# yuanzhi-zhu/DiffPIR

Hardware: AMD Instinct MI355X
Metric: restored images/sec @100 NFE, 256x256 (higher is better)
Workload: dtype f32 (GEMMs as 3 x f16 MFMA on hi/lo-split fp32 operands, fp32 accumulate; exact-fp32-MFMA mode in alt_precision); 1 GPU; configs[1]: ffhq topology 256x256 deblur (61x61 Gaussian PSF), 100 NFE, batch 16/GPU, device Philox noise, hipGraph=on; global_batch=16, nfe=100, collective=none

## Files before the change

### diffpir_amd/_lib.py

```python
from __future__ import annotations

import ctypes as C
import os

_HERE = os.path.dirname(os.path.abspath(__file__))
LIB_PATH = os.environ.get("DIFFPIR_LIB") or os.path.join(_HERE, "csrc", "libdiffpir_hip.so")
ABI_VERSION = 2



class UNetDesc(C.Structure):
    _fields_ = [("image_size", C.c_int32), ("in_channels", C.c_int32), ("model_channels", C.c_int32),
                ("out_channels", C.c_int32), ("num_res_blocks", C.c_int32), ("num_head_channels", C.c_int32),
                ("n_channel_mult", C.c_int32), ("channel_mult", C.c_float * 8),
                ("n_attention_ds", C.c_int32), ("attention_ds", C.c_int32 * 8), ("num_classes", C.c_int32)]


class Tensor(C.Structure):
    _fields_ = [("name", C.c_char_p), ("data", C.c_void_p), ("ndim", C.c_int32), ("shape", C.c_int64 * 4)]


class Step(C.Structure):
    _fields_ = [("t", C.c_int32), ("last", C.c_int32), ("c1", C.c_float), ("c2", C.c_float), ("tau", C.c_float),
                ("sa_t", C.c_float), ("s1m_t", C.c_float), ("sa_p", C.c_float),
                ("k1", C.c_float), ("q", C.c_float), ("es", C.c_float), ("k2", C.c_float)]


class ImageStep(C.Structure):
    _fields_ = [("tau", C.c_float), ("k1", C.c_float), ("k2", C.c_float), ("reserved", C.c_float)]


class LoopDesc(C.Structure):
    _fields_ = [("task", C.c_int32), ("B", C.c_int32), ("H", C.c_int32), ("W", C.c_int32), ("sf", C.c_int32),
                ("kh", C.c_int32), ("kw", C.c_int32), ("in_iter", C.c_int32), ("gamma", C.c_float),
                ("guidance", C.c_float), ("sa_start", C.c_float), ("s1m_start", C.c_float),
                ("y_dev", C.c_void_p), ("k_dev", C.c_void_p), ("mask_dev", C.c_void_p), ("labels_host", C.c_void_p),
                ("noise_init_dev", C.c_void_p), ("noise_n1_dev", C.c_void_p), ("noise_n2_dev", C.c_void_p),
                ("seed", C.c_uint64), ("image_offset", C.c_int64), ("use_graph", C.c_int32),
                ("skip_dead_final_eval", C.c_int32), ("generate_mode", C.c_int32), ("first_order", C.c_int32),
                ("noise_rp_dev", C.c_void_p), ("ddim_sample", C.c_int32)]


class InpaintRow(C.Structure):
    _fields_ = [("t", C.c_int32), ("last", C.c_int32), ("pos", C.c_int32), ("back", C.c_int32),
                ("c1", C.c_float), ("c2", C.c_float), ("tau", C.c_float), ("sa_t", C.c_float), ("s1m_t", C.c_float), ("sa_p", C.c_float),
                ("k1", C.c_float), ("q", C.c_float), ("es", C.c_float), ("k2", C.c_float),
                ("sae", C.c_float), ("sb", C.c_float), ("sa_n", C.c_float), ("s1m_n", C.c_float),
                ("mix_next", C.c_int32), ("reserved", C.c_int32)]


class ProgressDesc(C.Structure):
    _fields_ = [("panel_of_step_host", C.POINTER(C.c_int32)), ("n_entries", C.c_int32), ("n_panels", C.c_int32),
                ("strip_f32", C.c_void_p), ("strip_u8", C.c_void_p), ("masked_f32", C.c_void_p), ("masked_u8", C.c_void_p),
                ("minmax_dev", C.c_void_p)]


class DpsCoef(C.Structure):
    _fields_ = [("pc1", C.c_float), ("pc2", C.c_float), ("min_log", C.c_float), ("max_log", C.c_float), ("sa_prev", C.c_float), ("s1m_prev", C.c_float)]


class PSampleCoef(C.Structure):
    _fields_ = [("c1", C.c_float), ("c2", C.c_float), ("pc1", C.c_float), ("pc2", C.c_float), ("min_log", C.c_float), ("max_log", C.c_float),
                ("ddim", C.c_int32), ("sa_prev", C.c_float), ("s1m_prev", C.c_float)]


class DegradeDesc(C.Structure):
    _fields_ = [("task", C.c_int32), ("B", C.c_int32), ("H", C.c_int32), ("W", C.c_int32), ("sf", C.c_int32),
                ("kh", C.c_int32), ("kw", C.c_int32), ("noise_level_img", C.c_float), ("seed", C.c_uint64), ("image_offset", C.c_int64)]


class Conv3Desc(C.Structure):
    _fields_ = ([(n, C.c_int32) for n in ("B", "ca", "cb", "Cout", "H", "W", "mode", "res_mode", "scaled", "prologue", "route", "split",
                                          "defer", "Cout2")] +
                [(n, C.c_void_p) for n in ("xa", "xb", "w", "bias", "res", "prm", "gamma", "beta", "film", "gamma2", "beta2", "w2", "bias2",
                                           "out", "stat_out", "out2")] +
                [(n, C.c_int32) for n in ("stat_kind_out", "path_out", "ksplit_out", "reserved")])


class Conv9Desc(C.Structure):
    _fields_ = ([(n, C.c_int32) for n in ("B", "Cin", "Cout", "H", "W", "res_mode", "hop", "Cout2")] +
                [(n, C.c_void_p) for n in ("x", "w", "bias", "res", "prm", "gamma2", "beta2", "film2", "w2", "bias2", "out", "stat_out", "out2")] +
                [(n, C.c_int32) for n in ("ran_out", "iters")] + [("ms_out", C.c_double)])


class Conv11Desc(C.Structure):
    _fields_ = ([(n, C.c_int32) for n in ("B", "Cin", "Cout", "H", "W", "res_mode", "route", "ksplit", "hop", "Cout2")] +
                [(n, C.c_void_p) for n in ("x", "w", "bias", "res", "prm", "gamma2", "beta2", "film2", "w2", "bias2", "out", "stat_out", "out2")] +
                [(n, C.c_int32) for n in ("ran_out", "iters")] + [("ms_out", C.c_double)])


class ConvUpDesc(C.Structure):
    _fields_ = ([(n, C.c_int32) for n in ("B", "Cin", "Cout", "Hs", "Ws", "hop", "force_hop", "Cout2", "route", "reserved")] +
                [(n, C.c_void_p) for n in ("x", "w", "bias", "res", "prm", "gamma2", "beta2", "film2", "w2", "bias2", "out", "stat_out", "out2")] +
                [(n, C.c_int32) for n in ("ran_out", "iters")] + [("ms_out", C.c_double)])


class RouteRec(C.Structure):
    _fields_ = ([("layer", C.c_char * 80)] + [(n, C.c_int32) for n in ("kernel", "ks", "ksplit", "hop", "stat_kind", "reserved")] +
                [("workgroups", C.c_longlong)])


class ConvKnobs(C.Structure):
    _fields_ = [(n, C.c_int32) for n in ("conv8", "conv9", "conv9_min_wg", "conv11", "conv_up", "split_below", "split_target", "fuse_small",
                                         "fuse_h1", "emit_skip")]


CONV3_QUERY_FIELDS = ("B", "Cin", "Cout", "H", "W", "precision", "grad", "w16", "w8", "w11", "conv8_source", "defer", "hop", "has_res", "stats",
                      "force_kernel")


class Conv3Query(C.Structure):
    _fields_ = [(n, C.c_int32) for n in CONV3_QUERY_FIELDS] + [("slab_floats", C.c_longlong)]


class ConvPlan(C.Structure):
    _fields_ = ([(n, C.c_int32) for n in ("kernel", "hop", "geo", "ksplit", "chunks_per_split", "stat_kind", "stat_slots", "refused")] +
                [("workgroups", C.c_longlong)])


class ResblockQuery(C.Structure):
    _fields_ = ([(n, C.c_int32) for n in ("B", "Cin", "Cout", "H", "W", "mode", "concat", "precision", "grad", "hop_allowed")] +
                [("arena_words_left", C.c_longlong), ("slab_floats", C.c_longlong)])


class ResblockPlan(C.Structure):
    _fields_ = [(n, C.c_int32) for n in ("up", "skip_emit", "hop", "arena_counters")] + [("conv1", ConvPlan), ("conv2", ConvPlan)]


def route_log(engine):
    dbg = load_debug()
    n = C.c_int(0)
    assert dbg.dpir_debug_route_log(engine.h, None, 0, C.byref(n)) == 0
    recs = (RouteRec * max(n.value, 1))()
    assert dbg.dpir_debug_route_log(engine.h, recs, n.value, C.byref(n)) == 0
    return [dict(layer=r.layer.decode(), kernel=r.kernel, ks=r.ks, ksplit=r.ksplit, hop=r.hop, stat_kind=r.stat_kind, workgroups=r.workgroups)
            for r in recs[:n.value]]


class AttentionDesc(C.Structure):
    _fields_ = ([(n, C.c_int32) for n in ("B", "C", "T", "head_ch")] + [(n, C.c_void_p) for n in ("qkv", "dAtt", "out", "dqkv")] +
                [("guard_bad_out", C.c_uint64)])


class GroupNormDesc(C.Structure):
    _fields_ = ([(n, C.c_int32) for n in ("B", "ca", "cb", "Hs", "Ws", "mode", "silu", "acc_a", "acc_b", "reserved")] +
                [(n, C.c_void_p) for n in ("xa", "xb", "gamma", "beta", "film", "dA", "ga_init", "gb_init", "extra",
                                           "prm_out", "stats_out", "ga_out", "gb_out")] +
                [(n, C.c_int32) for n in ("ns_out", "reserved2")] + [("guard_bad_out", C.c_uint64)])


PROF_CLASSES = 8
PROF_NAMES = ["conv3x3", "conv1x1", "groupnorm_stats", "attention", "fft_prox", "elementwise", "unet_forward", "loop_graph"]

SIGNATURES = {
    "dpir_version": (C.c_int, []),
    "dpir_device_count": (C.c_int, [C.POINTER(C.c_int)]),
    "dpir_create": (C.c_int, [C.c_int, C.POINTER(C.c_void_p)]),
    "dpir_destroy": (None, [C.c_void_p]),
    "dpir_last_error": (C.c_char_p, [C.c_void_p]),
    "dpir_sync": (C.c_int, [C.c_void_p]),
    "dpir_stream": (C.c_void_p, [C.c_void_p]),
    "dpir_malloc": (C.c_int, [C.c_void_p, C.c_size_t, C.POINTER(C.c_void_p)]),
    "dpir_free": (C.c_int, [C.c_void_p, C.c_void_p]),
    "dpir_h2d": (C.c_int, [C.c_void_p, C.c_void_p, C.c_void_p, C.c_size_t]),
    "dpir_d2h": (C.c_int, [C.c_void_p, C.c_void_p, C.c_void_p, C.c_size_t]),
    "dpir_d2d": (C.c_int, [C.c_void_p, C.c_void_p, C.c_void_p, C.c_size_t]),
    "dpir_load_unet": (C.c_int, [C.c_void_p, C.POINTER(UNetDesc), C.POINTER(Tensor), C.c_int]),
    "dpir_set_precision": (C.c_int, [C.c_void_p, C.c_int]),
    "dpir_unet_forward": (C.c_int, [C.c_void_p, C.c_void_p, C.c_void_p, C.c_void_p, C.c_void_p, C.c_int, C.c_int, C.c_int]),
    "dpir_model_fn_xstart": (C.c_int, [C.c_void_p, C.c_void_p, C.c_int, C.c_float, C.c_float, C.c_void_p, C.c_void_p,
                                       C.c_int, C.c_int, C.c_int]),
    "dpir_enable_grad": (C.c_int, [C.c_void_p, C.c_int]),
    "dpir_unet_vjp": (C.c_int, [C.c_void_p, C.c_void_p, C.c_void_p, C.c_void_p, C.c_void_p, C.c_void_p, C.c_void_p, C.c_int, C.c_int, C.c_int]),
    "dpir_run_dps_loop": (C.c_int, [C.c_void_p, C.POINTER(LoopDesc), C.POINTER(Step), C.POINTER(DpsCoef), C.c_int, C.c_int, C.c_float,
                                    C.c_void_p, C.c_void_p, C.c_float, C.c_void_p, C.c_void_p]),
    "dpir_p_sample": (C.c_int, [C.c_void_p, C.c_void_p, C.c_int, C.POINTER(PSampleCoef), C.c_void_p, C.c_void_p, C.c_void_p, C.c_void_p, C.c_int, C.c_int, C.c_int]),
    "dpir_eps_from_xstart": (C.c_int, [C.c_void_p, C.c_void_p, C.c_void_p, C.c_float, C.c_float, C.c_int, C.c_void_p, C.c_size_t]),
    "dpir_grad_and_value": (C.c_int, [C.c_void_p, C.c_int, C.c_void_p, C.c_void_p, C.c_int, C.c_void_p, C.c_void_p, C.c_int, C.c_int, C.c_int]),
    "dpir_blur_reflect": (C.c_int, [C.c_void_p, C.c_void_p, C.c_void_p, C.c_int, C.c_int, C.c_float, C.c_float, C.c_void_p, C.c_int, C.c_int, C.c_int]),
    "dpir_blur_reflect_adjoint": (C.c_int, [C.c_void_p, C.c_void_p, C.c_void_p, C.c_int, C.c_int, C.c_float, C.c_void_p, C.c_int, C.c_int, C.c_int]),
    "dpir_grad_and_value_blur": (C.c_int, [C.c_void_p, C.c_int, C.c_void_p, C.c_void_p, C.c_void_p, C.c_int, C.c_int, C.c_void_p, C.c_void_p,
                                           C.c_int, C.c_int, C.c_int]),
    "dpir_run_deblur_grad_loop": (C.c_int, [C.c_void_p, C.POINTER(LoopDesc), C.POINTER(Step), C.POINTER(DpsCoef), C.c_int, C.c_int, C.c_float,
                                            C.c_void_p, C.c_void_p, C.c_void_p, C.c_void_p]),
    "dpir_unet_read_tap": (C.c_int, [C.c_void_p, C.c_char_p, C.c_void_p, C.c_size_t, C.POINTER(C.c_size_t)]),
    "dpir_prox_fft_precalc": (C.c_int, [C.c_void_p, C.c_void_p, C.c_void_p, C.c_int, C.c_int, C.c_int, C.c_int, C.c_int,
                                        C.c_int, C.POINTER(C.c_void_p)]),
    "dpir_prox_free": (None, [C.c_void_p, C.c_void_p]),
    "dpir_prox_read": (C.c_int, [C.c_void_p, C.c_void_p, C.c_int, C.c_void_p, C.c_size_t]),
    "dpir_data_solution": (C.c_int, [C.c_void_p, C.c_void_p, C.c_void_p, C.c_float, C.c_void_p]),
    "dpir_prox_fft_apply": (C.c_int, [C.c_void_p, C.c_void_p, C.c_void_p, C.c_float, C.c_float]),
    "dpir_set_prox_launch": (C.c_int, [C.c_void_p, C.c_int]),
    "dpir_prox_fft_apply_timed": (C.c_int, [C.c_void_p, C.c_void_p, C.c_void_p, C.c_float, C.c_float, C.c_int, C.c_int, C.POINTER(C.c_float)]),
    "dpir_prox_mask": (C.c_int, [C.c_void_p, C.c_void_p, C.c_void_p, C.c_void_p, C.c_float, C.c_float, C.c_int, C.c_int, C.c_int]),
    "dpir_resize_down": (C.c_int, [C.c_void_p, C.c_void_p, C.c_void_p, C.c_int, C.c_int, C.c_int, C.c_int]),
    "dpir_prox_ibp": (C.c_int, [C.c_void_p, C.c_void_p, C.c_void_p, C.c_float, C.c_float, C.c_int, C.c_int, C.c_int, C.c_int, C.c_int]),
    "dpir_bicubic_up": (C.c_int, [C.c_void_p, C.c_void_p, C.c_void_p, C.c_int, C.c_int, C.c_int, C.c_int]),
    "dpir_renoise": (C.c_int, [C.c_void_p, C.c_void_p, C.c_void_p, C.POINTER(Step), C.c_void_p, C.c_void_p, C.c_int, C.c_int, C.c_int]),
    "dpir_repaint_mix": (C.c_int, [C.c_void_p, C.c_void_p, C.c_void_p, C.c_void_p, C.c_void_p, C.c_void_p, C.c_int, C.c_int, C.c_int]),
    "dpir_finalize": (C.c_int, [C.c_void_p, C.c_void_p, C.c_void_p, C.c_void_p, C.c_int, C.c_int, C.c_int]),
    "dpir_progress_snapshot": (C.c_int, [C.c_void_p, C.c_void_p, C.c_void_p, C.c_void_p, C.c_int, C.c_int, C.c_void_p, C.c_void_p, C.c_void_p, C.c_void_p,
                                         C.c_void_p, C.c_int, C.c_int, C.c_int]),
    "dpir_set_progress": (C.c_int, [C.c_void_p, C.POINTER(ProgressDesc)]),
    "dpir_randn": (C.c_int, [C.c_void_p, C.c_void_p, C.c_uint64, C.c_uint64, C.c_int64, C.c_int, C.c_int, C.c_int, C.c_int]),
    "dpir_ewise": (C.c_int, [C.c_void_p, C.c_int, C.c_void_p, C.c_void_p, C.c_size_t, C.c_float, C.c_void_p, C.c_size_t]),
    "dpir_comm_unique_id": (C.c_int, [C.c_void_p]),
    "dpir_comm_version": (C.c_int, [C.POINTER(C.c_int)]),
    "dpir_device_info": (C.c_int, [C.c_void_p, C.c_char_p, C.c_size_t]),
    "dpir_comm_init": (C.c_int, [C.c_void_p, C.c_int, C.c_int, C.c_void_p]),
    "dpir_allgather_results": (C.c_int, [C.c_void_p, C.c_void_p, C.c_void_p, C.c_size_t]),
    "dpir_comm_allreduce_max": (C.c_int, [C.c_void_p, C.POINTER(C.c_double)]),
    "dpir_comm_barrier": (C.c_int, [C.c_void_p]),
    "dpir_comm_destroy": (C.c_int, [C.c_void_p]),
    "dpir_degrade": (C.c_int, [C.c_void_p, C.POINTER(DegradeDesc), C.c_void_p, C.c_void_p, C.c_void_p, C.c_void_p, C.c_void_p]),
    "dpir_metrics": (C.c_int, [C.c_void_p, C.c_void_p, C.c_void_p, C.c_int, C.c_int, C.c_int, C.c_void_p, C.c_void_p]),
    "dpir_lpips_load": (C.c_int, [C.c_void_p, C.POINTER(Tensor), C.c_int]),
    "dpir_lpips": (C.c_int, [C.c_void_p, C.c_void_p, C.c_void_p, C.c_void_p, C.c_int, C.c_int, C.c_int, C.c_void_p]),
    "dpir_lpips_keep_taps": (C.c_int, [C.c_void_p, C.c_int]),
    "dpir_lpips_read_tap": (C.c_int, [C.c_void_p, C.c_int, C.c_void_p, C.c_size_t, C.POINTER(C.c_size_t)]),
    "dpir_fid_load": (C.c_int, [C.c_void_p, C.POINTER(Tensor), C.c_int]),
    "dpir_fid_features": (C.c_int, [C.c_void_p, C.c_void_p, C.c_void_p, C.c_int, C.c_int, C.c_int, C.c_void_p]),
    "dpir_fid_keep_taps": (C.c_int, [C.c_void_p, C.c_int]),
    "dpir_fid_read_tap": (C.c_int, [C.c_void_p, C.c_int, C.c_void_p, C.c_size_t, C.POINTER(C.c_size_t)]),
    "dpir_run_loop": (C.c_int, [C.c_void_p, C.POINTER(LoopDesc), C.POINTER(Step), C.c_int, C.c_void_p, C.c_void_p]),
    "dpir_run_loop_per_image": (C.c_int, [C.c_void_p, C.POINTER(LoopDesc), C.POINTER(Step), C.c_int, C.POINTER(ImageStep), C.POINTER(C.c_int64),
                                          C.c_void_p, C.c_void_p]),
    "dpir_randn_indexed": (C.c_int, [C.c_void_p, C.c_void_p, C.c_uint64, C.c_uint64, C.POINTER(C.c_int64), C.c_int, C.c_int, C.c_int, C.c_int]),
    "dpir_inpaint_step": (C.c_int, [C.c_void_p, C.c_void_p, C.c_void_p, C.c_int, C.c_void_p, C.c_void_p, C.POINTER(InpaintRow), C.c_int, C.c_float,
                                    C.c_void_p, C.c_void_p, C.c_void_p, C.c_void_p, C.c_uint64, C.c_int64, C.c_int, C.c_void_p, C.c_int, C.c_int, C.c_int]),
    "dpir_run_inpaint_loop": (C.c_int, [C.c_void_p, C.POINTER(LoopDesc), C.POINTER(InpaintRow), C.c_int, C.c_void_p, C.c_void_p, C.c_void_p]),
    "dpir_prof_enable": (C.c_int, [C.c_void_p, C.c_int]),
    "dpir_prof_reset": (C.c_int, [C.c_void_p]),
    "dpir_prof_read": (C.c_int, [C.c_void_p, C.POINTER(C.c_double), C.POINTER(C.c_int64)]),
    "dpir_graph_cache_size": (C.c_int, [C.c_void_p]),
    "dpir_unet_flops": (C.c_double, [C.c_void_p, C.c_int, C.c_int]),
    "dpir_unet_flops_class": (C.c_double, [C.c_void_p, C.c_int, C.c_int, C.c_int]),
}

_lib = None


class EngineLibraryError(RuntimeError):
    pass


DEBUG_LIB_PATH = os.path.join(_HERE, "csrc", "libdiffpir_dbg.so")
_dbg = None


def load_debug():
    global _dbg
    if _dbg is not None:
        return _dbg
    load()
    if not os.path.exists(DEBUG_LIB_PATH):
        raise EngineLibraryError(f"{DEBUG_LIB_PATH} not found: `make -C diffpir_amd/csrc` builds it next to the product library")
    d = C.CDLL(DEBUG_LIB_PATH)
    d.dpir_debug_conv_bench.argtypes = [C.c_void_p] + [C.c_int] * 10 + [C.POINTER(C.c_double)]
    d.dpir_debug_conv7_emit_supported.argtypes = [C.c_void_p] + [C.c_int] * 4 + [C.POINTER(C.c_int)]
    d.dpir_debug_victim.argtypes = [C.c_void_p, C.c_int, C.c_int, C.c_int, C.c_longlong, C.c_int, C.POINTER(C.c_ulonglong)]
    d.dpir_debug_victim_alu.argtypes = [C.c_void_p, C.c_int, C.c_int, C.c_int, C.c_int, C.POINTER(C.c_ulonglong)]
    for fn in (d.dpir_debug_victim_fft_pk, d.dpir_debug_victim_fft_nopk):
        fn.argtypes = [C.c_void_p, C.c_int, C.c_int, C.c_int, C.POINTER(C.c_ulonglong)]
    d.dpir_debug_conv7_check.argtypes = [C.c_void_p] + [C.c_int] * 10 + [C.POINTER(C.c_double), C.POINTER(C.c_double), C.POINTER(C.c_ulonglong),
                                                                        C.POINTER(C.c_float), C.POINTER(C.c_int)]
    d.dpir_debug_conv5_layer.argtypes = [C.c_void_p] + [C.c_int] * 7 + [C.c_void_p] * 7 + [C.POINTER(C.c_int)]
    d.dpir_debug_conv5_layer.restype = C.c_int
    d.dpir_debug_conv3_layer.argtypes = [C.c_void_p, C.POINTER(Conv3Desc)]
    d.dpir_debug_conv3_layer.restype = C.c_int
    d.dpir_debug_conv9_layer.argtypes = [C.c_void_p, C.POINTER(Conv9Desc)]
    d.dpir_debug_conv9_layer.restype = C.c_int
    d.dpir_debug_conv11_layer.argtypes = [C.c_void_p, C.POINTER(Conv11Desc)]
    d.dpir_debug_conv11_layer.restype = C.c_int
    d.dpir_debug_conv_up_layer.argtypes = [C.c_void_p, C.POINTER(ConvUpDesc)]
    d.dpir_debug_conv_up_layer.restype = C.c_int
    d.dpir_debug_route_log.argtypes = [C.c_void_p, C.POINTER(RouteRec), C.c_int, C.POINTER(C.c_int)]
    d.dpir_debug_route_log.restype = C.c_int
    d.dpir_debug_conv_knobs_default.argtypes = [C.POINTER(ConvKnobs)]
    d.dpir_debug_conv_knobs_default.restype = None
    d.dpir_debug_conv3_plan.argtypes = [C.c_void_p, C.c_int, C.POINTER(ConvKnobs)] + [C.c_int] * 3 + [C.c_void_p]
    d.dpir_debug_conv3_plan.restype = C.c_int
    d.dpir_debug_resblock_plan.argtypes = [C.POINTER(ResblockQuery), C.POINTER(ConvKnobs)] + [C.c_int] * 3 + [C.POINTER(ResblockPlan)]
    d.dpir_debug_resblock_plan.restype = C.c_int
    d.dpir_debug_attention.argtypes = [C.c_void_p, C.POINTER(AttentionDesc)]
    d.dpir_debug_attention.restype = C.c_int
    d.dpir_debug_groupnorm.argtypes = [C.c_void_p, C.POINTER(GroupNormDesc)]
    d.dpir_debug_groupnorm.restype = C.c_int
    for n in ("dpir_debug_conv_bench", "dpir_debug_victim", "dpir_debug_victim_alu", "dpir_debug_victim_fft_pk", "dpir_debug_victim_fft_nopk",
              "dpir_debug_conv7_check"):
        getattr(d, n).restype = C.c_int
    _dbg = d
    return d


def load():
    global _lib
    if _lib is not None:
        return _lib
    if not os.path.exists(LIB_PATH):
        raise EngineLibraryError(
            f"{LIB_PATH} not found: build it with `python -c 'import __graft_entry__ as g; g.build()'` "
            f"or `make -C diffpir_amd/csrc`.  There is no CPU fallback.")
    try:
        import torch
    except ImportError:
        pass
    try:
        lib = C.CDLL(LIB_PATH)
    except OSError as ex:
        raise EngineLibraryError(f"cannot load {LIB_PATH}: {ex}") from ex
    for name, (res, args) in SIGNATURES.items():
        try:
            fn = getattr(lib, name)
        except AttributeError as ex:
            raise EngineLibraryError(f"{LIB_PATH} does not export {name}") from ex
        fn.restype = res
        fn.argtypes = args
    if lib.dpir_version() != ABI_VERSION:
        raise EngineLibraryError("ABI version mismatch")
    _lib = lib
    return lib
```

### diffpir_amd/csrc/conv_plan.cpp

```cpp
#include "conv_plan.h"
#include <stdlib.h>
namespace dpir {

static bool env_on(const char* name) { const char* v = getenv(name); return !(v && atoi(v) == 0); }
static int env_int(const char* name, int dflt) { const char* v = getenv(name); return v ? atoi(v) : dflt; }

const ConvKnobs& ConvKnobs::from_env() {
    static const ConvKnobs knobs = [] {
        ConvKnobs k;
        k.conv8 = env_on("DPIR_CONV8");
        k.conv9 = env_on("DPIR_CONV9");
        k.conv9_min_wg = env_int("DPIR_CONV9_MIN_WG", k.conv9_min_wg);
        k.conv11 = env_on("DPIR_CONV11");
        k.conv_up = env_on("DPIR_CONV_UP");
        k.split_below = env_int("DPIR_SPLIT_BELOW", k.split_below);
        k.split_target = env_int("DPIR_SPLIT_TARGET", k.split_target);
        k.fuse_small = env_on("DPIR_FUSE_SMALL");
        k.fuse_h1 = env_on("DPIR_FUSE_H1");
        k.emit_skip = env_int("DPIR_EMIT_SKIP", k.emit_skip);
        return k;
    }();
    return knobs;
}

static const size_t k4GiB = (size_t)1 << 32;

Conv3Geometry geometry(int H, int W) {
    Conv3Geometry g;
    if ((W & 3) || W < 8 || H < 8) return g;
    g.geo = W >= 32 ? 0 : (W >= 16 ? 1 : 2);
    g.tw = g.geo == 0 ? 32 : (g.geo == 1 ? 16 : 8);
    g.th = g.geo == 1 ? 16 : 8;
    g.ti = g.geo == 2 ? 4 : 1;
    g.tiles_x = (W + g.tw - 1) / g.tw;
    g.tiles_y = (H + g.th - 1) / g.th;
    g.stat_slots = g.tiles_x * g.tiles_y * ((g.tw * g.th) / 64);
    return g;
}

bool group_in_wave(int Cout, int wave_channels) { return Cout >= 32 && Cout % 32 == 0 && wave_channels % (Cout / 32) == 0; }

bool conv8_shape_ok(int B, int C, int Cout, int H, int W) {
    return B > 0 && Cout >= 1 && Cout <= 16 && C % 32 == 0 && C >= 32 && C <= kConv8MaxC && H % 8 == 0 && W % 32 == 0 &&
           (size_t)C * H * W < ((size_t)1 << 30);
}

const char* conv9_refusal(int B, int Cin, int Cout, int H, int W, bool hop) {
    if (B <= 0 || Cin <= 0 || Cout <= 0) return "conv9: empty launch";
    if (H != W) return "conv9: whole-image tiles need a square image";
    if (H != 8) return "conv9: the whole-image tile is built for 8 x 8 layers only";
    if (Cin % 16) return "conv9: the input channels must be a multiple of 16";
    if (Cout % 32) return "conv9: the output channels must be a multiple of 32";
    if (hop && !group_in_wave(Cout, 32)) return "conv9: fused emission needs GroupNorm groups that do not straddle a 32-channel tile";
    if ((size_t)B * (Cin / 8) * H * W * 16 >= k4GiB) return "conv9: split activation plane exceeds the 4 GiB buffer-descriptor range";
    return nullptr;
}

bool conv11_shape_ok(int Cin, int Cout, int H, int W) {
    return Cin > 0 && Cin % 32 == 0 && Cout > 0 && Cout % 128 == 0 && W > 0 && W % 32 == 0 && H > 0 && H % 8 == 0;
}
bool conv11_hop_ok(int Cout, int H, int W, int capacity) {
    if (Cout <= 0 || Cout % 128 || W <= 0 || W % 32 || H <= 0 || H % 8 || !group_in_wave(Cout, 64)) return false;
    return (W / 32) * (H / 8) <= capacity / 2;
}

long long conv_up_workgroups(int B, int Cout, int Hs, int Ws) { return (long long)B * (Ws / 32) * (Hs / 8) * ((Cout + 63) / 64) * 2; }

const char* conv_up_refusal(int B, int Cin, int Cout, int Hs, int Ws, bool hop, int min_wg_hop, int capacity) {
    if (B <= 0 || Cin <= 0 || Cout <= 0 || Hs <= 0 || Ws <= 0) return "conv_up: bad shape";
    if (Ws & 31) return "conv_up: the source width must be a multiple of 32";
    if (Hs & 7) return "conv_up: the source height must be a multiple of 8";
    if (Cin & 15) return "conv_up: the input channels must be a multiple of 16";
    if (Cout & 31) return "conv_up: the output channels must be a multiple of 32";
    const size_t HW = (size_t)Hs * Ws;
    if ((size_t)B * (Cin / 8) * HW * 16 >= k4GiB || (size_t)Cout * HW * 16 >= k4GiB || conv_up_workgroups(B, Cout, Hs, Ws) >= ((long long)1 << 31))
        return "conv_up: operand planes or one image's output exceed the 4 GiB buffer-descriptor range";
    if (hop) {
        if ((Cout & 63) || !group_in_wave(Cout, 32)) return "conv_up: GroupNorm groups of the hop must not straddle a wave's 32 channels (Cout 128, 256, 512 or 1024)";
        const int wait_set = 2 * (Ws / 32) * (Hs / 8);
        if (wait_set > capacity / 2) return "conv_up: the hop's wait set exceeds half of the resident workgroups";
        if (conv_up_workgroups(B, Cout, Hs, Ws) < min_wg_hop) return "conv_up: too few workgroups for the hop";
        if ((size_t)B * (Cout / 8) * HW * 4 * 16 >= k4GiB) return "conv_up: the emitted planes exceed the 4 GiB range";
    }
    return nullptr;
}

bool conv7_hop_ok(int B, int Cout, int H, int W, int capacity) {
    if (geometry(H, W).geo != 0 || (W & 31) || (H & 7) || Cout <= 0 || (Cout & 127) || !group_in_wave(Cout, 64)) return false;
    const long long tiles = (long long)(W / 32) * (H / 8);
    return tiles <= capacity / 2 && tiles * (Cout / 128) * B >= kHopMinWg;
}

static Conv3Plan refuse(const char* why, int geo = -1) { Conv3Plan p; p.refusal = why; p.geo = geo; return p; }

Conv3Plan plan_conv67(const Conv3Query& q, const ConvKnobs& knobs, const DeviceCaps& caps) {
    const Conv3Geometry g = geometry(q.H, q.W);
    if (!g.ok()) return refuse("conv6: shape not tiled");
    Conv3Plan p;
    p.geo = g.geo;
    const int chunks = (q.Cin + 15) / 16;
    const long long blocks = (long long)g.pixel_tiles(q.B) * ((q.Cout + 127) / 128);
    if (blocks < 1 || chunks < 1) return refuse("conv6: empty launch", g.geo);
    int S = 1;
    if (q.slab && blocks < knobs.split_below) {
        S = (int)((knobs.split_target + blocks - 1) / blocks);
        if (S > chunks / 2) S = chunks / 2;
        if (S > 16) S = 16;
        if (S < 1) S = 1;
        if ((size_t)S * q.B * q.Cout * q.H * q.W > q.slab_floats) S = 1;
    }
    p.chunks_per_split = (chunks + S - 1) / S;
    S = (chunks + p.chunks_per_split - 1) / p.chunks_per_split;
    p.ksplit = S;
    p.workgroups = blocks * S;
    if (q.hop) {
        if (S != 1 || !conv7_hop_ok(q.B, q.Cout, q.H, q.W, caps.conv7) || q.has_res || q.out_scale_dev)
            return refuse("conv6: this launch cannot emit the next convolution's planes", g.geo);
        p.kernel = CK_CONV7; p.hop = true;
        return p;
    }
    const bool idle_half = (q.Cout & 127) != 0 && (q.Cout & 127) <= 64 && q.Cout > 32;
    const bool use6 = q.force_kernel == CK_CONV6 || (q.force_kernel != CK_CONV7 && g.geo == 0 && (S > 1 || idle_half));
    if (use6 && g.geo != 0) return refuse("conv6 is built for the 8 x 32 geometry only (conv7 has the 16 x 16 and 8 x 8 ones)", g.geo);
    p.kernel = use6 ? CK_CONV6 : (conv7_narrow(g.geo, q.Cout) ? CK_CONV7_NARROW : CK_CONV7);
    if (S > 1) p.stat_kind = q.defer ? ST_PENDING : (q.stat_plane ? ST_PLANE : ST_NONE);
    else if (q.stat_slots) { p.stat_kind = ST_SLOTS; p.stat_slots = g.stat_slots; }
    return p;
}

Conv3Plan plan_conv3(const Conv3Query& q, const ConvKnobs& knobs, const DeviceCaps& caps) {
    const Conv3Geometry g = geometry(q.H, q.W);
    const bool forced = q.force_kernel != 0;
    Conv3Plan p;
    if (!forced && knobs.conv8 && q.w8 && q.conv8_source && !q.grad && !q.hop && !q.has_res && conv8_shape_ok(q.B, q.Cin, q.Cout, q.H, q.W)) {
        p.kernel = CK_CONV8; p.geo = 0;
        p.workgroups = (long long)(q.W / 32) * (q.H / 8) * q.B;
        return p;
    }
    if (!q.w16 || !g.ok()) {
        if (q.hop) return refuse("conv: fused emission was requested for a launch that is not on the f16 3x3 path");
        if (forced) return refuse("conv: a kernel cannot be forced here (f32 engine or a shape the f16 path refuses)");
        return p;
    }
    const bool f16_infer = !q.grad && q.precision != 0;
    if (q.force_kernel == CK_CONV9 || (!forced && knobs.conv9 && (long long)q.B * (q.Cout / 32) >= knobs.conv9_min_wg)) {
        const char* why = conv9_refusal(q.B, q.Cin, q.Cout, q.H, q.W, q.hop);
        if (f16_infer && !why) {
            p.kernel = CK_CONV9; p.hop = q.hop; p.geo = g.geo;
            p.workgroups = (long long)q.B * (q.Cout / 32);
            if (!q.hop && q.stat_plane) p.stat_kind = ST_PLANE;
            return p;
        }
        if (forced) return refuse(why ? why : "conv9: an f16 inference forward only");
    }
    if (q.force_kernel == CK_CONV11 || (!forced && knobs.conv11)) {
        const long long wgs = (long long)(q.W / 32) * (q.H / 8) * q.B * (q.Cout / 128);
        const bool shape = f16_infer && q.precision == 1 && q.w11 && conv11_shape_ok(q.Cin, q.Cout, q.H, q.W);
        const bool enough = forced || wgs >= (q.hop ? kHopMinWg : knobs.split_below);
        if (shape && enough && (!q.hop || conv11_hop_ok(q.Cout, q.H, q.W, caps.conv11))) {
            p.kernel = CK_CONV11; p.hop = q.hop; p.geo = 0; p.workgroups = wgs;
            if (!q.hop && q.stat_slots) { p.stat_kind = ST_SLOTS; p.stat_slots = g.stat_slots; }
            return p;
        }
        if (forced) return refuse("conv11: f16x3 inference, Cin % 32 == 0, Cout % 128 == 0, 8 x 32 tiles inside the image; the hop: groups inside a wave and an image's tiles resident");
    }
    return plan_conv67(q, knobs, caps);
}

ResblockPlan plan_resblock(const ResblockQuery& q, const ConvKnobs& knobs, const DeviceCaps& caps) {
    ResblockPlan rp;
    const int Ho = q.mode == 1 ? q.H * 2 : (q.mode == 2 ? q.H / 2 : q.H), Wo = q.mode == 1 ? q.W * 2 : (q.mode == 2 ? q.W / 2 : q.W);
    const Conv3Geometry g = geometry(Ho, Wo);
    const bool stats = g.stat_slots > 0 && q.Cout % 32 == 0;
    const bool hops = q.hop_allowed && knobs.fuse_h1 && !q.grad && q.precision != 0;
    const bool arena = hops && q.arena_words_left > 0;
    auto arena_room = [&](int counters) { return (size_t)q.B * 64 + (size_t)q.B * counters <= q.arena_words_left; };
    Conv3Query c1, c2;
    c1.B = c2.B = q.B; c1.H = c2.H = Ho; c1.W = c2.W = Wo; c1.Cout = c2.Cout = c2.Cin = q.Cout; c1.Cin = q.Cin;
    c1.precision = c2.precision = q.precision; c1.grad = c2.grad = q.grad;
    c1.w16 = q.conv1_w16; c1.w11 = q.conv1_w11; c2.w16 = q.conv2_w16; c2.w11 = q.conv2_w11;
    c1.slab = c2.slab = q.slab; c1.slab_floats = c2.slab_floats = q.slab_floats;
    c1.defer = c2.defer = knobs.fuse_small;
    c1.stat_slots = c1.stat_plane = c2.stat_slots = c2.stat_plane = stats;
    c2.has_res = true;

    rp.up = knobs.conv_up && q.mode == 1 && !q.grad && q.precision != 0 && q.conv1_wup && !q.concat && q.Cin == q.gn1_c &&
            !conv_up_refusal(q.B, q.Cin, q.Cout, q.H, q.W, false, 0, 0) && conv_up_workgroups(q.B, q.Cout, q.H, q.W) >= knobs.split_below;
    if (rp.up) {
        const bool hop = arena && q.gn2_c == q.Cout && q.conv2_w16 && g.ok() && !conv_up_refusal(q.B, q.Cin, q.Cout, q.H, q.W, true, kHopMinWg, caps.conv_up) &&
                         arena_room(q.Cout / 64);
        rp.conv1.kernel = CK_CONV_UP; rp.conv1.hop = hop; rp.conv1.geo = 0;
        rp.conv1.workgroups = conv_up_workgroups(q.B, q.Cout, q.H, q.W);
        if (hop) { rp.hop = HOP_CONV_UP; rp.arena_counters = q.Cout / 64; }
        else { rp.conv1.stat_kind = ST_SLOTS; rp.conv1.stat_slots = g.stat_slots; }
        rp.conv2 = plan_conv3(c2, knobs, caps);
        return rp;
    }
    rp.skip_emit = (knobs.emit_skip == 2 || (knobs.emit_skip == 1 && q.Cout <= 128)) && q.has_skip && q.mode == 0 && q.conv1_w16 && q.skip_w16 && g.ok() &&
                   q.conv5_ok && q.Cin % 16 == 0 && q.Cin <= kConv5EmitMaxC && (Ho * Wo) % 256 == 0 &&
                   (size_t)q.B * (2 * ((q.Cin + 15) / 16)) * Ho * Wo * 16 < k4GiB && !(knobs.fuse_small && q.small_prologue);
    const bool hop_arena = arena && q.conv1_w16 && q.conv2_w16 && q.gn2_c == q.Cout && conv7_hop_ok(q.B, q.Cout, Ho, Wo, caps.conv7) &&
                           arena_room(q.Cout / 128) && (size_t)q.B * (2 * ((q.Cout + 15) / 16)) * Ho * Wo * 16 < k4GiB;
    c1.hop = true;
    const bool hop9 = !rp.skip_emit && hops && q.gn2_c == q.Cout && plan_conv3(c1, knobs, caps).kernel == CK_CONV9 &&
                      plan_conv3(c2, knobs, caps).kernel == CK_CONV9;
    rp.hop = hop9 ? HOP_CONV9 : (hop_arena ? HOP_ARENA : HOP_NONE);
    if (rp.hop == HOP_ARENA) rp.arena_counters = q.Cout / 128;
    c1.hop = rp.hop != HOP_NONE;
    if (c1.hop) { c1.slab = false; c1.slab_floats = 0; c1.stat_slots = c1.stat_plane = false; }
    rp.conv1 = plan_conv3(c1, knobs, caps);
    rp.conv2 = plan_conv3(c2, knobs, caps);
    return rp;
}

}
```

### diffpir_amd/csrc/conv_plan.h

```cpp
#pragma once
#include <cstddef>
namespace dpir {

constexpr int kHopMinWg = 384;
constexpr int kConv9MinWg = 128;
constexpr int kConv5EmitMaxC = 384;
constexpr int kConv8MaxC = 256;

struct ConvKnobs {
    bool conv8 = true;
    bool conv9 = true;
    int conv9_min_wg = kConv9MinWg;
    bool conv11 = true;
    bool conv_up = true;
    int split_below = 256;
    int split_target = 256;
    bool fuse_small = true;
    bool fuse_h1 = true;
    int emit_skip = 1;
    static const ConvKnobs& from_env();
};

struct DeviceCaps { int conv7 = 0, conv11 = 0, conv_up = 0; };

struct Conv3Geometry {
    int geo = -1;
    int tw = 0, th = 0, ti = 0;
    int tiles_x = 0, tiles_y = 0;
    int stat_slots = 0;
    bool ok() const { return geo >= 0; }
    int pixel_tiles(int B) const { return tiles_x * tiles_y * ((B + ti - 1) / ti); }
};
Conv3Geometry geometry(int H, int W);

bool group_in_wave(int Cout, int wave_channels);
inline bool conv7_narrow(int geo, int Cout) { return geo == 0 && Cout <= 32; }

bool conv8_shape_ok(int B, int C, int Cout, int H, int W);
const char* conv9_refusal(int B, int Cin, int Cout, int H, int W, bool hop);
bool conv11_shape_ok(int Cin, int Cout, int H, int W);
bool conv11_hop_ok(int Cout, int H, int W, int capacity);
long long conv_up_workgroups(int B, int Cout, int Hs, int Ws);
const char* conv_up_refusal(int B, int Cin, int Cout, int Hs, int Ws, bool hop, int min_wg_hop, int capacity);
bool conv7_hop_ok(int B, int Cout, int H, int W, int capacity);

enum ConvKernel { CK_FP32 = 0, CK_CONV5 = 5, CK_CONV6 = 6, CK_CONV7 = 7, CK_CONV8 = 8, CK_CONV9 = 9, CK_CONV11 = 11, CK_CONV_UP = 12,
                  CK_CONV7_NARROW = 17, CK_RESOLVE = 60 };
enum StatKind { ST_NONE = 0, ST_SLOTS = 1, ST_PLANE = 2, ST_PENDING = 3 };
enum HopKind { HOP_NONE = 0, HOP_ARENA = 1, HOP_CONV9 = 2, HOP_CONV_UP = 3 };

struct Conv3Query {
    int B = 0, Cin = 0, Cout = 0, H = 0, W = 0;
    int precision = 1;
    bool grad = false;
    bool w16 = false, w8 = false, w11 = false;
    bool conv8_source = false;
    bool slab = false; size_t slab_floats = 0;
    bool defer = false;
    bool hop = false;
    bool has_res = false, out_scale_dev = false;
    bool stat_slots = false, stat_plane = false;
    int force_kernel = 0;
};
struct Conv3Plan {
    int kernel = CK_FP32;
    bool hop = false;
    int geo = -1;
    long long workgroups = 0;
    int ksplit = 1, chunks_per_split = 0;
    int stat_kind = ST_NONE, stat_slots = 0;
    const char* refusal = nullptr;
};
Conv3Plan plan_conv67(const Conv3Query& q, const ConvKnobs& knobs, const DeviceCaps& caps);
Conv3Plan plan_conv3(const Conv3Query& q, const ConvKnobs& knobs, const DeviceCaps& caps);

struct ResblockQuery {
    int B = 0, Cin = 0, Cout = 0, H = 0, W = 0;
    int mode = 0;
    bool concat = false, has_skip = false;
    int gn1_c = 0, gn2_c = 0;
    int precision = 1; bool grad = false;
    bool hop_allowed = false;
    size_t arena_words_left = 0;
    bool conv1_w16 = false, conv1_w11 = false, conv1_wup = false, conv2_w16 = false, conv2_w11 = false, skip_w16 = false;
    bool small_prologue = false;
    bool conv5_ok = false;
    bool slab = false; size_t slab_floats = 0;
};
struct ResblockPlan {
    bool up = false;
    bool skip_emit = false;
    int hop = HOP_NONE;
    int arena_counters = 0;
    Conv3Plan conv1, conv2;
};
ResblockPlan plan_resblock(const ResblockQuery& q, const ConvKnobs& knobs, const DeviceCaps& caps);

}
```

### diffpir_amd/csrc/dbg_conv.hip

```cpp
#include "engine.h"
#include "conv6_params.h"
#include "conv9.h"
#include "conv11.h"
#include "conv_up.h"
#include "../../include/diffpir_debug.h"
#include <string.h>
#include <vector>
using namespace dpir;
static int fail(dpir_engine* e, const Status& s) {
    if (e) e->last_error = s.msg;
    return s.code;
}
#define API_TRY(e, expr)                          \
    do {                                          \
        Status _s = (expr);                       \
        if (!_s.ok()) return fail((e), _s);       \
    } while (0)
#define API_HIP(e, expr)                                                                  \
    do {                                                                                  \
        hipError_t _h = (expr);                                                           \
        if (_h != hipSuccess)                                                             \
            return fail((e), Status{DPIR_ERR_HIP, std::string(#expr) + ": " + hipGetErrorString(_h)}); \
    } while (0)

__global__ void dbg_bitdiff_kernel(const float* a, const float* b, size_t n, unsigned long long* out) {
    unsigned long long cnt = 0; unsigned mx = 0;
    for (size_t i = (size_t)blockIdx.x * blockDim.x + threadIdx.x; i < n; i += (size_t)gridDim.x * blockDim.x) {
        const float x = a[i], y = b[i];
        if (__builtin_bit_cast(unsigned, x) != __builtin_bit_cast(unsigned, y)) {
            ++cnt;
            const float d = fabsf(x - y);
            const unsigned u = d == d ? __builtin_bit_cast(unsigned, d) : 0x7fc00000u;
            mx = u > mx ? u : mx;
        }
    }
    if (cnt) { atomicAdd(&out[0], cnt); atomicMax(&out[1], (unsigned long long)mx); }
}

template <class F>
static Status time_repeats(hipStream_t s, int iters, F&& launch, double* ms_out) {
    if (iters <= 0) return Status{};
    hipEvent_t e0, e1;
    DPIR_HIP(hipEventCreate(&e0)); DPIR_HIP(hipEventCreate(&e1));
    DPIR_HIP(hipEventRecord(e0, s));
    for (int i = 0; i < iters; ++i) DPIR_TRY(launch());
    DPIR_HIP(hipEventRecord(e1, s));
    DPIR_HIP(hipEventSynchronize(e1));
    float ms = 0; DPIR_HIP(hipEventElapsedTime(&ms, e0, e1));
    (void)hipEventDestroy(e0); (void)hipEventDestroy(e1);
    *ms_out = ms / iters;
    return Status{};
}

static Status fold_slots(const float2* st, size_t planes, int slots, double* stat_out) {
    std::vector<float2> hs(planes * slots);
    DPIR_HIP(hipMemcpy(hs.data(), st, hs.size() * 8, hipMemcpyDeviceToHost));
    for (size_t pl = 0; pl < planes; ++pl) {
        double s1 = 0.0, s2 = 0.0;
        for (int k = 0; k < slots; ++k) { s1 += (double)hs[pl * slots + k].x; s2 += (double)hs[pl * slots + k].y; }
        stat_out[2 * pl] = s1; stat_out[2 * pl + 1] = s2;
    }
    return Status{};
}

struct HopStage {
    char* s16b = nullptr; size_t plane2 = 0, no2 = 0, arena_words = 0;
    float *dbias2 = nullptr, *dout2 = nullptr; void* wp2 = nullptr; float w2_scale = 1.f; long long* arena = nullptr;
    Conv6Emit em;
};
template <class Desc>
static Status hop_stage(dpir_engine* e, const std::string& tag, const Desc* d, int B, int Cout, size_t HW, bool x1, int counters, HopStage* h) {
    const int Co2 = d->Cout2, C8b = 2 * ((Cout + 15) / 16);
    h->plane2 = (size_t)B * C8b * HW * 16; h->no2 = (size_t)B * Co2 * HW;
    float *dg = nullptr, *db = nullptr, *df = nullptr;
    DPIR_TRY(e->ws.getT(tag + "#s16b", 2 * h->plane2, &h->s16b));
    DPIR_TRY(e->ws.getT(tag + "#gamma2", (size_t)Cout, &dg));
    DPIR_TRY(e->ws.getT(tag + "#beta2", (size_t)Cout, &db));
    DPIR_TRY(e->ws.getT(tag + "#film2", (size_t)B * 2 * Cout, &df));
    DPIR_TRY(e->ws.getT(tag + "#b2", (size_t)round_up(Co2, 64), &h->dbias2));
    DPIR_TRY(e->ws.getT(tag + "#o2", h->no2, &h->dout2));
    DPIR_HIP(hipMemsetAsync(h->s16b, 0xFF, 2 * h->plane2, e->stream));
    DPIR_HIP(hipMemcpy(dg, d->gamma2, (size_t)Cout * 4, hipMemcpyHostToDevice));
    DPIR_HIP(hipMemcpy(db, d->beta2, (size_t)Cout * 4, hipMemcpyHostToDevice));
    if (d->film2) DPIR_HIP(hipMemcpy(df, d->film2, (size_t)B * 2 * Cout * 4, hipMemcpyHostToDevice));
    DPIR_HIP(hipMemset(h->dbias2, 0, (size_t)round_up(Co2, 64) * 4));
    DPIR_HIP(hipMemcpy(h->dbias2, d->bias2, (size_t)Co2 * 4, hipMemcpyHostToDevice));
    DPIR_HIP(hipMemsetAsync(h->dout2, 0xFF, h->no2 * 4, e->stream));
    std::vector<uint16_t> w16b;
    h->w2_scale = pack_weights_conv6(d->w2, Co2, Cout, w16b);
    DPIR_TRY(e->ws.get(tag + "#w16b", w16b.size() * 2, &h->wp2));
    DPIR_HIP(hipMemcpy(h->wp2, w16b.data(), w16b.size() * 2, hipMemcpyHostToDevice));
    Conv6Emit& em = h->em;
    em.hi = h->s16b; em.lo = x1 ? nullptr : h->s16b + h->plane2; em.C8 = C8b; em.gamma = dg; em.beta = db;
    em.film = d->film2 ? df : nullptr; em.film_stride = 2 * Cout; em.film_off = 0; em.frows = 2 * Cout; em.fstep = nullptr;
    em.range_ctr = e->range_ctr;
    if (counters > 0) {
        h->arena_words = (size_t)B * 64 + ((size_t)B * counters + 1) / 2;
        DPIR_TRY(e->ws.getT(tag + "#arena", h->arena_words, &h->arena));
        em.acc = h->arena; em.cnt = reinterpret_cast<unsigned*>(h->arena + (size_t)B * 64);
    }
    return Status{};
}
static Conv6Args second_conv6(const HopStage& h, int B, int Cin, int Cout, int H, int W, bool x1) {
    Conv6Args c6;
    c6.x1 = x1; c6.xhi = h.s16b; c6.xlo = h.s16b + h.plane2; c6.w16 = h.wp2; c6.w16_scale = h.w2_scale;
    c6.bias = h.dbias2; c6.out = h.dout2; c6.B = B; c6.Cin = Cin; c6.Cout = Cout; c6.H = H; c6.W = W;
    return c6;
}

extern "C" {
int dpir_debug_conv_bench(dpir_engine* e, int B, int Cin, int Cout, int H, int W, int ks, int mode, int with_prm,
                          int dbg, int iters, double* ms_out) {
    if (!e || !ms_out || iters <= 0) return DPIR_ERR_INVALID;
    (void)hipSetDevice(e->device);
    int taps = ks * ks, coutp = round_up(Cout, 64), cinp = round_up(Cin, 16);
    float *x = nullptr, *w = nullptr, *bias = nullptr, *out = nullptr, *partial = nullptr; float4* prm = nullptr;
    API_TRY(e, e->ws.getT("dbg#x", (size_t)B * Cin * H * W, &x));
    API_TRY(e, e->ws.getT("dbg#w", (size_t)cinp * taps * coutp, &w));
    API_TRY(e, e->ws.getT("dbg#b", (size_t)coutp, &bias));
    API_TRY(e, e->ws.getT("dbg#o", (size_t)B * Cout * H * W, &out));
    API_TRY(e, e->ws.getT("dbg#prm", (size_t)B * Cin, &prm));
    API_TRY(e, e->ws.getT("conv#partial", (size_t)16 * 1024 * 1024, &partial));
    API_TRY(e, launch_randn(e->stream, x, 1, 1, 0, 1, (size_t)B * Cin * H * W));
    API_TRY(e, launch_randn(e->stream, w, 2, 1, 0, 1, (size_t)cinp * taps * coutp));
    API_TRY(e, launch_randn(e->stream, bias, 3, 1, 0, 1, (size_t)coutp));
    API_TRY(e, launch_randn(e->stream, reinterpret_cast<float*>(prm), 4, 1, 0, 1, (size_t)B * Cin * 4));
    ConvArgs a;
    a.src.a = x; a.src.ca = Cin; a.src.Hs = H; a.src.Ws = W; a.src.mode = 0; a.src.prm = with_prm ? prm : nullptr;
    a.w = w; a.bias = bias; a.out = out; a.B = B; a.Cin = Cin; a.Cout = Cout; a.CoutP = coutp; a.H = H; a.W = W; a.ks = ks;
    a.partial = partial; a.partial_capacity = (size_t)16 * 1024 * 1024;
    const void* w16 = nullptr; float w16_scale = 1.f;
    if (dbg != 0) {
        std::vector<float> hw((size_t)Cout * Cin * taps);
        for (size_t i = 0; i < hw.size(); ++i) hw[i] = (float)((i * 2654435761u) % 2001) / 1000.0f * 0.05f - 0.05f;
        std::vector<uint16_t> w16v;
        w16_scale = ks == 1 ? pack_weights_f16x3_1x1(hw.data(), Cout, Cin, w16v) : pack_weights_conv6(hw.data(), Cout, Cin, w16v);
        void* wp = nullptr;
        API_TRY(e, e->ws.get("dbg#w16", w16v.size() * 2, &wp));
        API_HIP(e, hipMemcpy(wp, w16v.data(), w16v.size() * 2, hipMemcpyHostToDevice));
        w16 = wp;
    }
    Conv5Args a5;
    Conv6Args a6;
    const bool use5 = dbg != 0 && ks == 1, use6 = dbg != 0 && ks == 3;
    if (use5) {
        a5.src = CatSrc{x, Cin, nullptr, 0}; a5.prm = a.src.prm; a5.w16 = w16; a5.w16_scale = w16_scale; a5.bias = bias; a5.out = out;
        a5.B = B; a5.Cout = Cout; a5.H = H; a5.W = W; a5.x1 = e->precision == 2;
    }
    if (use6) {
        int C8 = 2 * ((Cin + 15) / 16);
        size_t plane = (size_t)B * C8 * H * W * 16;
        char* s16 = nullptr;
        API_TRY(e, e->ws.getT("dbg#s16", 2 * plane, &s16));
        API_TRY(e, launch_act_split(e->stream, CatSrc{x, Cin, nullptr, 0}, a.src.prm, 0, B, H, W, s16, s16 + plane));
        a6.xhi = s16; a6.xlo = s16 + plane; a6.w16 = w16; a6.w16_scale = w16_scale; a6.bias = bias; a6.out = out;
        a6.B = B; a6.Cin = Cin; a6.Cout = Cout; a6.H = H; a6.W = W; a6.partial = partial; a6.partial_capacity = a.partial_capacity;
        a6.x1 = e->precision == 2;
    }
    auto run_once = [&]() -> Status {
        if (use5) return launch_conv5(e->stream, a5);
        if (use6) {
            if (dbg == 1) DPIR_TRY(launch_act_split(e->stream, CatSrc{x, Cin, nullptr, 0}, a.src.prm, 0, B, H, W, const_cast<void*>(a6.xhi), const_cast<void*>(a6.xlo)));
            return launch_conv6(e->stream, a6);
        }
        return launch_conv(e->stream, a);
    };
    API_TRY(e, run_once());
    API_TRY(e, time_repeats(e->stream, iters, run_once, ms_out));
    return DPIR_OK;
}

int dpir_debug_conv7_check(dpir_engine* e, int B, int Cin, int Cout, int H, int W, int res_mode, int x1, int split, int scaled, int iters,
                            double* ms6_out, double* ms7_out, unsigned long long* mismatches_out, float* maxdiff_out, int* ksplit_out) {
    if (!e || !ms6_out || !ms7_out || !mismatches_out || !maxdiff_out || !ksplit_out || iters <= 0 || res_mode < -1 || res_mode > 2) return DPIR_ERR_INVALID;
    (void)hipSetDevice(e->device);
    if (!conv6_supported(H, W) || W < 32) return fail(e, invalid("conv7 check: conv6 only has the 8 x 32 geometry (W >= 32) to compare with"));
    const size_t nx = (size_t)B * Cin * H * W, no = (size_t)B * Cout * H * W;
    const size_t nres = res_mode == 1 ? no / 4 : (res_mode == 2 ? no * 4 : no);
    const int slots = conv6_stat_slots(H, W);
    const size_t nst = (size_t)B * Cout * slots;
    const size_t pcap = (size_t)16 * no;
    float *x = nullptr, *bias = nullptr, *o6 = nullptr, *o7 = nullptr, *res = nullptr, *p6 = nullptr, *p7 = nullptr, *scale = nullptr;
    float2 *st6 = nullptr, *st7 = nullptr;
    unsigned long long* cmp = nullptr;
    API_TRY(e, e->ws.getT("c7#x", nx, &x));
    API_TRY(e, e->ws.getT("c7#b", (size_t)round_up(Cout, 64), &bias));
    API_TRY(e, e->ws.getT("c7#o6", no, &o6));
    API_TRY(e, e->ws.getT("c7#o7", no, &o7));
    API_TRY(e, e->ws.getT("c7#res", nres, &res));
    API_TRY(e, e->ws.getT("c7#st6", nst, &st6));
    API_TRY(e, e->ws.getT("c7#st7", nst, &st7));
    API_TRY(e, e->ws.getT("c7#cmp", (size_t)2, &cmp));
    API_TRY(e, e->ws.getT("c7#scale", (size_t)4, &scale));
    if (split) { API_TRY(e, e->ws.getT("c7#p6", pcap, &p6)); API_TRY(e, e->ws.getT("c7#p7", pcap, &p7)); }
    API_TRY(e, launch_randn(e->stream, x, 11, 1, 0, 1, nx));
    API_TRY(e, launch_randn(e->stream, bias, 12, 1, 0, 1, (size_t)round_up(Cout, 64)));
    API_TRY(e, launch_randn(e->stream, res, 13, 1, 0, 1, nres));
    const float quarter = 0.25f;
    API_HIP(e, hipMemcpyAsync(scale, &quarter, 4, hipMemcpyHostToDevice, e->stream));
    std::vector<float> hw((size_t)Cout * Cin * 9);
    for (size_t i = 0; i < hw.size(); ++i) hw[i] = (float)((i * 2654435761u) % 2001) / 1000.0f * 0.05f - 0.05f;
    std::vector<uint16_t> w16v;
    const float w16_scale = pack_weights_conv6(hw.data(), Cout, Cin, w16v);
    void* wp = nullptr;
    API_TRY(e, e->ws.get("c7#w16", w16v.size() * 2, &wp));
    API_HIP(e, hipMemcpy(wp, w16v.data(), w16v.size() * 2, hipMemcpyHostToDevice));
    const int chunks = (Cin + 15) / 16, C8 = 2 * chunks;
    const size_t plane = (size_t)B * C8 * H * W * 16;
    char* s16 = nullptr;
    API_TRY(e, e->ws.getT("c7#s16", 2 * plane, &s16));
    API_TRY(e, launch_act_split(e->stream, CatSrc{x, Cin, nullptr, 0}, nullptr, 0, B, H, W, s16, x1 ? nullptr : s16 + plane));
    Conv6Args a6;
    a6.xhi = s16; a6.xlo = x1 ? nullptr : s16 + plane; a6.w16 = wp; a6.w16_scale = w16_scale; a6.bias = bias;
    a6.B = B; a6.Cin = Cin; a6.Cout = Cout; a6.H = H; a6.W = W; a6.x1 = x1 != 0;
    if (res_mode >= 0) { a6.res = res; a6.res_mode = res_mode; }
    if (scaled) a6.out_scale_dev = scale;
    a6.out = o6; a6.stat = st6; a6.force_kernel = 6;
    if (split) { a6.partial = p6; a6.partial_capacity = pcap; }
    Conv3Query q;
    q.B = B; q.Cin = Cin; q.Cout = Cout; q.H = H; q.W = W; q.w16 = true; q.slab = split != 0; q.slab_floats = pcap; q.defer = true;
    q.has_res = res_mode >= 0; q.out_scale_dev = scaled != 0; q.stat_slots = true; q.force_kernel = CK_CONV7;
    const Conv3Plan plan7 = plan_conv67(q, ConvKnobs::from_env(), DeviceCaps{});
    if (plan7.refusal) return fail(e, invalid(plan7.refusal));
    const Conv3Geometry g = geometry(H, W);
    const int S = plan7.ksplit, blocks = (int)(plan7.workgroups / S);
    Conv6K k;
    k.xhi = reinterpret_cast<const char*>(a6.xhi); k.xlo = reinterpret_cast<const char*>(a6.xlo);
    k.w16 = reinterpret_cast<const char*>(wp); k.bias = bias; k.out = o7; k.res = a6.res; k.res_mode = a6.res_mode;
    k.B = B; k.Cout = Cout; k.H = H; k.W = W; k.n_chunks_total = chunks; k.C8 = C8;
    k.out_scale = 1.0f / w16_scale; k.out_scale_dev = a6.out_scale_dev; k.zeros = nullptr;
    k.tiles_x = g.tiles_x; k.tiles_y = g.tiles_y; k.n_co_blocks = (Cout + 127) / 128;
    k.chunks_per_split = plan7.chunks_per_split; k.ksplit = S; k.partial = S > 1 ? p7 : nullptr;
    k.stat = S == 1 ? st7 : nullptr; k.stat_slots = plan7.stat_slots;
    *ksplit_out = S;
    API_HIP(e, hipMemsetAsync(o6, 0xFF, no * 4, e->stream));
    API_HIP(e, hipMemsetAsync(o7, 0x7F, no * 4, e->stream));
    API_HIP(e, hipMemsetAsync(st6, 0xFF, nst * 8, e->stream));
    API_HIP(e, hipMemsetAsync(st7, 0x7F, nst * 8, e->stream));
    if (split) { API_HIP(e, hipMemsetAsync(p6, 0xFF, (size_t)S * no * 4, e->stream)); API_HIP(e, hipMemsetAsync(p7, 0x7F, (size_t)S * no * 4, e->stream)); }
    API_HIP(e, hipMemsetAsync(cmp, 0, 16, e->stream));
    Conv3Plan plan6;
    PendingConv pend;
    API_TRY(e, launch_conv6(e->stream, a6, &plan6, &pend));
    if (plan6.kernel != CK_CONV6 || plan6.ksplit != S) return fail(e, Status{DPIR_ERR_INVALID, "conv7 check: forcing the kernel changed the plan"});
    API_TRY(e, launch_conv7(e->stream, k, blocks * S, x1 != 0));
    API_HIP(e, hipGetLastError());
    if (S > 1) {
        hipLaunchKernelGGL(dbg_bitdiff_kernel, dim3(2048), dim3(256), 0, e->stream, p6, p7, (size_t)S * no, cmp);
    } else {
        hipLaunchKernelGGL(dbg_bitdiff_kernel, dim3(2048), dim3(256), 0, e->stream, o6, o7, no, cmp);
        hipLaunchKernelGGL(dbg_bitdiff_kernel, dim3(256), dim3(256), 0, e->stream, reinterpret_cast<const float*>(st6), reinterpret_cast<const float*>(st7), nst * 2, cmp);
    }
    unsigned long long h[2] = {0, 0};
    API_HIP(e, hipMemcpyAsync(h, cmp, 16, hipMemcpyDeviceToHost, e->stream));
    API_HIP(e, hipStreamSynchronize(e->stream));
    *mismatches_out = h[0];
    const unsigned mb = (unsigned)h[1];
    *maxdiff_out = __builtin_bit_cast(float, mb);
    hipEvent_t e0, e1, e2;
    API_HIP(e, hipEventCreate(&e0)); API_HIP(e, hipEventCreate(&e1)); API_HIP(e, hipEventCreate(&e2));
    for (int i = 0; i < 3; ++i) { API_TRY(e, launch_conv6(e->stream, a6, &plan6, &pend)); API_TRY(e, launch_conv7(e->stream, k, blocks * S, x1 != 0)); }
    API_HIP(e, hipEventRecord(e0, e->stream));
    for (int i = 0; i < iters; ++i) API_TRY(e, launch_conv6(e->stream, a6, &plan6, &pend));
    API_HIP(e, hipEventRecord(e1, e->stream));
    for (int i = 0; i < iters; ++i) API_TRY(e, launch_conv7(e->stream, k, blocks * S, x1 != 0));
    API_HIP(e, hipEventRecord(e2, e->stream));
    API_HIP(e, hipEventSynchronize(e2));
    float m6 = 0, m7 = 0;
    API_HIP(e, hipEventElapsedTime(&m6, e0, e1)); API_HIP(e, hipEventElapsedTime(&m7, e1, e2));
    (void)hipEventDestroy(e0); (void)hipEventDestroy(e1); (void)hipEventDestroy(e2);
    *ms6_out = m6 / iters; *ms7_out = m7 / iters;
    return DPIR_OK;
}

int dpir_debug_conv5_layer(dpir_engine* e, int B, int ca, int cb, int Cout, int H, int W, int tile, const float* xa, const float* xb,
                           const float* w, const float* bias, const float* prm, const float* res, float* out, int* path_out) {
    if (!e || !xa || !w || !bias || !out || !path_out || B <= 0 || ca <= 0 || cb < 0 || (cb > 0 && !xb) || Cout <= 0 || tile < 0 || tile > 2) return DPIR_ERR_INVALID;
    if (e->precision == 0) return fail(e, invalid("conv5 layer: the engine is in f32 mode"));
    (void)hipSetDevice(e->device);
    const int C = ca + cb, HW = H * W;
    const size_t na = (size_t)B * ca * HW, nb = (size_t)B * cb * HW, no = (size_t)B * Cout * HW;
    float *dxa = nullptr, *dxb = nullptr, *dbias = nullptr, *dout = nullptr, *dres = nullptr, *dw = nullptr, *partial = nullptr; float4* dprm = nullptr;
    API_TRY(e, e->ws.getT("c5#xa", na, &dxa));
    API_TRY(e, e->ws.getT("c5#xb", nb + 1, &dxb));
    API_TRY(e, e->ws.getT("c5#b", (size_t)round_up(Cout, 64), &dbias));
    API_TRY(e, e->ws.getT("c5#o", no, &dout));
    API_TRY(e, e->ws.getT("c5#res", no, &dres));
    API_TRY(e, e->ws.getT("c5#prm", (size_t)B * C, &dprm));
    API_HIP(e, hipMemcpy(dxa, xa, na * 4, hipMemcpyHostToDevice));
    if (cb) API_HIP(e, hipMemcpy(dxb, xb, nb * 4, hipMemcpyHostToDevice));
    API_HIP(e, hipMemset(dbias, 0, (size_t)round_up(Cout, 64) * 4));
    API_HIP(e, hipMemcpy(dbias, bias, (size_t)Cout * 4, hipMemcpyHostToDevice));
    if (prm) API_HIP(e, hipMemcpy(dprm, prm, (size_t)B * C * 16, hipMemcpyHostToDevice));
    if (res) API_HIP(e, hipMemcpy(dres, res, no * 4, hipMemcpyHostToDevice));
    API_HIP(e, hipMemset(dout, 0xFF, no * 4));
    std::vector<uint16_t> w16v;
    const float w16_scale = pack_weights_f16x3_1x1(w, Cout, C, w16v);
    void* wp = nullptr;
    API_TRY(e, e->ws.get("c5#w16", w16v.size() * 2, &wp));
    API_HIP(e, hipMemcpy(wp, w16v.data(), w16v.size() * 2, hipMemcpyHostToDevice));
    const bool has_prm = prm != nullptr;
    const bool use5 = !(has_prm && C % 16) && (tile != 0 || conv5_supported(B, Cout, H, W, has_prm) || conv5_small_supported(B, ca, cb, Cout, H, W, has_prm));
    Status st;
    if (use5) {
        Conv5Args a5;
        a5.src = CatSrc{dxa, ca, cb ? dxb : nullptr, cb}; a5.prm = has_prm ? dprm : nullptr; a5.w16 = wp; a5.w16_scale = w16_scale;
        a5.bias = dbias; a5.out = dout; a5.res = res ? dres : nullptr; a5.B = B; a5.Cout = Cout; a5.H = H; a5.W = W;
// ... 179 lines not shown
        float* o2 = nullptr;
        API_TRY(e, e->ws.getT("c3#o_again", no, &o2));
        b6.out = o2;
        API_HIP(e, hipStreamSynchronize(e->stream));
        std::vector<float> first(no);
        API_HIP(e, hipMemcpy(first.data(), dout, no * 4, hipMemcpyDeviceToHost));
        API_TRY(e, launch_conv6(e->stream, b6, nullptr, &probe));
        if (probe.partial) API_TRY(e, launch_conv6_resolve(e->stream, probe));
        API_HIP(e, hipStreamSynchronize(e->stream));
        std::vector<float> again(no);
        API_HIP(e, hipMemcpy(again.data(), o2, no * 4, hipMemcpyDeviceToHost));
        if (memcmp(first.data(), again.data(), no * 4) != 0) return fail(e, Status{DPIR_ERR_STATE, "conv3 layer: two identical split-K launches disagree"});
    }
    if (d->defer) {
        if (kind != ST_PENDING) return fail(e, invalid("conv3 layer: defer was asked for but launch_conv6 did not split this launch"));
        const int Cn = Cout, Co2 = d->Cout2;
        if (Cn % 16 || !gn_act_small_supported(Cn, H, W, 0)) return fail(e, Status{DPIR_ERR_UNSUPPORTED, "conv3 layer: gn_act_small refuses the second stage"});
        const int C8b = 2 * ((Cn + 15) / 16);
        const size_t plane2 = (size_t)B * C8b * HW * 16, no2 = (size_t)B * Co2 * HW;
        char* s16b = nullptr; float *dg = nullptr, *db = nullptr, *dbias2 = nullptr, *dout2 = nullptr;
        API_TRY(e, e->ws.getT("c3#s16b", 2 * plane2, &s16b));
        API_TRY(e, e->ws.getT("c3#gamma2", (size_t)Cn, &dg));
        API_TRY(e, e->ws.getT("c3#beta2", (size_t)Cn, &db));
        API_TRY(e, e->ws.getT("c3#b2", (size_t)round_up(Co2, 64), &dbias2));
        API_TRY(e, e->ws.getT("c3#o2", no2, &dout2));
        API_HIP(e, hipMemset(s16b, 0xFF, 2 * plane2));
        API_HIP(e, hipMemcpy(dg, d->gamma2, (size_t)Cn * 4, hipMemcpyHostToDevice));
        API_HIP(e, hipMemcpy(db, d->beta2, (size_t)Cn * 4, hipMemcpyHostToDevice));
        API_HIP(e, hipMemset(dbias2, 0, (size_t)round_up(Co2, 64) * 4));
        API_HIP(e, hipMemcpy(dbias2, d->bias2, (size_t)Co2 * 4, hipMemcpyHostToDevice));
        API_HIP(e, hipMemset(dout2, 0xFF, no2 * 4));
        GnActArgs ga;
        ga.src = CatSrc{dout, Cn, nullptr, 0}; ga.pend = pc; ga.gamma = dg; ga.beta = db;
        ga.silu = true; ga.mode = 0; ga.B = B; ga.Hs = H; ga.Ws = W;
        ga.hi = s16b; ga.lo = x1 ? nullptr : s16b + plane2; ga.range_ctr = e->range_ctr;
        API_TRY(e, launch_gn_act_small(e->stream, ga));
        std::vector<uint16_t> w16b;
        const float w16b_scale = pack_weights_conv6(d->w2, Co2, Cn, w16b);
        void* wp2 = nullptr;
        API_TRY(e, e->ws.get("c3#w16b", w16b.size() * 2, &wp2));
        API_HIP(e, hipMemcpy(wp2, w16b.data(), w16b.size() * 2, hipMemcpyHostToDevice));
        Conv6Args c6;
        c6.x1 = x1; c6.xhi = s16b; c6.xlo = s16b + plane2; c6.w16 = wp2; c6.w16_scale = w16b_scale;
        c6.bias = dbias2; c6.out = dout2; c6.B = B; c6.Cin = Cn; c6.Cout = Co2; c6.H = H; c6.W = W;
        API_TRY(e, launch_conv6(e->stream, c6));
        API_HIP(e, hipStreamSynchronize(e->stream));
        API_HIP(e, hipMemcpy(d->out2, dout2, no2 * 4, hipMemcpyDeviceToHost));
    }
    API_HIP(e, hipStreamSynchronize(e->stream));
    API_HIP(e, hipMemcpy(d->out, dout, no * 4, hipMemcpyDeviceToHost));
    if (d->stat_out && (kind == 1 || kind == 2)) {
        if (kind == 1) {
            API_TRY(e, fold_slots(st, (size_t)B * Cout, slots, d->stat_out));
        } else {
            API_HIP(e, hipMemcpy(d->stat_out, sp, (size_t)B * Cout * 16, hipMemcpyDeviceToHost));
        }
    }
    return DPIR_OK;
}

int dpir_debug_conv9_layer(dpir_engine* e, dpir_debug_conv9_desc* d) {
    if (!e || !d) return DPIR_ERR_INVALID;
    d->ran_out = 0;
    const int B = d->B, Cin = d->Cin, Cout = d->Cout, H = d->H, W = d->W;
    if (!d->x || !d->w || !d->bias || B <= 0 || Cin <= 0 || Cout <= 0 || H <= 0 || W <= 0 || d->res_mode < -1 || d->res_mode > 2 ||
        (d->res_mode >= 0 && !d->res) || (!d->hop && !d->out) || (d->hop && (!d->gamma2 || !d->beta2 || !d->w2 || !d->bias2 || !d->out2 || d->Cout2 <= 0)))
        return fail(e, invalid("conv9 layer: bad descriptor"));
    if (e->grad_enabled) return fail(e, Status{DPIR_ERR_UNSUPPORTED, "conv9 layer: a gradient-mode engine keeps launch_conv6's route"});
    if (e->precision == 0) return fail(e, Status{DPIR_ERR_UNSUPPORTED, "conv9 layer: the f32 precision keeps the fp32 kernel"});
    if (d->hop && d->res_mode >= 0) return fail(e, invalid("conv9 layer: the hop's first layer takes no residual"));
    if ((d->res_mode == 1 && ((H | W) & 1))) return fail(e, invalid("conv9 layer: a half-resolution residual needs an even output size"));
    (void)hipSetDevice(e->device);
    const bool x1 = e->precision == 2;
    const size_t HW = (size_t)H * W, nx = (size_t)B * Cin * HW, no = (size_t)B * Cout * HW;
    const size_t nres = d->res_mode == 1 ? no / 4 : (d->res_mode == 2 ? no * 4 : no);
    const int chunks = (Cin + 15) / 16, C8 = 2 * chunks;
    const size_t plane = (size_t)B * C8 * HW * 16;
    float *dx = nullptr, *dbias = nullptr, *dout = nullptr, *dres = nullptr; float4* dprm = nullptr; double2* sp = nullptr; char* s16 = nullptr;
    API_TRY(e, e->ws.getT("c9#x", nx, &dx));
    API_TRY(e, e->ws.getT("c9#b", (size_t)round_up(Cout, 64), &dbias));
    API_TRY(e, e->ws.getT("c9#o", no, &dout));
    API_TRY(e, e->ws.getT("c9#res", nres, &dres));
    API_TRY(e, e->ws.getT("c9#prm", (size_t)B * Cin, &dprm));
    API_TRY(e, e->ws.getT("c9#sp", (size_t)B * Cout, &sp));
    API_TRY(e, e->ws.getT("c9#s16", 2 * plane, &s16));
    API_HIP(e, hipMemcpy(dx, d->x, nx * 4, hipMemcpyHostToDevice));
    API_HIP(e, hipMemset(dbias, 0, (size_t)round_up(Cout, 64) * 4));
    API_HIP(e, hipMemcpy(dbias, d->bias, (size_t)Cout * 4, hipMemcpyHostToDevice));
    if (d->prm) API_HIP(e, hipMemcpy(dprm, d->prm, (size_t)B * Cin * 16, hipMemcpyHostToDevice));
    if (d->res_mode >= 0) API_HIP(e, hipMemcpy(dres, d->res, nres * 4, hipMemcpyHostToDevice));
    API_HIP(e, hipMemsetAsync(dout, 0xFF, no * 4, e->stream));
    API_HIP(e, hipMemsetAsync(sp, 0xFF, (size_t)B * Cout * 16, e->stream));
    API_HIP(e, hipMemsetAsync(s16, 0xFF, 2 * plane, e->stream));
    API_TRY(e, launch_act_split(e->stream, CatSrc{dx, Cin, nullptr, 0}, d->prm ? dprm : nullptr, 0, B, H, W, s16, x1 ? nullptr : s16 + plane, e->range_ctr));
    std::vector<uint16_t> w16v;
    const float w16_scale = pack_weights_conv6(d->w, Cout, Cin, w16v);
    void* wp = nullptr;
    API_TRY(e, e->ws.get("c9#w16", w16v.size() * 2, &wp));
    API_HIP(e, hipMemcpy(wp, w16v.data(), w16v.size() * 2, hipMemcpyHostToDevice));
    Conv9Args a9;
    a9.xhi = s16; a9.xlo = s16 + plane; a9.w16 = wp; a9.w16_scale = w16_scale; a9.bias = dbias; a9.out = dout;
    if (d->res_mode >= 0) { a9.res = dres; a9.res_mode = d->res_mode; }
    a9.B = B; a9.Cin = Cin; a9.Cout = Cout; a9.H = H; a9.W = W; a9.stat_plane = sp; a9.x1 = x1;
    d->ms_out = 0.0;
    if (!d->hop) {
        API_TRY(e, launch_conv9(e->stream, a9));
        API_TRY(e, time_repeats(e->stream, d->iters, [&]() { return launch_conv9(e->stream, a9); }, &d->ms_out));
        API_HIP(e, hipStreamSynchronize(e->stream));
        d->ran_out = 1;
        API_HIP(e, hipMemcpy(d->out, dout, no * 4, hipMemcpyDeviceToHost));
        if (d->stat_out) API_HIP(e, hipMemcpy(d->stat_out, sp, (size_t)B * Cout * 16, hipMemcpyDeviceToHost));
        return DPIR_OK;
    }
    HopStage h;
    API_TRY(e, hop_stage(e, "c9", d, B, Cout, HW, x1, 0, &h));
    a9.out = nullptr; a9.stat_plane = nullptr; a9.emit = &h.em;
    API_TRY(e, launch_conv9(e->stream, a9));
    Conv9Args b9;
    b9.xhi = h.s16b; b9.xlo = h.s16b + h.plane2; b9.w16 = h.wp2; b9.w16_scale = h.w2_scale; b9.bias = h.dbias2; b9.out = h.dout2;
    b9.B = B; b9.Cin = Cout; b9.Cout = d->Cout2; b9.H = H; b9.W = W; b9.x1 = x1;
    API_TRY(e, launch_conv9(e->stream, b9));
    API_TRY(e, time_repeats(e->stream, d->iters, [&]() -> Status { DPIR_TRY(launch_conv9(e->stream, a9)); return launch_conv9(e->stream, b9); }, &d->ms_out));
    API_HIP(e, hipStreamSynchronize(e->stream));
    d->ran_out = 1;
    API_HIP(e, hipMemcpy(d->out2, h.dout2, h.no2 * 4, hipMemcpyDeviceToHost));
    return DPIR_OK;
}

int dpir_debug_conv11_layer(dpir_engine* e, dpir_debug_conv11_desc* d) {
    if (!e || !d) return DPIR_ERR_INVALID;
    d->ran_out = 0; d->ms_out = 0.0;
    const int B = d->B, Cin = d->Cin, Cout = d->Cout, H = d->H, W = d->W;
    if (!d->x || !d->w || !d->bias || (!d->hop && !d->out) || B <= 0 || Cin <= 0 || Cout <= 0 || H <= 0 || W <= 0 || d->res_mode < -1 || d->res_mode > 2 ||
        (d->res_mode >= 0 && !d->res) || (d->route != 0 && d->route != 7) || (d->hop && d->route != 0) ||
        (d->hop && (!d->gamma2 || !d->beta2 || !d->w2 || !d->bias2 || !d->out2 || d->Cout2 <= 0)))
        return fail(e, invalid("conv11 layer: bad descriptor"));
    if (d->hop && d->res_mode >= 0) return fail(e, invalid("conv11 layer: the hop's first layer takes no residual"));
    if ((d->res_mode == 1 && ((H | W) & 1))) return fail(e, invalid("conv11 layer: a half-resolution residual needs an even output size"));
    (void)hipSetDevice(e->device);
    const size_t HW = (size_t)H * W, nx = (size_t)B * Cin * HW, no = (size_t)B * Cout * HW;
    const size_t nres = d->res_mode == 1 ? no / 4 : (d->res_mode == 2 ? no * 4 : no);
    const int chunks = (Cin + 15) / 16, C8 = 2 * chunks;
    const size_t plane = (size_t)B * C8 * HW * 16;
    Conv11Args a11;
    a11.B = B; a11.Cin = Cin; a11.Cout = Cout; a11.H = H; a11.W = W;
    a11.ksplit = d->ksplit; a11.precision = e->precision; a11.grad = e->grad_enabled;
    if (d->route == 0) {
        Conv11Args probe = a11;
        if (probe.grad || probe.precision != 1 || probe.ksplit != 1 || !conv11_supported(Cin, Cout, H, W)) {
            const Status st = launch_conv11(e->stream, probe);
            if (!st.ok()) return fail(e, st);
        }
        if (d->hop && !conv11_emit_supported(Cout, H, W))
            return fail(e, Status{DPIR_ERR_UNSUPPORTED, "conv11 layer: fused emission needs GroupNorm groups inside a wave's 64 channels and an image's tiles resident with room to spare"});
    } else if (e->grad_enabled || e->precision != 1) {
        return fail(e, Status{DPIR_ERR_UNSUPPORTED, "conv11 layer: the conv7 arm is timed on an f16x3 inference engine"});
    }
    const int slots = conv6_stat_slots(H, W);
    const size_t nst = (size_t)B * Cout * slots;
    float *dx = nullptr, *dbias = nullptr, *dout = nullptr, *dres = nullptr; float4* dprm = nullptr; float2* st = nullptr; char* s16 = nullptr;
    API_TRY(e, e->ws.getT("c11#x", nx, &dx));
    API_TRY(e, e->ws.getT("c11#b", (size_t)round_up(Cout, 64), &dbias));
    API_TRY(e, e->ws.getT("c11#o", no, &dout));
    API_TRY(e, e->ws.getT("c11#res", nres, &dres));
    API_TRY(e, e->ws.getT("c11#prm", (size_t)B * Cin, &dprm));
    API_TRY(e, e->ws.getT("c11#st", nst > 0 ? nst : 1, &st));
    API_TRY(e, e->ws.getT("c11#s16", 2 * plane, &s16));
    API_HIP(e, hipMemcpy(dx, d->x, nx * 4, hipMemcpyHostToDevice));
    API_HIP(e, hipMemset(dbias, 0, (size_t)round_up(Cout, 64) * 4));
    API_HIP(e, hipMemcpy(dbias, d->bias, (size_t)Cout * 4, hipMemcpyHostToDevice));
    if (d->prm) API_HIP(e, hipMemcpy(dprm, d->prm, (size_t)B * Cin * 16, hipMemcpyHostToDevice));
    if (d->res_mode >= 0) API_HIP(e, hipMemcpy(dres, d->res, nres * 4, hipMemcpyHostToDevice));
    API_HIP(e, hipMemsetAsync(dout, 0xFF, no * 4, e->stream));
    if (nst) API_HIP(e, hipMemsetAsync(st, 0xFF, nst * 8, e->stream));
    API_HIP(e, hipMemsetAsync(s16, 0xFF, 2 * plane, e->stream));
    API_TRY(e, launch_act_split(e->stream, CatSrc{dx, Cin, nullptr, 0}, d->prm ? dprm : nullptr, 0, B, H, W, s16, s16 + plane, e->range_ctr));
    std::vector<uint16_t> w16v, w11v;
    const float w16_scale = pack_weights_conv6(d->w, Cout, Cin, w16v);
    void* wp = nullptr;
    if (d->route == 0) {
        pack_weights_conv11(d->w, Cout, Cin, w16_scale, w11v);
        API_TRY(e, e->ws.get("c11#w11", w11v.size() * 2, &wp));
        API_HIP(e, hipMemcpy(wp, w11v.data(), w11v.size() * 2, hipMemcpyHostToDevice));
    } else {
        API_TRY(e, e->ws.get("c11#w16", w16v.size() * 2, &wp));
        API_HIP(e, hipMemcpy(wp, w16v.data(), w16v.size() * 2, hipMemcpyHostToDevice));
    }
    a11.xhi = s16; a11.xlo = s16 + plane; a11.w11 = wp; a11.w_scale = w16_scale; a11.bias = dbias; a11.out = dout;
    if (d->res_mode >= 0) { a11.res = dres; a11.res_mode = d->res_mode; }
    a11.stat = nst ? st : nullptr;
    Conv6Args a6;
    a6.xhi = s16; a6.xlo = s16 + plane; a6.w16 = wp; a6.w16_scale = w16_scale; a6.bias = dbias; a6.out = dout;
    if (d->res_mode >= 0) { a6.res = dres; a6.res_mode = d->res_mode; }
    a6.B = B; a6.Cin = Cin; a6.Cout = Cout; a6.H = H; a6.W = W; a6.stat = nst ? st : nullptr; a6.force_kernel = 7;
    HopStage h;
    Conv6Args c6;
    if (d->hop) {
        API_TRY(e, hop_stage(e, "c11", d, B, Cout, HW, false, (Cout + 63) / 64, &h));
        a11.out = nullptr; a11.stat = nullptr; a11.emit = &h.em;
        c6 = second_conv6(h, B, Cout, d->Cout2, H, W, false);
    }
    auto launch = [&]() -> Status {
        if (d->route != 0) return launch_conv6(e->stream, a6);
        if (!d->hop) return launch_conv11(e->stream, a11);
        DPIR_HIP(hipMemsetAsync(h.arena, 0, h.arena_words * 8, e->stream));
        DPIR_TRY(launch_conv11(e->stream, a11));
        return launch_conv6(e->stream, c6);
    };
    API_TRY(e, launch());
    API_TRY(e, time_repeats(e->stream, d->iters, launch, &d->ms_out));
    API_HIP(e, hipStreamSynchronize(e->stream));
    d->ran_out = d->route == 0 ? (d->hop ? 12 : 11) : 7;
    if (d->hop) {
        API_HIP(e, hipMemcpy(d->out2, h.dout2, h.no2 * 4, hipMemcpyDeviceToHost));
        return DPIR_OK;
    }
    API_HIP(e, hipMemcpy(d->out, dout, no * 4, hipMemcpyDeviceToHost));
    if (d->stat_out && nst) API_TRY(e, fold_slots(st, (size_t)B * Cout, slots, d->stat_out));
    return DPIR_OK;
}

int dpir_debug_conv_up_layer(dpir_engine* e, dpir_debug_conv_up_desc* d) {
    if (!e || !d) return DPIR_ERR_INVALID;
    d->ran_out = 0; d->ms_out = 0.0;
    const int B = d->B, Cin = d->Cin, Cout = d->Cout, Hs = d->Hs, Ws = d->Ws;
    if (!d->x || !d->w || !d->bias || B <= 0 || Cin <= 0 || Cout <= 0 || Hs <= 0 || Ws <= 0 || (!d->hop && !d->out) || d->route < 0 || d->route > 1 ||
        (d->hop && (!d->gamma2 || !d->beta2 || !d->w2 || !d->bias2 || !d->out2 || d->Cout2 <= 0)))
        return fail(e, invalid("conv_up layer: bad descriptor"));
    if (e->grad_enabled) return fail(e, Status{DPIR_ERR_UNSUPPORTED, "conv_up layer: a gradient-mode engine keeps launch_conv6's route"});
    if (e->precision == 0) return fail(e, Status{DPIR_ERR_UNSUPPORTED, "conv_up layer: the f32 precision keeps the fp32 kernel"});
    if (d->res) return fail(e, invalid("conv_up: conv1 of an up-sampling ResBlock takes no residual"));
    const int min_wg = d->force_hop ? 0 : kHopMinWg;
    if (d->route == 0) {
        if (const char* why = conv_up_supported(B, Cin, Cout, Hs, Ws, d->hop != 0, min_wg)) return fail(e, Status{DPIR_ERR_UNSUPPORTED, why});
    } else if (Cin % 16 || !conv6_supported(2 * Hs, 2 * Ws) || (d->hop && !conv7_emit_supported(B, Cout, 2 * Hs, 2 * Ws))) {
        return fail(e, Status{DPIR_ERR_UNSUPPORTED, "conv_up layer: launch_conv6's route refuses this shape"});
    }
    (void)hipSetDevice(e->device);
    const bool x1 = e->precision == 2;
    const int H = 2 * Hs, W = 2 * Ws;
    const size_t HWs = (size_t)Hs * Ws, HW = 4 * HWs, nx = (size_t)B * Cin * HWs, no = (size_t)B * Cout * HW;
    const int C8 = 2 * ((Cin + 15) / 16);
    const size_t plane_s = (size_t)B * C8 * HWs * 16, plane = 4 * plane_s;
    const int slots = conv_up_stat_slots(Hs, Ws);
    const size_t nst = (size_t)B * Cout * slots;
    float *dx = nullptr, *dbias = nullptr, *dout = nullptr; float4* dprm = nullptr; float2* st = nullptr; char* s16 = nullptr;
    API_TRY(e, e->ws.getT("cu#x", nx, &dx));
    API_TRY(e, e->ws.getT("cu#b", (size_t)round_up(Cout, 64), &dbias));
    API_TRY(e, e->ws.getT("cu#o", no, &dout));
    API_TRY(e, e->ws.getT("cu#prm", (size_t)B * Cin, &dprm));
    API_TRY(e, e->ws.getT("cu#st", nst, &st));
    API_TRY(e, e->ws.getT("cu#s16", 2 * plane, &s16));
    API_HIP(e, hipMemcpy(dx, d->x, nx * 4, hipMemcpyHostToDevice));
    API_HIP(e, hipMemset(dbias, 0, (size_t)round_up(Cout, 64) * 4));
    API_HIP(e, hipMemcpy(dbias, d->bias, (size_t)Cout * 4, hipMemcpyHostToDevice));
    if (d->prm) API_HIP(e, hipMemcpy(dprm, d->prm, (size_t)B * Cin * 16, hipMemcpyHostToDevice));
    API_HIP(e, hipMemsetAsync(dout, 0xFF, no * 4, e->stream));
    API_HIP(e, hipMemsetAsync(st, 0xFF, nst * 8, e->stream));
    API_HIP(e, hipMemsetAsync(s16, 0xFF, 2 * plane, e->stream));
    std::vector<uint16_t> wv;
    const float w_scale = d->route == 0 ? pack_weights_conv_up(d->w, Cout, Cin, wv) : pack_weights_conv6(d->w, Cout, Cin, wv);
    void* wp = nullptr;
    API_TRY(e, e->ws.get("cu#w", wv.size() * 2, &wp));
    API_HIP(e, hipMemcpy(wp, wv.data(), wv.size() * 2, hipMemcpyHostToDevice));
    const CatSrc src{dx, Cin, nullptr, 0};
    const float4* prm = d->prm ? dprm : nullptr;
    HopStage h;
    if (d->hop) API_TRY(e, hop_stage(e, "cu", d, B, Cout, HW, x1, (Cout + 63) / 64, &h));
    auto once = [&]() -> Status {
        if (d->hop) DPIR_HIP(hipMemsetAsync(h.arena, 0, h.arena_words * 8, e->stream));
        if (d->route == 0) {
            DPIR_TRY(launch_act_split(e->stream, src, prm, 0, B, Hs, Ws, s16, x1 ? nullptr : s16 + plane_s, e->range_ctr));
            ConvUpArgs a;
            a.xhi = s16; a.xlo = s16 + plane_s; a.wup = wp; a.wup_scale = w_scale; a.bias = dbias; a.out = d->hop ? nullptr : dout;
            a.B = B; a.Cin = Cin; a.Cout = Cout; a.Hs = Hs; a.Ws = Ws; a.stat = d->hop ? nullptr : st; a.x1 = x1;
            a.emit = d->hop ? &h.em : nullptr; a.min_wg_hop = min_wg;
            DPIR_TRY(launch_conv_up(e->stream, a));
        } else {
            DPIR_TRY(launch_act_split(e->stream, src, prm, 1, B, H, W, s16, x1 ? nullptr : s16 + plane, e->range_ctr));
            Conv6Args a6;
            a6.x1 = x1; a6.xhi = s16; a6.xlo = s16 + plane; a6.w16 = wp; a6.w16_scale = w_scale; a6.bias = dbias; a6.out = d->hop ? nullptr : dout;
            a6.B = B; a6.Cin = Cin; a6.Cout = Cout; a6.H = H; a6.W = W; a6.stat = d->hop ? nullptr : st;
            a6.emit = d->hop ? &h.em : nullptr;
            Conv3Plan ran;
            DPIR_TRY(launch_conv6(e->stream, a6, &ran));
            if (!d->hop && ran.stat_kind != ST_SLOTS) return invalid("conv_up layer: launch_conv6 produced no epilogue statistics here");
        }
        if (d->hop) DPIR_TRY(launch_conv6(e->stream, second_conv6(h, B, Cout, d->Cout2, H, W, x1)));
        return Status{};
    };
    API_TRY(e, once());
    API_TRY(e, time_repeats(e->stream, d->iters, once, &d->ms_out));
    API_HIP(e, hipStreamSynchronize(e->stream));
    d->ran_out = d->route == 0 ? (d->hop ? 2 : 1) : 7;
    if (d->hop) {
        API_HIP(e, hipMemcpy(d->out2, h.dout2, h.no2 * 4, hipMemcpyDeviceToHost));
        return DPIR_OK;
    }
    API_HIP(e, hipMemcpy(d->out, dout, no * 4, hipMemcpyDeviceToHost));
    if (d->stat_out) API_TRY(e, fold_slots(st, (size_t)B * Cout, slots, d->stat_out));
    return DPIR_OK;
}

int dpir_debug_route_log(dpir_engine* e, dpir_debug_route_rec* recs, int cap, int* n_out) {
    if (!e || !n_out || (cap > 0 && !recs)) return DPIR_ERR_INVALID;
    *n_out = (int)e->route_log.size();
    for (int i = 0; i < *n_out && i < cap; ++i) {
        const RouteRec& r = e->route_log[i];
        snprintf(recs[i].layer, sizeof recs[i].layer, "%s", r.layer.c_str());
        recs[i].kernel = r.kernel; recs[i].ks = r.ks; recs[i].ksplit = r.ksplit; recs[i].hop = r.hop; recs[i].stat_kind = r.stat_kind;
        recs[i].workgroups = r.workgroups;
    }
    return DPIR_OK;
}

static ConvKnobs knobs_of(const dpir_debug_conv_knobs* k) {
    ConvKnobs o;
    if (!k) return o;
    o.conv8 = k->conv8 != 0; o.conv9 = k->conv9 != 0; o.conv9_min_wg = k->conv9_min_wg; o.conv11 = k->conv11 != 0; o.conv_up = k->conv_up != 0;
    o.split_below = k->split_below; o.split_target = k->split_target; o.fuse_small = k->fuse_small != 0; o.fuse_h1 = k->fuse_h1 != 0;
    o.emit_skip = k->emit_skip;
    return o;
}
static dpir_debug_conv_plan plan_out(const Conv3Plan& p) {
    dpir_debug_conv_plan o;
    o.kernel = p.kernel; o.hop = p.hop; o.geo = p.geo; o.ksplit = p.ksplit; o.chunks_per_split = p.chunks_per_split;
    o.stat_kind = p.stat_kind; o.stat_slots = p.stat_slots; o.refused = p.refusal != nullptr; o.workgroups = p.workgroups;
    return o;
}
void dpir_debug_conv_knobs_default(dpir_debug_conv_knobs* k) {
    const ConvKnobs d;
    *k = dpir_debug_conv_knobs{d.conv8, d.conv9, d.conv9_min_wg, d.conv11, d.conv_up, d.split_below, d.split_target, d.fuse_small, d.fuse_h1, d.emit_skip};
}
int dpir_debug_conv3_plan(const dpir_debug_conv3_query* qs, int n, const dpir_debug_conv_knobs* knobs, int cap7, int cap11, int cap_up, dpir_debug_conv_plan* out) {
    if (!qs || !out || n < 0) return DPIR_ERR_INVALID;
    const ConvKnobs k = knobs_of(knobs);
    const DeviceCaps caps{cap7, cap11, cap_up};
    for (int i = 0; i < n; ++i) {
        const dpir_debug_conv3_query& d = qs[i];
        Conv3Query q;
        q.B = d.B; q.Cin = d.Cin; q.Cout = d.Cout; q.H = d.H; q.W = d.W; q.precision = d.precision; q.grad = d.grad != 0;
        q.w16 = d.w16 != 0; q.w8 = d.w8 != 0; q.w11 = d.w11 != 0; q.conv8_source = d.conv8_source != 0;
        q.slab = d.slab_floats > 0; q.slab_floats = (size_t)d.slab_floats; q.defer = d.defer != 0; q.hop = d.hop != 0; q.has_res = d.has_res != 0;
        q.stat_slots = q.stat_plane = d.stats != 0; q.force_kernel = d.force_kernel;
        out[i] = plan_out(plan_conv3(q, k, caps));
    }
    return DPIR_OK;
}
int dpir_debug_resblock_plan(const dpir_debug_resblock_query* d, const dpir_debug_conv_knobs* knobs, int cap7, int cap11, int cap_up, dpir_debug_resblock_plan_out* out) {
    if (!d || !out) return DPIR_ERR_INVALID;
    ResblockQuery q;
    q.B = d->B; q.Cin = d->Cin; q.Cout = d->Cout; q.H = d->H; q.W = d->W; q.mode = d->mode; q.concat = d->concat != 0; q.has_skip = d->Cin != d->Cout;
    q.gn1_c = d->Cin; q.gn2_c = d->Cout; q.precision = d->precision; q.grad = d->grad != 0;
    q.hop_allowed = d->hop_allowed != 0; q.arena_words_left = (size_t)d->arena_words_left;
    const bool f16 = d->precision != 0;
    q.conv1_w16 = q.conv2_w16 = f16; q.skip_w16 = f16 && q.has_skip;
    q.conv1_w11 = d->precision == 1 && conv11_supported(d->Cin, d->Cout, 8, 32); q.conv2_w11 = d->precision == 1 && conv11_supported(d->Cout, d->Cout, 8, 32);
    q.conv1_wup = f16 && d->mode == 1 && d->Cin % 16 == 0 && d->Cout % 32 == 0;
    const int Ho = d->mode == 1 ? d->H * 2 : (d->mode == 2 ? d->H / 2 : d->H), Wo = d->mode == 1 ? d->W * 2 : (d->mode == 2 ? d->W / 2 : d->W);
    q.small_prologue = gn_act_small_supported(d->Cin, d->H, d->W, 0); q.conv5_ok = conv5_supported(d->B, d->Cout, Ho, Wo);
    q.slab = d->slab_floats > 0; q.slab_floats = (size_t)d->slab_floats;
    const ResblockPlan rp = plan_resblock(q, knobs_of(knobs), DeviceCaps{cap7, cap11, cap_up});
    out->up = rp.up; out->skip_emit = rp.skip_emit; out->hop = rp.hop; out->arena_counters = rp.arena_counters;
    out->conv1 = plan_out(rp.conv1); out->conv2 = plan_out(rp.conv2);
    return DPIR_OK;
}

int dpir_debug_conv7_emit_supported(dpir_engine* e, int B, int Cout, int H, int W, int* capacity_out) {
    if (!e) return 0;
    (void)hipSetDevice(e->device);
    if (capacity_out) *capacity_out = device_caps().conv7;
    return conv7_emit_supported(B, Cout, H, W) ? 1 : 0;
}

}
```

### diffpir_amd/csrc/engine.h

```cpp
#pragma once
#include <functional>
#include "common.h"
#include "elem.h"
#include "prox.h"

namespace dpir {

struct DevBuf {
    void* p = nullptr;
    size_t bytes = 0;
};

struct Workspace {
    std::map<std::string, DevBuf> bufs;
    size_t total = 0;
    bool frozen = false;
    uint64_t generation = 0;
    Status get(const std::string& name, size_t bytes, void** out);
    template <class T> Status getT(const std::string& name, size_t count, T** out) {
        void* p = nullptr;
        DPIR_TRY(get(name, count * sizeof(T), &p));
        *out = reinterpret_cast<T*>(p);
        return Status{};
    }
    void release();
};

struct ConvW { float* w = nullptr; float* bias = nullptr; int cin = 0, cout = 0, coutp = 0, ks = 3;
               void* w16 = nullptr; float w16_scale = 1.f;
               float* wT = nullptr; int coutpT = 0;
               void* w8 = nullptr; float w8_scale = 1.f;
               void* w16T = nullptr; float w16T_scale = 1.f;
               void* wup = nullptr; float wup_scale = 1.f;
               void* w11 = nullptr; };
struct GnW { float* gamma = nullptr; float* beta = nullptr; int c = 0; };
struct ResW {
    std::string name;
    int cin = 0, cout = 0, mode = 0;
    GnW gn1; ConvW conv1; GnW gn2; ConvW conv2;
    bool has_skip = false; ConvW skip;
    int film_off = 0;
};
struct AttnW { std::string name; int c = 0; GnW norm; ConvW qkv; ConvW proj; };
struct Layer { int kind; int idx; std::string name; };
typedef std::vector<Layer> Block;

struct UNet {
    bool loaded = false;
    dpir_unet_desc desc{};
    std::vector<float> cm;
    std::vector<Block> in_blocks, out_blocks;
    Block mid;
    ConvW conv_in;
    std::vector<ResW> res;
    std::vector<AttnW> attn;
    GnW out_gn; ConvW out_conv;
    float *te_w0 = nullptr, *te_b0 = nullptr, *te_w2 = nullptr, *te_b2 = nullptr, *label_emb = nullptr, *freqs = nullptr;
    float *film_w = nullptr, *film_b = nullptr;
    int film_rows = 0;
    std::vector<void*> allocs;
};

struct TapInfo { const float* p; size_t numel; };
struct RouteRec { std::string layer; int kernel, ks, ksplit, hop, stat_kind; long long workgroups; };

struct TapeRes { int idx; CatSrc in; int inH, inW, Ho, Wo; float* h1; float* sk; float* out; float4* prm1; float2* st1; float4* prm2; float2* st2; };
struct TapeAttn { int idx; const float* in; int H, W; float* qkv; float* att; float* out; float4* prm; float2* st; };
struct TapeNode { int kind; int idx; };
struct Tape {
    bool valid = false;
    unsigned long long serial = 0;
    int B = 0, H = 0, W = 0;
    float* conv_in_out = nullptr;
    std::vector<TapeNode> nodes; std::vector<TapeRes> res; std::vector<TapeAttn> attn;
    const float* final_h = nullptr; float4* final_prm = nullptr; float2* final_st = nullptr;
    void clear() { valid = false; nodes.clear(); res.clear(); attn.clear(); }
};

struct LpipsState;
struct FidState;

struct ResizerTab { int in_len = 0, out_len = 0, taps = 0; float* w = nullptr; int* idx = nullptr; };

}

struct dpir_prox { dpir::ProxState st; };

struct dpir_engine {
    int device = 0;
    hipStream_t stream = nullptr;
    std::string last_error;
    dpir::Profiler prof;
    dpir::UNet net;
    dpir::Workspace ws;
    std::map<std::string, dpir::TapInfo> taps;
    std::vector<dpir::RouteRec> route_log;
    dpir::ProxCache prox_cache;
    std::map<std::pair<int, int>, dpir::ResizerTab> resizers;
    std::vector<void*> user_allocs;
    bool collect_taps = true;
    int precision = 0;
    bool grad_enabled = false;
    dpir::Tape tape;
    float ps_c1 = 0.f, ps_c2 = 0.f; int ps_B = 0, ps_H = 0, ps_W = 0; const float* ps_x0 = nullptr;
    unsigned long long fwd_serial = 0, ps_serial = 0;
    struct GraphKey {
        int32_t task, B, H, W, sf, in_iter, generate_mode, kind;
        int32_t host_n1, host_n2, host_rp, has_labels;
        float gamma, guidance;
        int32_t loop, loop_pad;
        int32_t per_image, image_index;
        uint64_t ws_generation;
    };
    struct GraphEntry { GraphKey key; hipGraphExec_t exec = nullptr; uint64_t last_use = 0; };
    std::vector<GraphEntry> graphs;
    uint64_t graph_clock = 0;
    static constexpr size_t kMaxGraphs = 16;
    dpir::ProxState loop_prox;
    void invalidate_graphs() {
        for (auto& g : graphs) if (g.exec) (void)hipGraphExecDestroy(g.exec);
        graphs.clear();
    }
    unsigned long long* range_ctr = nullptr;
    int prox_mode = 1; int cus = 256;
    bool fuse_h1_off = false;
    int fwd_since_sync = 0;
    std::function<int()> replay_last;
    unsigned long long replay_serial = 0;
    unsigned long long enqueue_serial() const { return prof.serial + copy_serial; }
    unsigned long long copy_serial = 0;
    void arm_replay(std::function<int()> fn) { ++fwd_since_sync; replay_last = std::move(fn); replay_serial = enqueue_serial(); }
    struct Progress {
        bool armed = false;
        std::vector<int> panel_of; int n_panels = 0;
        float* strip_f32 = nullptr; uint8_t* strip_u8 = nullptr; float* masked_f32 = nullptr; uint8_t* masked_u8 = nullptr; float* minmax = nullptr;
    } progress;
    float* progress_premix = nullptr; size_t progress_premix_bytes = 0;
    dpir::LpipsState* lpips = nullptr;
    bool lpips_keep_taps = false;
    dpir::FidState* fid = nullptr;
    bool fid_keep_taps = false;
    void* comm = nullptr; int comm_world = 1, comm_rank = 0;

    dpir::Status resizer(int in_len, int sf, dpir::ResizerTab* out);
};

namespace dpir {
Status unet_load(dpir_engine* e, const dpir_unet_desc* desc, const dpir_tensor* weights, int n);
void unet_free(dpir_engine* e);
Status unet_forward(dpir_engine* e, const float* x, const int* t_dev, const int* y_dev, float* out, int B, int H, int W,
                    const float* film_table = nullptr, const StepDev* film_step = nullptr, bool uniform_t = false);
Status unet_film_table(dpir_engine* e, const int* t_dev, int n_steps, float* table);
Status unet_backward(dpir_engine* e, const float* gout, float* dx);
double unet_flops(const UNet& net, int H, int W, int cls = -1);
Status comm_allreduce_sum_f64(dpir_engine* e, double* dev, size_t n);
}
```

### diffpir_amd/csrc/unet.hip

```cpp
#include "engine.h"
#include "conv6_params.h"
#include "conv9.h"
#include "conv11.h"
#include "conv_up.h"
#include <unordered_map>
#include <cstdint>
#include <math.h>
#include <string.h>
#include <stdlib.h>

namespace dpir {

Status Workspace::get(const std::string& name, size_t bytes, void** out) {
    auto it = bufs.find(name);
    if (it != bufs.end() && it->second.bytes >= bytes) { *out = it->second.p; return Status{}; }
    if (frozen) return Status{DPIR_ERR_STATE, "workspace allocation of '" + name + "' during graph capture"};
    if (it != bufs.end()) { (void)hipFree(it->second.p); total -= it->second.bytes; bufs.erase(it); }
    void* p = nullptr;
    size_t rb = (bytes + 255) & ~(size_t)255;
    hipError_t err = hipMalloc(&p, rb);
    if (err != hipSuccess) return Status{DPIR_ERR_NOMEM, "hipMalloc(" + std::to_string(rb) + ") for '" + name + "' failed"};
    bufs[name] = DevBuf{p, rb};
    total += rb;
    ++generation;
    *out = p;
    return Status{};
}
void Workspace::release() {
    for (auto& kv : bufs) (void)hipFree(kv.second.p);
    bufs.clear();
    total = 0;
}

namespace {
struct WeightMap {
    std::map<std::string, const dpir_tensor*> m;
    Status find(const std::string& key, std::vector<int64_t> shape, const float** out) const {
        auto it = m.find(key);
        if (it == m.end()) return invalid("state-dict key missing: " + key);
        const dpir_tensor* t = it->second;
        if (t->ndim != (int)shape.size()) return invalid("state-dict key " + key + ": wrong rank");
        for (size_t i = 0; i < shape.size(); ++i)
            if (t->shape[i] != shape[i]) return invalid("state-dict key " + key + ": wrong shape");
        if (!t->data) return invalid("state-dict key " + key + ": null data");
        *out = t->data;
        return Status{};
    }
};

Status upload(dpir_engine* e, const float* host, size_t n, float** dev) {
    void* p = nullptr;
    if (hipMalloc(&p, n * sizeof(float)) != hipSuccess) return Status{DPIR_ERR_NOMEM, "hipMalloc for weights failed"};
    e->net.allocs.push_back(p);
    DPIR_HIP(hipMemcpy(p, host, n * sizeof(float), hipMemcpyHostToDevice));
    *dev = reinterpret_cast<float*>(p);
    return Status{};
}
Status upload16(dpir_engine* e, const std::vector<uint16_t>& pack, const char* what, void** dev) {
    void* p = nullptr;
    if (hipMalloc(&p, pack.size() * 2) != hipSuccess) return Status{DPIR_ERR_NOMEM, std::string("hipMalloc for ") + what + " failed"};
    e->net.allocs.push_back(p);
    DPIR_HIP(hipMemcpy(p, pack.data(), pack.size() * 2, hipMemcpyHostToDevice));
    *dev = p;
    return Status{};
}

Status load_conv(dpir_engine* e, const WeightMap& wm, const std::string& p, int cin, int cout, int ks, bool one_d, ConvW* out, bool up_pack = false) {
    const float *w = nullptr, *b = nullptr;
    std::vector<int64_t> shape = one_d ? std::vector<int64_t>{cout, cin, 1} : std::vector<int64_t>{cout, cin, ks, ks};
    DPIR_TRY(wm.find(p + ".weight", shape, &w));
    DPIR_TRY(wm.find(p + ".bias", {cout}, &b));
    int taps = ks * ks;
    int coutp = round_up(cout, 64);
    int cinp = round_up(cin, 16);
    std::vector<float> packed((size_t)cinp * taps * coutp, 0.f);
    for (int co = 0; co < cout; ++co)
        for (int ci = 0; ci < cin; ++ci)
            for (int t = 0; t < taps; ++t)
                packed[((size_t)ci * taps + t) * coutp + co] = w[((size_t)co * cin + ci) * taps + t];
    out->cin = cin; out->cout = cout; out->coutp = coutp; out->ks = ks;
    DPIR_TRY(upload(e, packed.data(), packed.size(), &out->w));
    DPIR_TRY(upload(e, b, cout, &out->bias));
    if (e->grad_enabled) {
        const int cinT = round_up(cout, 16), coutT = round_up(cin, 64);
        std::vector<float> pt((size_t)cinT * taps * coutT, 0.f);
        for (int co = 0; co < cout; ++co)
            for (int ci = 0; ci < cin; ++ci)
                for (int t = 0; t < taps; ++t)
                    pt[((size_t)co * taps + t) * coutT + ci] = w[((size_t)co * cin + ci) * taps + (taps - 1 - t)];
        out->coutpT = coutT;
        DPIR_TRY(upload(e, pt.data(), pt.size(), &out->wT));
        if (e->precision >= 1 && (ks == 3 || ks == 1)) {
            std::vector<float> wt((size_t)cin * cout * taps);
            for (int co = 0; co < cout; ++co)
                for (int ci = 0; ci < cin; ++ci)
                    for (int t = 0; t < taps; ++t)
                        wt[((size_t)ci * cout + co) * taps + t] = w[((size_t)co * cin + ci) * taps + (taps - 1 - t)];
            std::vector<uint16_t> w16t;
            out->w16T_scale = ks == 3 ? pack_weights_conv6(wt.data(), cin, cout, w16t) : pack_weights_f16x3_1x1(wt.data(), cin, cout, w16t);
            DPIR_TRY(upload16(e, w16t, "the split dgrad weights", &out->w16T));
        }
    }
    if (e->precision >= 1 && (ks == 3 || ks == 1)) {
        std::vector<uint16_t> w16;
        out->w16_scale = ks == 3 ? pack_weights_conv6(w, cout, cin, w16) : pack_weights_f16x3_1x1(w, cout, cin, w16);
        DPIR_TRY(upload16(e, w16, "split weights", &out->w16));
        if (ks == 3 && !one_d && cout <= 16 && cin % 32 == 0) {
            std::vector<uint16_t> w8;
            out->w8_scale = pack_weights_conv8(w, cout, cin, w8);
            DPIR_TRY(upload16(e, w8, "the conv8 weights", &out->w8));
        }
        if (e->precision == 1 && ks == 3 && !one_d && conv11_supported(cin, cout, 8, 32)) {
            std::vector<uint16_t> w11;
            pack_weights_conv11(w, cout, cin, out->w16_scale, w11);
            DPIR_TRY(upload16(e, w11, "the conv11 weights", &out->w11));
        }
        if (up_pack && ks == 3 && !one_d && cin % 16 == 0 && cout % 32 == 0) {
            std::vector<uint16_t> wu;
            out->wup_scale = pack_weights_conv_up(w, cout, cin, wu);
            DPIR_TRY(upload16(e, wu, "the phase weights", &out->wup));
        }
    }
    return Status{};
}
Status load_gn(dpir_engine* e, const WeightMap& wm, const std::string& p, int c, GnW* out) {
    const float *g = nullptr, *b = nullptr;
    if (c % 32) return invalid("GroupNorm32 channels not divisible by 32 at " + p);
    DPIR_TRY(wm.find(p + ".weight", {c}, &g));
    DPIR_TRY(wm.find(p + ".bias", {c}, &b));
    out->c = c;
    DPIR_TRY(upload(e, g, c, &out->gamma));
    DPIR_TRY(upload(e, b, c, &out->beta));
    return Status{};
}
}

void unet_free(dpir_engine* e) {
    for (void* p : e->net.allocs) (void)hipFree(p);
    e->net = UNet{};
}

Status unet_load(dpir_engine* e, const dpir_unet_desc* d, const dpir_tensor* weights, int n) {
    unet_free(e);
    UNet& net = e->net;
    net.desc = *d;
    if (d->in_channels != 3) return invalid("in_channels must be 3");
    if (d->model_channels <= 0 || d->model_channels % 32) return invalid("model_channels must be a positive multiple of 32");
    if (d->num_head_channels != 64) return Status{DPIR_ERR_UNSUPPORTED, "only num_head_channels=64 is supported"};
    if (d->n_channel_mult > 8 || d->n_attention_ds > 8) return invalid("too many channel_mult / attention_ds entries");
    if (d->n_channel_mult > 0) net.cm.assign(d->channel_mult, d->channel_mult + d->n_channel_mult);
    else if (d->image_size == 512) net.cm = {0.5f, 1, 1, 2, 2, 4, 4};
    else if (d->image_size == 256) net.cm = {1, 1, 2, 2, 4, 4};
    else if (d->image_size == 128) net.cm = {1, 1, 2, 3, 4};
    else if (d->image_size == 64) net.cm = {1, 2, 3, 4};
    else return invalid("unsupported image_size for default channel_mult");
    WeightMap wm;
    for (int i = 0; i < n; ++i) wm.m[weights[i].name] = &weights[i];

    const int mc = d->model_channels, ted = 4 * mc;
    auto has_attn = [&](int ds) { for (int i = 0; i < d->n_attention_ds; ++i) if (d->attention_ds[i] == ds) return true; return false; };
    int film_rows = 0;
    std::vector<std::pair<std::string, int>> film_parts;

    auto add_res = [&](const std::string& p, int cin, int cout, int mode, Block& blk) -> Status {
        ResW r; r.name = p; r.cin = cin; r.cout = cout; r.mode = mode;
        DPIR_TRY(load_gn(e, wm, p + ".in_layers.0", cin, &r.gn1));
        DPIR_TRY(load_conv(e, wm, p + ".in_layers.2", cin, cout, 3, false, &r.conv1, mode == 1));
        DPIR_TRY(load_gn(e, wm, p + ".out_layers.0", cout, &r.gn2));
        DPIR_TRY(load_conv(e, wm, p + ".out_layers.3", cout, cout, 3, false, &r.conv2));
        r.has_skip = cin != cout;
        if (r.has_skip) {
            if (mode != 0) return invalid("resampling ResBlock with channel change is not part of this architecture");
            DPIR_TRY(load_conv(e, wm, p + ".skip_connection", cin, cout, 1, false, &r.skip));
        }
        r.film_off = film_rows;
        film_rows += 2 * cout;
        film_parts.push_back({p + ".emb_layers.1", cout});
        blk.push_back(Layer{1, (int)net.res.size(), p});
        net.res.push_back(r);
        return Status{};
    };
    auto add_attn = [&](const std::string& p, int c, Block& blk) -> Status {
        AttnW a; a.name = p; a.c = c;
        if (c % 64) return invalid("attention channels not divisible by 64");
        DPIR_TRY(load_gn(e, wm, p + ".norm", c, &a.norm));
        DPIR_TRY(load_conv(e, wm, p + ".qkv", c, 3 * c, 1, true, &a.qkv));
        DPIR_TRY(load_conv(e, wm, p + ".proj_out", c, c, 1, true, &a.proj));
        blk.push_back(Layer{2, (int)net.attn.size(), p});
        net.attn.push_back(a);
        return Status{};
    };

    int ch = (int)(net.cm[0] * mc);
    const int input_ch = ch;
    {
        Block b0;
        DPIR_TRY(load_conv(e, wm, "input_blocks.0.0", 3, ch, 3, false, &net.conv_in));
        b0.push_back(Layer{0, 0, "input_blocks.0.0"});
        net.in_blocks.push_back(b0);
    }
    std::vector<int> chans{ch};
    int ds = 1;
    const int nlev = (int)net.cm.size();
    for (int level = 0; level < nlev; ++level) {
        for (int k = 0; k < d->num_res_blocks; ++k) {
            Block blk;
            std::string p = "input_blocks." + std::to_string(net.in_blocks.size());
            int cout = (int)(net.cm[level] * mc);
            DPIR_TRY(add_res(p + ".0", ch, cout, 0, blk));
            ch = cout;
            if (has_attn(ds)) DPIR_TRY(add_attn(p + ".1", ch, blk));
            net.in_blocks.push_back(blk);
            chans.push_back(ch);
        }
        if (level != nlev - 1) {
            Block blk;
            std::string p = "input_blocks." + std::to_string(net.in_blocks.size());
            DPIR_TRY(add_res(p + ".0", ch, ch, 2, blk));
            net.in_blocks.push_back(blk);
            chans.push_back(ch);
            ds *= 2;
        }
    }
    DPIR_TRY(add_res("middle_block.0", ch, ch, 0, net.mid));
    DPIR_TRY(add_attn("middle_block.1", ch, net.mid));
    DPIR_TRY(add_res("middle_block.2", ch, ch, 0, net.mid));
    for (int level = nlev - 1; level >= 0; --level) {
        for (int i = 0; i <= d->num_res_blocks; ++i) {
            Block blk;
            std::string p = "output_blocks." + std::to_string(net.out_blocks.size());
            int ich = chans.back(); chans.pop_back();
            int cout = (int)(mc * net.cm[level]);
            int j = 0;
            DPIR_TRY(add_res(p + "." + std::to_string(j++), ch + ich, cout, 0, blk));
            ch = cout;
            if (has_attn(ds)) DPIR_TRY(add_attn(p + "." + std::to_string(j++), ch, blk));
            if (level && i == d->num_res_blocks) {
                DPIR_TRY(add_res(p + "." + std::to_string(j++), ch, ch, 1, blk));
                ds /= 2;
            }
            net.out_blocks.push_back(blk);
        }
    }
    DPIR_TRY(load_gn(e, wm, "out.0", ch, &net.out_gn));
    DPIR_TRY(load_conv(e, wm, "out.2", input_ch, d->out_channels, 3, false, &net.out_conv));
    if (ch != input_ch) return invalid("final channel count mismatch");

    const float* p0 = nullptr;
    DPIR_TRY(wm.find("time_embed.0.weight", {ted, mc}, &p0)); DPIR_TRY(upload(e, p0, (size_t)ted * mc, &net.te_w0));
    DPIR_TRY(wm.find("time_embed.0.bias", {ted}, &p0)); DPIR_TRY(upload(e, p0, ted, &net.te_b0));
    DPIR_TRY(wm.find("time_embed.2.weight", {ted, ted}, &p0)); DPIR_TRY(upload(e, p0, (size_t)ted * ted, &net.te_w2));
    DPIR_TRY(wm.find("time_embed.2.bias", {ted}, &p0)); DPIR_TRY(upload(e, p0, ted, &net.te_b2));
    if (d->num_classes > 0) {
        DPIR_TRY(wm.find("label_emb.weight", {d->num_classes, ted}, &p0));
        DPIR_TRY(upload(e, p0, (size_t)d->num_classes * ted, &net.label_emb));
    }
    {
        std::vector<float> fw((size_t)film_rows * ted), fb(film_rows);
        size_t row = 0;
        for (auto& fp : film_parts) {
            const float *w = nullptr, *b = nullptr;
            DPIR_TRY(wm.find(fp.first + ".weight", {2 * fp.second, ted}, &w));
            DPIR_TRY(wm.find(fp.first + ".bias", {2 * fp.second}, &b));
            memcpy(&fw[row * ted], w, (size_t)2 * fp.second * ted * sizeof(float));
            memcpy(&fb[row], b, (size_t)2 * fp.second * sizeof(float));
            row += 2 * fp.second;
        }
        DPIR_TRY(upload(e, fw.data(), fw.size(), &net.film_w));
        DPIR_TRY(upload(e, fb.data(), fb.size(), &net.film_b));
        net.film_rows = film_rows;
    }
    {
        int half = mc / 2;
        std::vector<float> fr(half);
        for (int i = 0; i < half; ++i) {
            float arg = -(float)log(10000.0) * (float)i / (float)half;
            fr[i] = (float)exp((double)arg);
        }
        DPIR_TRY(upload(e, fr.data(), half, &net.freqs));
    }
    net.loaded = true;
    return Status{};
}

namespace {
struct Act {
    const float* a = nullptr; int ca = 0;
    const float* b = nullptr; int cb = 0;
    int H = 0, W = 0;
    int C() const { return ca + cb; }
};

struct Fwd {
    dpir_engine* e;
    hipStream_t s;
    Workspace& ws;
    int B;
    const float* film;
    int film_rows;
    int film_stride;
    const StepDev* fstep;
    float* partial;
    size_t partial_cap;
    const ConvKnobs& knobs = ConvKnobs::from_env();
    DeviceCaps caps;
    struct FusedStat { const float2* slots; int nslots; const double2* part; };
    std::unordered_map<const float*, FusedStat> fused;
    PendingConv pending;
    bool grad = false;
    bool x1() const { return e->precision == 2; }

    std::string layer;
    int pending_rec = -1;
    void log(int kernel, int ks, const Conv3Plan& p, int hop) {
        if (!e->collect_taps) return;
        if (p.stat_kind == ST_PENDING) pending_rec = (int)e->route_log.size();
        e->route_log.push_back(RouteRec{layer, kernel, ks, p.ksplit, hop, p.stat_kind, p.workgroups});
    }

    Status resolve() {
        if (!pending.partial) return Status{};
        ProfScope ps(&e->prof, PC_CONV3);
        DPIR_TRY(launch_conv6_resolve(s, pending));
        if (pending.stat_plane) fused[pending.out] = FusedStat{nullptr, 0, pending.stat_plane};
        else fused.erase(pending.out);
        if (e->collect_taps && pending_rec >= 0) {
            RouteRec r = e->route_log[pending_rec];
            e->route_log[pending_rec].stat_kind = pending.stat_plane ? ST_PLANE : ST_NONE;
            r.kernel = CK_RESOLVE; r.hop = HOP_NONE; r.stat_kind = e->route_log[pending_rec].stat_kind; r.workgroups = ((long long)pending.B * pending.Cout + 3) / 4;
            e->route_log.push_back(r);
        }
        pending = PendingConv{}; pending_rec = -1;
        return Status{};
    }
    bool is_pending(const float* p) const { return pending.partial && p && p == pending.out; }

    Conv3Query query(const ConvW& cw, int Cin, int Ho, int Wo, bool hop, bool has_res) const {
        Conv3Query q;
        q.B = B; q.Cin = Cin; q.Cout = cw.cout; q.H = Ho; q.W = Wo; q.precision = e->precision; q.grad = grad;
        q.w16 = cw.ks == 3 && cw.w16; q.w8 = cw.ks == 3 && cw.w8; q.w11 = cw.ks == 3 && cw.w11;
        q.hop = hop; q.has_res = has_res;
        q.slab = !hop; q.slab_floats = hop ? 0 : partial_cap; q.defer = knobs.fuse_small;
        return q;
    }

    Status small_prologue(const GnW& g, const std::string& tag, int film_off, const Act& in, int mode, const float* res, char* s16, size_t plane,
                          float4** prm_out = nullptr, float2** stats_out = nullptr) {
        if (pending.partial && !is_pending(in.a)) DPIR_TRY(resolve());
        if (is_pending(res)) return invalid("gn_conv: residual is an unfinished convolution");
        GnActArgs ga;
        ga.src = CatSrc{in.a, in.ca, in.b, in.cb};
        ga.pend = pending;
        ga.gamma = g.gamma; ga.beta = g.beta;
        ga.film = film_off >= 0 ? film : nullptr; ga.film_stride = film_stride; ga.film_off = film_off < 0 ? 0 : film_off;
        ga.fstep = fstep; ga.frows = film_rows;
        ga.silu = true; ga.mode = mode; ga.B = B; ga.Hs = in.H; ga.Ws = in.W;
        ga.hi = s16; ga.lo = x1() ? nullptr : s16 + plane; ga.range_ctr = e->range_ctr;
        if (grad) {
            DPIR_TRY(ws.getT(tag + "#prm", (size_t)B * in.C(), &ga.prm_out));
            DPIR_TRY(ws.getT(tag + "#gst", (size_t)B * 32, &ga.stats_out));
            if (prm_out) *prm_out = ga.prm_out;
            if (stats_out) *stats_out = ga.stats_out;
        }
        {
            ProfScope ps(&e->prof, PC_ELEM);
            DPIR_TRY(launch_gn_act_small(s, ga));
        }
        if (pending.partial) { fused.erase(pending.out); pending = PendingConv{}; pending_rec = -1; }
        return Status{};
    }

    Status gn_conv(const GnW& g, const std::string& tag, int film_off, const ConvW& cw, const Act& in, int mode,
                   const float* res, int res_mode, float* out, int Ho, int Wo, float4** prm_out = nullptr, float2** stats_out = nullptr,
                   const Conv6Emit* emit = nullptr) {
        const int C = in.C();
        const bool planes = cw.ks == 3 && plan_conv3(query(cw, C, Ho, Wo, emit != nullptr, res != nullptr), knobs, caps).kernel != CK_FP32;
        if (knobs.fuse_small && planes && C == g.c && C % 16 == 0 && gn_act_small_supported(C, in.H, in.W, mode)) {
            int eh = mode == 1 ? Ho / 2 : (mode == 2 ? Ho * 2 : Ho), ew = mode == 1 ? Wo / 2 : (mode == 2 ? Wo * 2 : Wo);
            if (eh != in.H || ew != in.W) return invalid("conv: source resolution does not match mode");
            const int C8 = 2 * ((C + 15) / 16);
            const size_t plane = (size_t)B * C8 * Ho * Wo * 16;
            char* s16 = nullptr;
            DPIR_TRY(ws.getT("act#s16", 2 * plane, &s16));
            DPIR_TRY(small_prologue(g, tag, film_off, in, mode, res, s16, plane, prm_out, stats_out));
            return conv6_on_planes(cw, s16, plane, res, res_mode, out, Ho, Wo, emit);
        }
        DPIR_TRY(resolve());
        float4* prm = nullptr;
        DPIR_TRY(gn(g, in, tag, film_off, true, &prm, stats_out));
        if (prm_out) *prm_out = prm;
        return conv(cw, in, mode, prm, res, res_mode, out, Ho, Wo, emit);
    }

    Status conv6_on_planes(const ConvW& cw, char* s16, size_t plane, const float* res, int res_mode, float* out, int Ho, int Wo,
                           const Conv6Emit* emit = nullptr) {
        const int slots = geometry(Ho, Wo).stat_slots;
        float2* st = nullptr; double2* sp = nullptr;
        if (slots > 0 && cw.cout % 32 == 0) {
            const std::string key = std::to_string(reinterpret_cast<uintptr_t>(out));
            DPIR_TRY(ws.getT("st#" + key, (size_t)B * cw.cout * slots, &st));
            DPIR_TRY(ws.getT("sp#" + key, (size_t)B * cw.cout, &sp));
        }
        if (emit) { st = nullptr; sp = nullptr; }
        Conv3Query q = query(cw, cw.cin, Ho, Wo, emit != nullptr, res != nullptr);
        q.w8 = false;
        q.stat_slots = st != nullptr; q.stat_plane = sp != nullptr;
        Conv3Plan p = plan_conv3(q, knobs, caps);
        if (p.refusal) return invalid(p.refusal);
        ProfScope ps(&e->prof, PC_CONV3);
        if (p.kernel == CK_CONV9) {
            Conv9Args a9;
            a9.xhi = s16; a9.xlo = s16 + plane; a9.w16 = cw.w16; a9.w16_scale = cw.w16_scale; a9.bias = cw.bias; a9.out = out;
            a9.res = res; a9.res_mode = res_mode; a9.B = B; a9.Cin = cw.cin; a9.Cout = cw.cout; a9.H = Ho; a9.W = Wo;
            a9.stat_plane = sp; a9.x1 = x1(); a9.emit = emit;
            DPIR_TRY(launch_conv9(s, a9));
        } else if (p.kernel == CK_CONV11) {
            Conv11Args a11;
            a11.xhi = s16; a11.xlo = s16 + plane; a11.w11 = cw.w11; a11.w_scale = cw.w16_scale; a11.bias = cw.bias; a11.out = out;
            a11.res = res; a11.res_mode = res_mode; a11.B = B; a11.Cin = cw.cin; a11.Cout = cw.cout; a11.H = Ho; a11.W = Wo;
            a11.stat = st; a11.precision = e->precision; a11.grad = grad; a11.emit = emit;
            DPIR_TRY(launch_conv11(s, a11));
        } else {
            Conv6Args a6;
            a6.x1 = x1();
            a6.xhi = s16; a6.xlo = s16 + plane; a6.w16 = cw.w16; a6.w16_scale = cw.w16_scale;
            a6.bias = cw.bias; a6.out = out; a6.res = res; a6.res_mode = res_mode;
            a6.B = B; a6.Cin = cw.cin; a6.Cout = cw.cout; a6.H = Ho; a6.W = Wo;
            if (q.slab) { a6.partial = partial; a6.partial_capacity = partial_cap; }
            a6.stat = st; a6.stat_plane = sp; a6.emit = emit;
            PendingConv pc;
            DPIR_TRY(launch_conv6(s, a6, &p, q.defer ? &pc : nullptr));
            if (p.stat_kind == ST_PENDING) pending = pc;
        }
        if (p.stat_kind == ST_SLOTS) fused[out] = FusedStat{st, p.stat_slots, nullptr};
        else if (p.stat_kind == ST_PLANE) fused[out] = FusedStat{nullptr, 0, sp};
        else fused.erase(out);
        log(p.kernel, 3, p, !p.hop ? HOP_NONE : (p.kernel == CK_CONV9 ? HOP_CONV9 : HOP_ARENA));
        return Status{};
    }

    Status conv(const ConvW& cw, const Act& in, int mode, const float4* prm, const float* res, int res_mode, float* out, int Ho, int Wo,
                const Conv6Emit* emit = nullptr) {
        const bool use5 = cw.w16 && cw.ks == 1 && mode == 0 && (!res || res_mode == 0) && !(prm && in.C() % 16) &&
                          (conv5_supported(B, cw.cout, Ho, Wo, prm != nullptr) ||
                           conv5_small_supported(B, in.ca, in.b ? in.cb : 0, cw.cout, Ho, Wo, prm != nullptr));
        if (pending.partial && (is_pending(in.a) || is_pending(in.b) || is_pending(res) || !use5)) DPIR_TRY(resolve());
        Conv3Plan p;
        if (cw.ks == 3) {
            Conv3Query q = query(cw, in.C(), Ho, Wo, emit != nullptr, res != nullptr);
            q.conv8_source = prm && mode == 0 && !in.b && in.H == Ho && in.W == Wo;
            p = plan_conv3(q, knobs, caps);
            if (p.refusal) return invalid(p.refusal);
        } else if (emit) {
            return invalid("conv: fused emission was requested for a launch that is not on the f16 3x3 path");
        }
        if (p.kernel == CK_CONV8) {
            Conv8Args a8;
            a8.x = in.a; a8.prm = prm; a8.w = cw.w8; a8.w_scale = cw.w8_scale; a8.bias = cw.bias; a8.out = out;
            a8.B = B; a8.C = in.C(); a8.Cout = cw.cout; a8.H = Ho; a8.W = Wo; a8.range_ctr = e->range_ctr; a8.x1 = x1();
            fused.erase(out);
            log(CK_CONV8, 3, p, HOP_NONE);
            ProfScope ps(&e->prof, PC_CONV3);
            return launch_conv8(s, a8);
        }
        if (p.kernel != CK_FP32) {
            int eh = mode == 1 ? Ho / 2 : (mode == 2 ? Ho * 2 : Ho), ew = mode == 1 ? Wo / 2 : (mode == 2 ? Wo * 2 : Wo);
            if (eh != in.H || ew != in.W) return invalid("conv: source resolution does not match mode");
            const int C = in.C(), C8 = 2 * ((C + 15) / 16);
            const size_t plane = (size_t)B * C8 * Ho * Wo * 16;
            if (plane >= ((size_t)1 << 32)) return invalid("conv: split activation plane exceeds the 4 GiB buffer-descriptor range; reduce the batch");
            char* s16 = nullptr;
            DPIR_TRY(ws.getT("act#s16", 2 * plane, &s16));
            {
                ProfScope ps(&e->prof, PC_ELEM);
                DPIR_TRY(launch_act_split(s, CatSrc{in.a, in.ca, in.b, in.cb}, prm, mode, B, Ho, Wo, s16, x1() ? nullptr : s16 + plane, e->range_ctr));
            }
            return conv6_on_planes(cw, s16, plane, res, res_mode, out, Ho, Wo, emit);
        }
        fused.erase(out);
        log(use5 ? CK_CONV5 : CK_FP32, cw.ks, Conv3Plan{}, HOP_NONE);
        if (use5) {
            Conv5Args a5;
            a5.src = CatSrc{in.a, in.ca, in.b, in.cb}; a5.prm = prm; a5.w16 = cw.w16; a5.w16_scale = cw.w16_scale;
            a5.bias = cw.bias; a5.out = out; a5.res = res; a5.B = B; a5.Cout = cw.cout; a5.H = Ho; a5.W = Wo;
            a5.range_ctr = e->range_ctr; a5.x1 = x1();
            ProfScope ps(&e->prof, PC_CONV1);
            return launch_conv5(s, a5);
        }
        ConvArgs a;
        a.src.a = in.a; a.src.ca = in.ca; a.src.b = in.b; a.src.cb = in.cb; a.src.Hs = in.H; a.src.Ws = in.W;
        a.src.mode = mode; a.src.prm = prm;
        a.w = cw.w; a.bias = cw.bias; a.out = out; a.res = res; a.res_mode = res_mode;
        a.B = B; a.Cin = cw.cin; a.Cout = cw.cout; a.CoutP = cw.coutp; a.H = Ho; a.W = Wo; a.ks = cw.ks;
        a.partial = partial; a.partial_capacity = partial_cap;
        ProfScope ps(&e->prof, cw.ks == 3 ? PC_CONV3 : PC_CONV1);
        return launch_conv(s, a);
    }
    Status gn(const GnW& g, const Act& in, const std::string& tag, int film_off, bool silu, float4** prm_out, float2** stats_out = nullptr) {
        float4* prm = nullptr;
        float2* gst = nullptr;
        if (grad) DPIR_TRY(ws.getT(tag + "#gst", (size_t)B * 32, &gst));
        if (is_pending(in.a) || is_pending(in.b)) DPIR_TRY(resolve());
        DPIR_TRY(ws.getT(tag + "#prm", (size_t)B * g.c, &prm));
        GnStatSrc src[2];
        const float* tp[2] = {in.a, in.b};
        const int tc[2] = {in.ca, in.cb};
        for (int k = 0; k < 2; ++k) {
            src[k].c = tc[k];
            if (!tp[k] || tc[k] == 0) { src[k].c = 0; continue; }
            auto it = fused.find(tp[k]);
            if (it != fused.end()) { src[k].slots = it->second.slots; src[k].nslots = it->second.nslots; src[k].part = it->second.part; continue; }
            double2* part = nullptr;
            DPIR_TRY(ws.getT(tag + "#stats" + std::to_string(k), (size_t)B * tc[k], &part));
            ProfScope ps(&e->prof, PC_GN);
            DPIR_TRY(launch_gn_stats(s, CatSrc{tp[k], tc[k], nullptr, 0}, B, in.H * in.W, part));
            src[k].part = part;
        }
        ProfScope ps(&e->prof, PC_ELEM);
        DPIR_TRY(launch_gn_prm(s, src[0], src[1], in.H * in.W, g.gamma, g.beta, film_off >= 0 ? film : nullptr, film_stride, film_off < 0 ? 0 : film_off, B, g.c, silu, prm, fstep, film_rows, gst));
        *prm_out = prm;
        if (stats_out) *stats_out = gst;
        return Status{};
    }
    void tap(const std::string& name, const float* p, size_t numel) {
        if (e->collect_taps) e->taps[name] = TapInfo{p, numel};
    }

    bool fuse_h1 = true;
    long long* fuse_arena = nullptr; size_t fuse_cap = 0, fuse_off = 0;
    Status make_emit(const ResW& r, int Ho, int Wo, int counters, Conv6Emit* em, char** s16b, size_t* plane2) {
        const int C8 = 2 * ((r.cout + 15) / 16);
        *plane2 = (size_t)B * C8 * Ho * Wo * 16;
        DPIR_TRY(ws.getT("act#s16b", 2 * *plane2, s16b));
        em->hi = *s16b; em->lo = x1() ? nullptr : *s16b + *plane2; em->C8 = C8;
        em->gamma = r.gn2.gamma; em->beta = r.gn2.beta;
        em->film = r.film_off >= 0 ? film : nullptr; em->film_stride = film_stride; em->film_off = r.film_off < 0 ? 0 : r.film_off;
        em->frows = film_rows; em->fstep = fstep;
        em->range_ctr = e->range_ctr;
        if (counters <= 0) return Status{};
        em->acc = fuse_arena + fuse_off;
        fuse_off += (size_t)B * 64;
        em->cnt = reinterpret_cast<unsigned*>(fuse_arena + fuse_off);
        fuse_off += ((size_t)B * counters + 1) / 2;
        static const int spin_env = getenv("DPIR_FUSE_SPIN_LIMIT") ? atoi(getenv("DPIR_FUSE_SPIN_LIMIT")) : 0;
        static const int extra_env = getenv("DPIR_FUSE_EXPECT_EXTRA") ? atoi(getenv("DPIR_FUSE_EXPECT_EXTRA")) : 0;
        static const int sleep_env = getenv("DPIR_FUSE_SLEEP") ? atoi(getenv("DPIR_FUSE_SLEEP")) : 5;
        em->sleep_sel = sleep_env;
        if (spin_env > 0) em->spin_limit = spin_env;
        em->expect_extra = extra_env;
        return Status{};
    }

    Status resblock_up(const ResW& r, const ResblockPlan& rp, const Act& in, Act* out, int Ho, int Wo, float* h1, size_t on) {
        const int C = in.C(), C8 = 2 * (C / 16);
        const size_t plane = (size_t)B * C8 * in.H * in.W * 16;
        char* s16 = nullptr;
        DPIR_TRY(ws.getT("act#s16", 2 * plane, &s16));
        if (knobs.fuse_small && gn_act_small_supported(C, in.H, in.W, 0)) {
            DPIR_TRY(small_prologue(r.gn1, r.name + "#gn1", -1, in, 0, nullptr, s16, plane));
        } else {
            DPIR_TRY(resolve());
            float4* prm = nullptr;
            DPIR_TRY(gn(r.gn1, in, r.name + "#gn1", -1, true, &prm));
            ProfScope ps(&e->prof, PC_ELEM);
            DPIR_TRY(launch_act_split(s, CatSrc{in.a, in.ca, nullptr, 0}, prm, 0, B, in.H, in.W, s16, x1() ? nullptr : s16 + plane, e->range_ctr));
        }
        ConvUpArgs a;
        a.xhi = s16; a.xlo = s16 + plane; a.wup = r.conv1.wup; a.wup_scale = r.conv1.wup_scale; a.bias = r.conv1.bias;
        a.B = B; a.Cin = C; a.Cout = r.cout; a.Hs = in.H; a.Ws = in.W; a.x1 = x1();
        float* o = nullptr;
        DPIR_TRY(ws.getT(r.name + "#out", on, &o));
        Conv6Emit em; char* s16b = nullptr; size_t plane2 = 0;
        float2* st = nullptr;
        if (rp.hop) {
            DPIR_TRY(make_emit(r, Ho, Wo, rp.arena_counters, &em, &s16b, &plane2));
            a.emit = &em; a.min_wg_hop = kHopMinWg;
        } else {
            DPIR_TRY(ws.getT("st#" + std::to_string(reinterpret_cast<uintptr_t>(h1)), (size_t)B * r.cout * rp.conv1.stat_slots, &st));
            a.out = h1; a.stat = st;
        }
        {
            ProfScope ps(&e->prof, PC_CONV3);
            DPIR_TRY(launch_conv_up(s, a));
        }
        layer = r.name + "#conv1";
        log(CK_CONV_UP, 3, rp.conv1, rp.hop);
        layer = r.name + "#conv2";
        if (rp.hop) {
            DPIR_TRY(conv6_on_planes(r.conv2, s16b, plane2, in.a, 1, o, Ho, Wo));
        } else {
            fused[h1] = FusedStat{st, rp.conv1.stat_slots, nullptr};
            tap(r.name + "#h1", h1, on);
            Act h1a; h1a.a = h1; h1a.ca = r.cout; h1a.H = Ho; h1a.W = Wo;
            DPIR_TRY(gn_conv(r.gn2, r.name + "#gn2", r.film_off, r.conv2, h1a, 0, in.a, 1, o, Ho, Wo));
        }
        tap(r.name, o, on);
        out->a = o; out->ca = r.cout; out->b = nullptr; out->cb = 0; out->H = Ho; out->W = Wo;
        return Status{};
    }

    Status resblock(const ResW& r, const Act& in, Act* out) {
        if (in.C() != r.cin) return invalid("resblock " + r.name + ": input channels mismatch");
        int Ho = r.mode == 1 ? in.H * 2 : (r.mode == 2 ? in.H / 2 : in.H);
        int Wo = r.mode == 1 ? in.W * 2 : (r.mode == 2 ? in.W / 2 : in.W);
        if (r.mode == 2 && ((in.H | in.W) & 1)) return invalid("resblock " + r.name + ": odd size cannot be average-pooled");
        size_t on = (size_t)B * r.cout * Ho * Wo;
        float* h1 = nullptr;
        DPIR_TRY(ws.getT(r.name + "#h1", on, &h1));
        const int Cin = in.C();
        ResblockQuery rq;
        rq.B = B; rq.Cin = Cin; rq.Cout = r.cout; rq.H = in.H; rq.W = in.W; rq.mode = r.mode; rq.concat = in.b != nullptr; rq.has_skip = r.has_skip;
        rq.gn1_c = r.gn1.c; rq.gn2_c = r.gn2.c; rq.precision = e->precision; rq.grad = grad;
        rq.hop_allowed = fuse_h1; rq.arena_words_left = fuse_arena ? fuse_cap - fuse_off : 0;
        rq.conv1_w16 = r.conv1.w16; rq.conv1_w11 = r.conv1.w11; rq.conv1_wup = r.conv1.wup; rq.conv2_w16 = r.conv2.w16; rq.conv2_w11 = r.conv2.w11;
        rq.skip_w16 = r.has_skip && r.skip.w16;
        rq.small_prologue = gn_act_small_supported(Cin, in.H, in.W, 0); rq.conv5_ok = conv5_supported(B, r.cout, Ho, Wo);
        rq.slab = true; rq.slab_floats = partial_cap;
        const ResblockPlan rp = plan_resblock(rq, knobs, caps);
        if (rp.up) return resblock_up(r, rp, in, out, Ho, Wo, h1, on);
        Act h1a; h1a.a = h1; h1a.ca = r.cout; h1a.H = Ho; h1a.W = Wo;
        const float* res = nullptr; int res_mode = 0;
        const bool fuse = rp.hop != HOP_NONE;
        Conv6Emit em; char* s16b = nullptr; size_t plane2 = 0;
        float* o = nullptr;
        if (rp.skip_emit) {
            const size_t eplane = (size_t)B * (2 * ((Cin + 15) / 16)) * Ho * Wo * 16;
            float4* prm1 = nullptr;
            TapeRes tr{};
            DPIR_TRY(resolve());
            DPIR_TRY(gn(r.gn1, in, r.name + "#gn1", -1, true, &prm1, &tr.st1));
            tr.prm1 = prm1;
            char* s16 = nullptr;
            DPIR_TRY(ws.getT("act#s16", 2 * eplane, &s16));
            float* sk = nullptr;
            DPIR_TRY(ws.getT(r.name + "#skip", on, &sk));
            Conv5Args a5;
            a5.src = CatSrc{in.a, in.ca, in.b, in.cb}; a5.prm = nullptr; a5.w16 = r.skip.w16; a5.w16_scale = r.skip.w16_scale;
            a5.bias = r.skip.bias; a5.out = sk; a5.res = nullptr; a5.B = B; a5.Cout = r.cout; a5.H = Ho; a5.W = Wo;
            a5.range_ctr = e->range_ctr; a5.x1 = x1();
            a5.emit_prm = prm1; a5.emit_hi = s16; a5.emit_lo = x1() ? nullptr : s16 + eplane;
            fused.erase(sk);
            layer = r.name + "#skip";
            log(CK_CONV5, 1, Conv3Plan{}, HOP_NONE);
            {
                ProfScope ps(&e->prof, PC_CONV1);
                DPIR_TRY(launch_conv5(s, a5));
            }
            DPIR_TRY(ws.getT(r.name + "#out", on, &o));
            layer = r.name + "#conv1";
            if (fuse) {
                DPIR_TRY(make_emit(r, Ho, Wo, rp.arena_counters, &em, &s16b, &plane2));
                DPIR_TRY(conv6_on_planes(r.conv1, s16, eplane, nullptr, 0, nullptr, Ho, Wo, &em));
                layer = r.name + "#conv2";
                DPIR_TRY(conv6_on_planes(r.conv2, s16b, plane2, sk, 0, o, Ho, Wo));
            } else {
                DPIR_TRY(conv6_on_planes(r.conv1, s16, eplane, nullptr, 0, h1, Ho, Wo));
                tap(r.name + "#h1", h1, on);
                layer = r.name + "#conv2";
                DPIR_TRY(gn_conv(r.gn2, r.name + "#gn2", r.film_off, r.conv2, h1a, 0, sk, 0, o, Ho, Wo, &tr.prm2, &tr.st2));
            }
            tap(r.name, o, on);
            if (grad) {
                tr.idx = (int)(&r - e->net.res.data());
                tr.in = CatSrc{in.a, in.ca, in.b, in.cb}; tr.inH = in.H; tr.inW = in.W; tr.Ho = Ho; tr.Wo = Wo; tr.h1 = h1; tr.sk = sk; tr.out = o;
                e->tape.nodes.push_back(TapeNode{1, (int)e->tape.res.size()});
                e->tape.res.push_back(tr);
            }
            out->a = o; out->ca = r.cout; out->b = nullptr; out->cb = 0; out->H = Ho; out->W = Wo;
            return Status{};
        }
        TapeRes tr{};
        float* sk = nullptr;
        if (r.has_skip) DPIR_TRY(ws.getT(r.name + "#skip", on, &sk));
        if (fuse) DPIR_TRY(make_emit(r, Ho, Wo, rp.arena_counters, &em, &s16b, &plane2));
        layer = r.name + "#conv1";
        DPIR_TRY(gn_conv(r.gn1, r.name + "#gn1", -1, r.conv1, in, r.mode, nullptr, 0, fuse ? nullptr : h1, Ho, Wo, &tr.prm1, &tr.st1, fuse ? &em : nullptr));
        if (!fuse) tap(r.name + "#h1", h1, on);
        if (r.has_skip) {
            layer = r.name + "#skip";
            DPIR_TRY(conv(r.skip, in, 0, nullptr, nullptr, 0, sk, Ho, Wo));
            res = sk;
            tr.sk = sk;
        } else {
            if (in.b) return invalid("resblock " + r.name + ": identity skip on a concatenated input");
            res = in.a; res_mode = r.mode;
        }
        DPIR_TRY(ws.getT(r.name + "#out", on, &o));
        layer = r.name + "#conv2";
        if (fuse) DPIR_TRY(conv6_on_planes(r.conv2, s16b, plane2, res, res_mode, o, Ho, Wo));
        else DPIR_TRY(gn_conv(r.gn2, r.name + "#gn2", r.film_off, r.conv2, h1a, 0, res, res_mode, o, Ho, Wo, &tr.prm2, &tr.st2));
        tap(r.name, o, on);
        if (grad) {
            tr.idx = (int)(&r - e->net.res.data());
            tr.in = CatSrc{in.a, in.ca, in.b, in.cb}; tr.inH = in.H; tr.inW = in.W; tr.Ho = Ho; tr.Wo = Wo; tr.h1 = h1; tr.out = o;
            e->tape.nodes.push_back(TapeNode{1, (int)e->tape.res.size()});
            e->tape.res.push_back(tr);
        }
        out->a = o; out->ca = r.cout; out->b = nullptr; out->cb = 0; out->H = Ho; out->W = Wo;
        return Status{};
    }

    Status attention(const AttnW& aw, const Act& in, Act* out) {
        if (in.b || in.ca != aw.c) return invalid("attention " + aw.name + ": bad input");
        int T = in.H * in.W;
        float4* prm = nullptr;
        float2* gst = nullptr;
        DPIR_TRY(resolve());
        DPIR_TRY(gn(aw.norm, in, aw.name + "#norm", -1, false, &prm, &gst));
        float *qkv = nullptr, *att = nullptr, *o = nullptr;
        DPIR_TRY(ws.getT(aw.name + "#qkv", (size_t)B * 3 * aw.c * T, &qkv));
        DPIR_TRY(ws.getT(aw.name + "#att", (size_t)B * aw.c * T, &att));
        DPIR_TRY(ws.getT(aw.name + "#out", (size_t)B * aw.c * T, &o));
        layer = aw.name + "#qkv";
        DPIR_TRY(conv(aw.qkv, in, 0, prm, nullptr, 0, qkv, in.H, in.W));
        {
            ProfScope ps(&e->prof, PC_ATTN);
            DPIR_TRY(launch_attention(s, qkv, att, B, aw.c, T, 64));
        }
        Act aa; aa.a = att; aa.ca = aw.c; aa.H = in.H; aa.W = in.W;
        layer = aw.name + "#proj";
        DPIR_TRY(conv(aw.proj, aa, 0, nullptr, in.a, 0, o, in.H, in.W));
        tap(aw.name + "#qkv", qkv, (size_t)B * 3 * aw.c * T);
        tap(aw.name + "#att", att, (size_t)B * aw.c * T);
        tap(aw.name, o, (size_t)B * aw.c * T);
        if (grad) {
            e->tape.nodes.push_back(TapeNode{2, (int)e->tape.attn.size()});
            e->tape.attn.push_back(TapeAttn{(int)(&aw - e->net.attn.data()), in.a, in.H, in.W, qkv, att, o, prm, gst});
        }
        out->a = o; out->ca = aw.c; out->b = nullptr; out->cb = 0; out->H = in.H; out->W = in.W;
        return Status{};
    }

    Status run_block(const UNet& net, const Block& blk, Act in, Act* out) {
        Act cur = in;
        for (const Layer& l : blk) {
            Act nxt;
            if (l.kind == 1) DPIR_TRY(resblock(net.res[l.idx], cur, &nxt));
            else if (l.kind == 2) DPIR_TRY(attention(net.attn[l.idx], cur, &nxt));
            else return invalid("unexpected layer kind");
            cur = nxt;
        }
        *out = cur;
        return Status{};
    }
};
}

Status unet_film_table(dpir_engine* e, const int* t_dev, int n_steps, float* table) {
    UNet& net = e->net;
    if (!net.loaded) return Status{DPIR_ERR_STATE, "dpir_load_unet has not been called"};
    if (net.desc.num_classes > 0) return invalid("FiLM hoisting needs a class-unconditional model");
    const int mc = net.desc.model_channels, ted = 4 * mc;
    float *tmp = nullptr, *semb = nullptr;
    DPIR_TRY(e->ws.getT("embS#tmp", (size_t)n_steps * (mc + ted), &tmp));
    DPIR_TRY(e->ws.getT("embS#semb", (size_t)n_steps * ted, &semb));
    ProfScope ps(&e->prof, PC_ELEM);
    DPIR_TRY(launch_time_embed(e->stream, t_dev, nullptr, net.freqs, net.te_w0, net.te_b0, net.te_w2, net.te_b2, nullptr, n_steps, mc, tmp, semb));
    DPIR_TRY(launch_rows_gemv(e->stream, net.film_w, net.film_b, semb, n_steps, net.film_rows, ted, table));
    return Status{};
}

Status unet_forward(dpir_engine* e, const float* x, const int* t_dev, const int* y_dev, float* out, int B, int H, int W,
                    const float* film_table, const StepDev* film_step, bool uniform_t) {
    UNet& net = e->net;
    if (!net.loaded) return Status{DPIR_ERR_STATE, "dpir_load_unet has not been called"};
    if ((net.desc.num_classes > 0) != (y_dev != nullptr))
        return invalid("must specify y if and only if the model is class-conditional");
    if (B <= 0 || H <= 0 || W <= 0) return invalid("bad batch / image size");
    Workspace& ws = e->ws;
    hipStream_t s = e->stream;
    ProfScope whole(&e->prof, PC_UNET);
    const int mc = net.desc.model_channels, ted = 4 * mc;
    float *tmp = nullptr, *semb = nullptr, *film = nullptr;
    const bool hoisted = film_table != nullptr && film_step != nullptr;
    static const bool one_row_env = !(getenv("DPIR_UNIFORM_T") && atoi(getenv("DPIR_UNIFORM_T")) == 0);
    const bool one_row = one_row_env && !hoisted && uniform_t && net.desc.num_classes == 0 && y_dev == nullptr;
    if (hoisted && net.desc.num_classes > 0) return invalid("hoisted FiLM table with a class-conditional model");
    if (!hoisted) {
        DPIR_TRY(ws.getT("emb#tmp", (size_t)B * (mc + ted), &tmp));
        DPIR_TRY(ws.getT("emb#semb", (size_t)B * ted, &semb));
        DPIR_TRY(ws.getT("emb#film", (size_t)B * net.film_rows, &film));
        ProfScope ps(&e->prof, PC_ELEM);
        const int Be = one_row ? 1 : B;
        DPIR_TRY(launch_time_embed(s, t_dev, y_dev, net.freqs, net.te_w0, net.te_b0, net.te_w2, net.te_b2, net.label_emb, Be, mc, tmp, semb));
        DPIR_TRY(launch_rows_gemv(s, net.film_w, net.film_b, semb, Be, net.film_rows, ted, film));
    }
    float* partial = nullptr;
    size_t partial_cap = (size_t)16 * 1024 * 1024;
    DPIR_TRY(ws.getT("conv#partial", partial_cap, &partial));
    Fwd f{e, s, ws, B, hoisted ? film_table : film, net.film_rows, (hoisted || one_row) ? 0 : net.film_rows, hoisted ? film_step : nullptr, partial, partial_cap};
    {
        f.grad = e->grad_enabled;
        f.caps = device_caps();
        f.fuse_h1 = f.knobs.fuse_h1 && !e->fuse_h1_off && !f.grad && e->precision != 0;
        if (f.fuse_h1) {
            f.fuse_cap = (size_t)B * 4096;
            DPIR_TRY(ws.getT("fuse#arena", f.fuse_cap, &f.fuse_arena));
            DPIR_HIP(hipMemsetAsync(f.fuse_arena, 0, f.fuse_cap * sizeof(long long), s));
        }
        ++e->fwd_serial;
        if (f.grad) { e->tape.clear(); e->tape.serial = e->fwd_serial; e->tape.B = B; e->tape.H = H; e->tape.W = W; }
    }
    if (e->collect_taps) { e->taps.clear(); e->route_log.clear(); }

    std::vector<Act> hs;
    Act h;
    {
        float* o = nullptr;
        size_t on = (size_t)B * net.conv_in.cout * H * W;
        DPIR_TRY(ws.getT("input_blocks.0.0#out", on, &o));
        Act xin; xin.a = x; xin.ca = 3; xin.H = H; xin.W = W;
        f.layer = "input_blocks.0.0";
        DPIR_TRY(f.conv(net.conv_in, xin, 0, nullptr, nullptr, 0, o, H, W));
        f.tap("input_blocks.0.0", o, on);
        h.a = o; h.ca = net.conv_in.cout; h.H = H; h.W = W;
        hs.push_back(h);
        if (f.grad) e->tape.conv_in_out = o;
    }
    for (size_t i = 1; i < net.in_blocks.size(); ++i) {
        Act o;
        DPIR_TRY(f.run_block(net, net.in_blocks[i], h, &o));
        h = o;
        hs.push_back(h);
    }
    {
        Act o;
        DPIR_TRY(f.run_block(net, net.mid, h, &o));
        h = o;
    }
    for (size_t i = 0; i < net.out_blocks.size(); ++i) {
        Act skip = hs.back(); hs.pop_back();
        if (skip.H != h.H || skip.W != h.W) return invalid("skip connection size mismatch (image size not divisible by the UNet stride)");
        Act cat; cat.a = h.a; cat.ca = h.ca; cat.b = skip.a; cat.cb = skip.ca; cat.H = h.H; cat.W = h.W;
        Act o;
        DPIR_TRY(f.run_block(net, net.out_blocks[i], cat, &o));
        h = o;
    }
    float4* fprm = nullptr; float2* fst = nullptr;
    f.layer = "out";
    DPIR_TRY(f.gn_conv(net.out_gn, "out#gn", -1, net.out_conv, h, 0, nullptr, 0, out, H, W, &fprm, &fst));
    DPIR_TRY(f.resolve());
    if (f.grad) { e->tape.final_h = h.a; e->tape.final_prm = fprm; e->tape.final_st = fst; e->tape.valid = true; }
    f.tap("out", out, (size_t)B * net.desc.out_channels * H * W);
    return Status{};
}

double unet_flops(const UNet& net, int H, int W, int cls) {
    if (!net.loaded) return 0.0;
    const double mc = net.desc.model_channels, ted = 4 * mc;
    double f3 = 0, f1 = 0, fa = 0, fl = 2 * (mc * ted + ted * ted);
    double h = H, w = W;
    auto res = [&](const ResW& r) {
        if (r.mode == 1) { h *= 2; w *= 2; } else if (r.mode == 2) { h /= 2; w /= 2; }
        f3 += 2.0 * 9 * r.cin * r.cout * h * w + 2.0 * 9 * r.cout * r.cout * h * w;
        fl += 2.0 * ted * 2 * r.cout;
        if (r.has_skip) f1 += 2.0 * r.cin * r.cout * h * w;
    };
    auto att = [&](const AttnW& a) {
        double T = h * w, c = a.c;
        f1 += 2 * c * 3 * c * T + 2 * c * c * T;
        fa += 2 * 2 * T * T * c;
    };
    auto blk = [&](const Block& b) {
        for (const Layer& l : b) {
            if (l.kind == 0) f3 += 2.0 * 9 * 3 * net.conv_in.cout * h * w;
            else if (l.kind == 1) res(net.res[l.idx]);
            else att(net.attn[l.idx]);
        }
    };
    for (auto& b : net.in_blocks) blk(b);
    blk(net.mid);
    for (auto& b : net.out_blocks) blk(b);
    f3 += 2.0 * 9 * net.out_conv.cin * net.out_conv.cout * H * W;
    if (cls == PC_CONV3) return f3;
    if (cls == PC_CONV1) return f1;
    if (cls == PC_ATTN) return fa;
    if (cls == PC_ELEM) return fl;
    return f3 + f1 + fa + fl;
}

}
```

### include/diffpir_debug.h

```cpp
#ifndef DIFFPIR_DEBUG_H
#define DIFFPIR_DEBUG_H
#include "diffpir_engine.h"
#ifdef __cplusplus
extern "C" {
#endif
int dpir_debug_conv_bench(dpir_engine* e, int B, int Cin, int Cout, int H, int W, int ks, int mode, int with_prm,
                          int dbg, int iters, double* ms_out);
int dpir_debug_victim(dpir_engine* e, int lds_bytes, int threads, int blocks, long long spin_ticks, int iters, unsigned long long* bad_out);
int dpir_debug_victim_alu(dpir_engine* e, int mode, int blocks, int iters_in_kernel, int launches, unsigned long long* bad_out);
int dpir_debug_victim_fft_pk(dpir_engine* e, int blocks, int iters_in_kernel, int launches, unsigned long long* bad_out);
int dpir_debug_victim_fft_nopk(dpir_engine* e, int blocks, int iters_in_kernel, int launches, unsigned long long* bad_out);
int dpir_debug_conv7_check(dpir_engine* e, int B, int Cin, int Cout, int H, int W, int res_mode, int x1, int split, int scaled, int iters,
                           double* ms6_out, double* ms7_out, unsigned long long* mismatches_out, float* maxdiff_out, int* ksplit_out);
int dpir_debug_conv7_emit_supported(dpir_engine* e, int B, int Cout, int H, int W, int* capacity_out);
int dpir_debug_conv5_layer(dpir_engine* e, int B, int ca, int cb, int Cout, int H, int W, int tile, const float* xa, const float* xb,
                           const float* w, const float* bias, const float* prm, const float* res, float* out, int* path_out);
typedef struct dpir_debug_conv3_desc {
    int32_t B, ca, cb, Cout, H, W, mode, res_mode, scaled, prologue, route, split, defer, Cout2;
    const float *xa, *xb, *w, *bias, *res, *prm, *gamma, *beta, *film, *gamma2, *beta2, *w2, *bias2;
    float* out; double* stat_out; float* out2;
    int32_t stat_kind_out, path_out, ksplit_out, reserved;
} dpir_debug_conv3_desc;
int dpir_debug_conv3_layer(dpir_engine* e, dpir_debug_conv3_desc* d);
typedef struct dpir_debug_conv9_desc {
    int32_t B, Cin, Cout, H, W, res_mode, hop, Cout2;
    const float *x, *w, *bias, *res, *prm, *gamma2, *beta2, *film2, *w2, *bias2;
    float* out; double* stat_out; float* out2;
    int32_t ran_out, iters;
    double ms_out;
} dpir_debug_conv9_desc;
int dpir_debug_conv9_layer(dpir_engine* e, dpir_debug_conv9_desc* d);
typedef struct dpir_debug_conv11_desc {
    int32_t B, Cin, Cout, H, W, res_mode, route, ksplit, hop, Cout2;
    const float *x, *w, *bias, *res, *prm, *gamma2, *beta2, *film2, *w2, *bias2;
    float* out; double* stat_out; float* out2;
    int32_t ran_out, iters;
    double ms_out;
} dpir_debug_conv11_desc;
int dpir_debug_conv11_layer(dpir_engine* e, dpir_debug_conv11_desc* d);
typedef struct dpir_debug_conv_up_desc {
    int32_t B, Cin, Cout, Hs, Ws, hop, force_hop, Cout2, route, reserved;
    const float *x, *w, *bias, *res, *prm, *gamma2, *beta2, *film2, *w2, *bias2;
    float* out; double* stat_out; float* out2;
    int32_t ran_out, iters;
    double ms_out;
} dpir_debug_conv_up_desc;
int dpir_debug_conv_up_layer(dpir_engine* e, dpir_debug_conv_up_desc* d);
typedef struct dpir_debug_route_rec {
    char layer[80];
    int32_t kernel, ks, ksplit, hop, stat_kind, reserved;
    long long workgroups;
} dpir_debug_route_rec;
int dpir_debug_route_log(dpir_engine* e, dpir_debug_route_rec* recs, int cap, int* n_out);
typedef struct dpir_debug_conv_knobs {
    int32_t conv8, conv9, conv9_min_wg, conv11, conv_up, split_below, split_target, fuse_small, fuse_h1, emit_skip;
} dpir_debug_conv_knobs;
void dpir_debug_conv_knobs_default(dpir_debug_conv_knobs* k);
typedef struct dpir_debug_conv3_query {
    int32_t B, Cin, Cout, H, W, precision, grad, w16, w8, w11, conv8_source, defer, hop, has_res, stats, force_kernel;
    long long slab_floats;
} dpir_debug_conv3_query;
typedef struct dpir_debug_conv_plan {
    int32_t kernel, hop, geo, ksplit, chunks_per_split, stat_kind, stat_slots, refused;
    long long workgroups;
} dpir_debug_conv_plan;
int dpir_debug_conv3_plan(const dpir_debug_conv3_query* q, int n, const dpir_debug_conv_knobs* knobs, int cap7, int cap11, int cap_up,
                          dpir_debug_conv_plan* out);
typedef struct dpir_debug_resblock_query {
    int32_t B, Cin, Cout, H, W, mode, concat, precision, grad, hop_allowed;
    long long arena_words_left, slab_floats;
} dpir_debug_resblock_query;
typedef struct dpir_debug_resblock_plan_out {
    int32_t up, skip_emit, hop, arena_counters;
    dpir_debug_conv_plan conv1, conv2;
} dpir_debug_resblock_plan_out;
int dpir_debug_resblock_plan(const dpir_debug_resblock_query* q, const dpir_debug_conv_knobs* knobs, int cap7, int cap11, int cap_up,
                             dpir_debug_resblock_plan_out* out);
typedef struct dpir_debug_attention_desc {
    int32_t B, C, T, head_ch;
    const float *qkv, *dAtt;
    float *out, *dqkv;
    uint64_t guard_bad_out;
} dpir_debug_attention_desc;
int dpir_debug_attention(dpir_engine* e, dpir_debug_attention_desc* d);
typedef struct dpir_debug_groupnorm_desc {
    int32_t B, ca, cb, Hs, Ws, mode, silu, acc_a, acc_b, reserved;
    const float *xa, *xb, *gamma, *beta, *film, *dA, *ga_init, *gb_init, *extra;
    float *prm_out, *stats_out, *ga_out, *gb_out;
    int32_t ns_out, reserved2;
    uint64_t guard_bad_out;
} dpir_debug_groupnorm_desc;
int dpir_debug_groupnorm(dpir_engine* e, dpir_debug_groupnorm_desc* d);
#ifdef __cplusplus
}
#endif
#endif
```

Measured before the change: 9.654 images/s.

## Fuse conv_in stem with block-1 GroupNorm stats and operand-plane emission

Adds a dedicated stem kernel for the 3-channel input convolution. A separate stats kernel computes GroupNorm statistics for the conv output analytically, using a Gram-matrix approach over the input. The stem then writes both the fp32 output and the GN+SiLU-applied hi/lo f16 operand planes that block 1's conv1 consumes. This is meant to remove the generic conv_in launch, a separate GN stats pass and the act_split pass over the full-resolution activation, at the cost of new kernel complexity and planning conditions.

```diff
diff --git a/diffpir_amd/_lib.py b/diffpir_amd/_lib.py
--- a/diffpir_amd/_lib.py
+++ b/diffpir_amd/_lib.py
@@ -93,6 +93,12 @@
     _fields_ = ([(n, C.c_int32) for n in ("B", "Cin", "Cout", "Hs", "Ws", "hop", "force_hop", "Cout2", "route", "reserved")] +
                 [(n, C.c_void_p) for n in ("x", "w", "bias", "res", "prm", "gamma2", "beta2", "film2", "w2", "bias2", "out", "stat_out", "out2")] +
                 [(n, C.c_int32) for n in ("ran_out", "iters")] + [("ms_out", C.c_double)])
+
+
+class StemDesc(C.Structure):
+    _fields_ = ([(n, C.c_int32) for n in ("B", "Cout", "H", "W", "route", "emit", "iters", "ran_out")] +
+                [(n, C.c_void_p) for n in ("x", "w", "bias", "gamma", "beta", "out", "stat_out", "prm_out", "hi_out", "lo_out")] +
+                [("ms_out", C.c_double)])
 
 
 class RouteRec(C.Structure):
@@ -274,7 +280,9 @@
     d.dpir_debug_conv11_layer.restype = C.c_int
     d.dpir_debug_conv_up_layer.argtypes = [C.c_void_p, C.POINTER(ConvUpDesc)]
     d.dpir_debug_conv_up_layer.restype = C.c_int
-    d.dpir_debug_route_log.argtypes = [C.c_void_p, C.POINTER(RouteRec), C.c_int, C.POINTER(C.c_int)]
+    d.dpir_debug_stem.argtypes = [C.c_void_p, C.POINTER(StemDesc)]
+    d.dpir_debug_stem.restype = C.c_int
+    d.dpir_debug_route_log.argtypes =[C.c_void_p, C.POINTER(RouteRec), C.c_int, C.POINTER(C.c_int)]
     d.dpir_debug_route_log.restype = C.c_int
     d.dpir_debug_conv_knobs_default.argtypes = [C.POINTER(ConvKnobs)]
     d.dpir_debug_conv_knobs_default.restype = None
diff --git a/diffpir_amd/csrc/conv_plan.cpp b/diffpir_amd/csrc/conv_plan.cpp
--- a/diffpir_amd/csrc/conv_plan.cpp
+++ b/diffpir_amd/csrc/conv_plan.cpp
@@ -18,6 +18,8 @@
         k.fuse_small = env_on("DPIR_FUSE_SMALL");
         k.fuse_h1 = env_on("DPIR_FUSE_H1");
         k.emit_skip = env_int("DPIR_EMIT_SKIP", k.emit_skip);
+        k.stem = env_on("DPIR_STEM");
+        k.stem_min_wg = env_int("DPIR_STEM_MIN_WG", k.stem_min_wg);
         return k;
     }();
     return knobs;
@@ -89,6 +91,13 @@
     if (geometry(H, W).geo != 0 || (W & 31) || (H & 7) || Cout <= 0 || (Cout & 127) || !group_in_wave(Cout, 64)) return false;
     const long long tiles = (long long)(W / 32) * (H / 8);
     return tiles <= capacity / 2 && tiles * (Cout / 128) * B >= kHopMinWg;
+}
+
+const char* stem_shape_refusal(int Cout, int H, int W) {
+    if (Cout <= 0 || Cout % 32) return "stem: Cout must be a multiple of 32";
+    if (H <= 0 || H % 8) return "stem: 8 x 32 tiles inside the image only (H % 8 == 0)";
+    if (W <= 0 || W % 32) return "stem: 8 x 32 tiles inside the image only (W % 32 == 0)";
+    return nullptr;
 }
 
 static Conv3Plan refuse(const char* why, int geo = -1) { Conv3Plan p; p.refusal = why; p.geo = geo; return p; }
@@ -213,4 +222,25 @@
     return rp;
 }
 
-}
+StemPlan plan_stem(const StemQuery& q, const ConvKnobs& knobs) {
+    StemPlan p;
+    auto no = [&](const char* why) { p.refusal = why; return p; };
+    if (!knobs.stem) return no("stem: switched off (DPIR_STEM=0)");
+    if (q.precision == 0) return no("stem: the f32 precision keeps the fp32 kernel");
+    if (q.grad) return no("stem: a gradient-mode forward keeps conv_in's own launch");
+    if (q.Cin != 3) return no("stem: conv_in must read 3 channels");
+    if (const char* why = stem_shape_refusal(q.Cout, q.H, q.W)) return no(why);
+    if ((long long)(q.W / 32) * (q.H / 8) * q.B < knobs.stem_min_wg) return no("stem: too few workgroups, conv_in keeps its own launches");
+    if (q.B <= 0 || (size_t)q.B * 3 * q.H * q.W * 4 >= k4GiB || (size_t)q.Cout * q.H * q.W * 4 >= k4GiB)
+        return no("stem: the input or an image's output exceeds the 4 GiB buffer-descriptor range");
+    if (!q.pack) return no("stem: the weight pack is not loaded");
+    if (!q.block1_res || q.block1_mode != 0 || q.block1_gn1_c != q.Cout) return no("stem: block 1 does not open with a plain ResBlock normalising conv_in's channels");
+    if (q.block1.up || q.block1.skip_emit) return no("stem: block 1's conv1 gets its planes from another kernel (conv5's emission)");
+    if (q.block1_small_prologue) return no("stem: block 1's conv1 takes the fused low-resolution prologue");
+    if (q.block1.conv1.kernel == CK_FP32 || q.block1.conv1.kernel == CK_CONV8 || q.block1.conv1.refusal) return no("stem: block 1's conv1 does not run on operand planes");
+    p.take = true;
+    p.workgroups = (long long)(q.W / 32) * (q.H / 8) * q.B;
+    return p;
+}
+
+}
diff --git a/diffpir_amd/csrc/conv_plan.h b/diffpir_amd/csrc/conv_plan.h
--- a/diffpir_amd/csrc/conv_plan.h
+++ b/diffpir_amd/csrc/conv_plan.h
@@ -4,6 +4,7 @@
 
 constexpr int kHopMinWg = 384;
 constexpr int kConv9MinWg = 128;
+constexpr int kStemMinWg = 1024;
 constexpr int kConv5EmitMaxC = 384;
 constexpr int kConv8MaxC = 256;
 
@@ -18,6 +19,8 @@
     bool fuse_small = true;
     bool fuse_h1 = true;
     int emit_skip = 1;
+    bool stem = true;
+    int stem_min_wg = kStemMinWg;
     static const ConvKnobs& from_env();
 };
 
@@ -43,9 +46,10 @@
 long long conv_up_workgroups(int B, int Cout, int Hs, int Ws);
 const char* conv_up_refusal(int B, int Cin, int Cout, int Hs, int Ws, bool hop, int min_wg_hop, int capacity);
 bool conv7_hop_ok(int B, int Cout, int H, int W, int capacity);
+const char* stem_shape_refusal(int Cout, int H, int W);
 
 enum ConvKernel { CK_FP32 = 0, CK_CONV5 = 5, CK_CONV6 = 6, CK_CONV7 = 7, CK_CONV8 = 8, CK_CONV9 = 9, CK_CONV11 = 11, CK_CONV_UP = 12,
-                  CK_CONV7_NARROW = 17, CK_RESOLVE = 60 };
+                  CK_STEM = 13, CK_CONV7_NARROW = 17, CK_RESOLVE = 60 };
 enum StatKind { ST_NONE = 0, ST_SLOTS = 1, ST_PLANE = 2, ST_PENDING = 3 };
 enum HopKind { HOP_NONE = 0, HOP_ARENA = 1, HOP_CONV9 = 2, HOP_CONV_UP = 3 };
 
@@ -96,4 +100,20 @@
 };
 ResblockPlan plan_resblock(const ResblockQuery& q, const ConvKnobs& knobs, const DeviceCaps& caps);
 
+struct StemQuery {
+    int B = 0, Cin = 0, Cout = 0, H = 0, W = 0;
+    int precision = 1; bool grad = false;
+    bool pack = false;
+    bool block1_res = false;
+    int block1_mode = 0, block1_gn1_c = 0;
+    ResblockPlan block1;
+    bool block1_small_prologue = false;
+};
+struct StemPlan {
+    bool take = false;
+    const char* refusal = nullptr;
+    long long workgroups = 0;
+};
+StemPlan plan_stem(const StemQuery& q, const ConvKnobs& knobs);
+
 }
diff --git a/diffpir_amd/csrc/dbg_conv.hip b/diffpir_amd/csrc/dbg_conv.hip
--- a/diffpir_amd/csrc/dbg_conv.hip
+++ b/diffpir_amd/csrc/dbg_conv.hip
@@ -3,6 +3,7 @@
 #include "conv9.h"
 #include "conv11.h"
 #include "conv_up.h"
+#include "stem.h"
 #include "../../include/diffpir_debug.h"
 #include <string.h>
 #include <vector>
@@ -788,6 +789,100 @@
     return DPIR_OK;
 }
 
+int dpir_debug_stem(dpir_engine* e, dpir_debug_stem_desc* d) {
+    if (!e || !d) return DPIR_ERR_INVALID;
+    d->ran_out = 0; d->ms_out = 0.0;
+    const int B = d->B, Cout = d->Cout, H = d->H, W = d->W;
+    if (!d->x || !d->w || !d->bias || B <= 0 || Cout <= 0 || H <= 0 || W <= 0 || d->route < 0 || d->route > 1 || (d->emit && (!d->gamma || !d->beta)))
+        return fail(e, invalid("stem: bad descriptor"));
+    if (e->grad_enabled) return fail(e, Status{DPIR_ERR_UNSUPPORTED, "stem: a gradient-mode forward keeps conv_in's own launch"});
+    if (e->precision == 0) return fail(e, Status{DPIR_ERR_UNSUPPORTED, "stem: the f32 precision keeps the fp32 kernel"});
+    if (d->route == 0) {
+        if (const char* why = stem_refusal(Cout, H, W)) return fail(e, Status{DPIR_ERR_UNSUPPORTED, why});
+    } else if (Cout % 32 || !conv6_supported(H, W)) {
+        return fail(e, Status{DPIR_ERR_UNSUPPORTED, "stem: launch_conv6's route refuses this shape"});
+    }
+    (void)hipSetDevice(e->device);
+    const bool x1 = e->precision == 2;
+    const size_t HW = (size_t)H * W, nx = (size_t)B * 3 * HW, no = (size_t)B * Cout * HW;
+    const int C8 = Cout / 8;
+    const size_t plane = (size_t)B * C8 * HW * 16, xplane = (size_t)B * 2 * HW * 16;
+    const int slots = conv6_stat_slots(H, W);
+    const size_t nst = (size_t)B * Cout * (slots > 0 ? slots : 1);
+    float *dx = nullptr, *dw = nullptr, *dbias = nullptr, *dg = nullptr, *db = nullptr, *dout = nullptr; float4* dprm = nullptr; float2* st = nullptr;
+    double2* sp = nullptr; double* gram = nullptr; char *s16 = nullptr, *xs16 = nullptr;
+    API_TRY(e, e->ws.getT("stem#x", nx, &dx));
+    API_TRY(e, e->ws.getT("stem#w", (size_t)Cout * 27, &dw));
+    API_TRY(e, e->ws.getT("stem#b", (size_t)round_up(Cout, 64), &dbias));
+    API_TRY(e, e->ws.getT("stem#gamma", (size_t)Cout, &dg));
+    API_TRY(e, e->ws.getT("stem#beta", (size_t)Cout, &db));
+    API_TRY(e, e->ws.getT("stem#o", no, &dout));
+    API_TRY(e, e->ws.getT("stem#prm", (size_t)B * Cout, &dprm));
+    API_TRY(e, e->ws.getT("stem#st", nst, &st));
+    API_TRY(e, e->ws.getT("stem#sp", (size_t)B * Cout, &sp));
+    API_TRY(e, e->ws.getT("stem#gram", stem_gram_scratch(B, round_up(H, 8), W), &gram));
+    API_TRY(e, e->ws.getT("stem#s16", 2 * plane, &s16));
+    API_TRY(e, e->ws.getT("stem#xs16", 2 * xplane, &xs16));
+    API_HIP(e, hipMemcpy(dx, d->x, nx * 4, hipMemcpyHostToDevice));
+    API_HIP(e, hipMemcpy(dw, d->w, (size_t)Cout * 27 * 4, hipMemcpyHostToDevice));
+    API_HIP(e, hipMemset(dbias, 0, (size_t)round_up(Cout, 64) * 4));
+    API_HIP(e, hipMemcpy(dbias, d->bias, (size_t)Cout * 4, hipMemcpyHostToDevice));
+    if (d->emit) {
+        API_HIP(e, hipMemcpy(dg, d->gamma, (size_t)Cout * 4, hipMemcpyHostToDevice));
+        API_HIP(e, hipMemcpy(db, d->beta, (size_t)Cout * 4, hipMemcpyHostToDevice));
+    }
+    API_HIP(e, hipMemsetAsync(dout, 0xFF, no * 4, e->stream));
+    API_HIP(e, hipMemsetAsync(st, 0xFF, nst * 8, e->stream));
+    API_HIP(e, hipMemsetAsync(sp, 0xFF, (size_t)B * Cout * 16, e->stream));
+    API_HIP(e, hipMemsetAsync(dprm, 0xFF, (size_t)B * Cout * 16, e->stream));
+    API_HIP(e, hipMemsetAsync(s16, 0xFF, 2 * plane, e->stream));
+    std::vector<uint16_t> w16v, wsv;
+    const float w_scale = pack_weights_conv6(d->w, Cout, 3, w16v);
+    if (d->route == 0) pack_weights_stem(d->w, Cout, w_scale, wsv);
+    const std::vector<uint16_t>& wv = d->route == 0 ? wsv : w16v;
+    void* wp = nullptr;
+    API_TRY(e, e->ws.get("stem#wp", wv.size() * 2, &wp));
+    API_HIP(e, hipMemcpy(wp, wv.data(), wv.size() * 2, hipMemcpyHostToDevice));
+    auto once = [&]() -> Status {
+        if (d->route == 0) {
+            StemArgs a;
+            a.x = dx; a.wst = wp; a.w_scale = w_scale; a.bias = dbias; a.out = dout; a.B = B; a.Cout = Cout; a.H = H; a.W = W;
+            a.range_ctr = e->range_ctr; a.x1 = x1;
+            if (d->emit) {
+                DPIR_TRY(launch_stem_stats(e->stream, dx, dw, 1, 27, w_scale, dbias, B, Cout, H, W, x1, gram, sp));
+                DPIR_TRY(launch_gn_prm(e->stream, GnStatSrc{nullptr, 0, sp, Cout}, GnStatSrc{}, (int)HW, dg, db, nullptr, 0, 0, B, Cout, true, dprm));
+                a.prm = dprm; a.hi = s16; a.lo = x1 ? nullptr : s16 + plane;
+            }
+            return launch_stem(e->stream, a);
+        }
+        DPIR_TRY(launch_act_split(e->stream, CatSrc{dx, 3, nullptr, 0}, nullptr, 0, B, H, W, xs16, x1 ? nullptr : xs16 + xplane, e->range_ctr));
+        Conv6Args a6;
+        a6.x1 = x1; a6.xhi = xs16; a6.xlo = xs16 + xplane; a6.w16 = wp; a6.w16_scale = w_scale; a6.bias = dbias; a6.out = dout;
+        a6.B = B; a6.Cin = 3; a6.Cout = Cout; a6.H = H; a6.W = W; a6.stat = slots > 0 ? st : nullptr;
+        Conv3Plan ran;
+        DPIR_TRY(launch_conv6(e->stream, a6, &ran));
+        if (!d->emit) return Status{};
+        if (ran.stat_kind != ST_SLOTS) return invalid("stem: launch_conv6 produced no epilogue statistics here");
+        DPIR_TRY(launch_gn_prm(e->stream, GnStatSrc{st, ran.stat_slots, nullptr, Cout}, GnStatSrc{}, (int)HW, dg, db, nullptr, 0, 0, B, Cout, true, dprm));
+        return launch_act_split(e->stream, CatSrc{dout, Cout, nullptr, 0}, dprm, 0, B, H, W, s16, x1 ? nullptr : s16 + plane, e->range_ctr);
+    };
+    API_TRY(e, once());
+    API_TRY(e, time_repeats(e->stream, d->iters, once, &d->ms_out));
+    API_HIP(e, hipStreamSynchronize(e->stream));
+    d->ran_out = d->route == 0 ? 1 : 7;
+    if (d->out) API_HIP(e, hipMemcpy(d->out, dout, no * 4, hipMemcpyDeviceToHost));
+    if (d->emit) {
+        if (d->stat_out) {
+            if (d->route == 0) API_HIP(e, hipMemcpy(d->stat_out, sp, (size_t)B * Cout * 16, hipMemcpyDeviceToHost));
+            else API_TRY(e, fold_slots(st, (size_t)B * Cout, slots, d->stat_out));
+        }
+        if (d->prm_out) API_HIP(e, hipMemcpy(d->prm_out, dprm, (size_t)B * Cout * 16, hipMemcpyDeviceToHost));
+        if (d->hi_out) API_HIP(e, hipMemcpy(d->hi_out, s16, plane, hipMemcpyDeviceToHost));
+        if (d->lo_out && !x1) API_HIP(e, hipMemcpy(d->lo_out, s16 + plane, plane, hipMemcpyDeviceToHost));
+    }
+    return DPIR_OK;
+}
+
 int dpir_debug_route_log(dpir_engine* e, dpir_debug_route_rec* recs, int cap, int* n_out) {
     if (!e || !n_out || (cap > 0 && !recs)) return DPIR_ERR_INVALID;
     *n_out = (int)e->route_log.size();
diff --git a/diffpir_amd/csrc/engine.h b/diffpir_amd/csrc/engine.h
--- a/diffpir_amd/csrc/engine.h
+++ b/diffpir_amd/csrc/engine.h
@@ -32,7 +32,8 @@
                void* w8 = nullptr; float w8_scale = 1.f;
                void* w16T = nullptr; float w16T_scale = 1.f;
                void* wup = nullptr; float wup_scale = 1.f;
-               void* w11 = nullptr; };
+               void* w11 = nullptr;
+               void* wst = nullptr; };
 struct GnW { float* gamma = nullptr; float* beta = nullptr; int c = 0; };
 struct ResW {
     std::string name;
diff --git a/diffpir_amd/csrc/stem.h b/diffpir_amd/csrc/stem.h
--- /dev/null
+++ b/diffpir_amd/csrc/stem.h
@@ -0,0 +1,23 @@
+#pragma once
+#include "common.h"
+#include <vector>
+namespace dpir {
+
+struct StemArgs {
+    const float* x = nullptr;
+    const void* wst = nullptr; float w_scale = 1.f;
+    const float* bias = nullptr; float* out = nullptr;
+    const float4* prm = nullptr; void* hi = nullptr; void* lo = nullptr;
+    int B = 0, Cout = 0, H = 0, W = 0;
+    unsigned long long* range_ctr = nullptr;
+    bool x1 = false;
+};
+const char* stem_refusal(int Cout, int H, int W);
+Status launch_stem(hipStream_t s, const StemArgs& a);
+void pack_weights_stem(const float* w_oihw, int cout, float scale, std::vector<uint16_t>& out);
+
+size_t stem_gram_scratch(int B, int H, int W);
+Status launch_stem_stats(hipStream_t s, const float* x, const float* w, int w_kstride, int w_cstride, float w_scale, const float* bias, int B, int Cout,
+                         int H, int W, bool x1, double* gram, double2* part);
+
+}
diff --git a/diffpir_amd/csrc/stem.hip b/diffpir_amd/csrc/stem.hip
--- /dev/null
+++ b/diffpir_amd/csrc/stem.hip
@@ -0,0 +1,386 @@
+#include "common.h"
+#include "elem.h"
+#include "lds_dma.h"
+#include "stem.h"
+
+namespace dpir {
+
+typedef float floatx4s __attribute__((ext_vector_type(4)));
+typedef double doublex4s __attribute__((ext_vector_type(4)));
+typedef _Float16 half8s __attribute__((ext_vector_type(8)));
+
+namespace stm {
+constexpr int TW = 32, TH = 8, LW = TW + 2, LH = TH + 2;
+constexpr int PATCH = LH * LW;
+constexpr int XS = 1024;
+constexpr int TS = 68;
+constexpr int SLAB = 16 * TS;
+constexpr size_t LDS_FIXED = (size_t)(XS + 4 * SLAB) * 4;
+constexpr int GRAM = 3 * 256;
+__device__ __forceinline__ int tap_off(int k) { const int ci = k / 9, t = k - ci * 9; return ci * PATCH + (t / 3) * LW + t % 3; }
+}
+
+struct StemK {
+    const float* x; const char* w; const float* bias; float* out;
+    const float4* prm; char* hi; char* lo; unsigned long long* range_ctr;
+    int B, Cout, H, W, tiles_x, tiles_y;
+    float out_scale;
+};
+
+__device__ __forceinline__ float silu_st(float v) {
+    float e = __builtin_amdgcn_exp2f(v * -1.4426950408889634f);
+    return v * __builtin_amdgcn_rcpf(1.0f + e);
+}
+
+#if defined(__HIP_DEVICE_COMPILE__)
+__device__ __forceinline__ bool stem_load_patch(const float* x, int B, int H, int W, int n0, int ty0, int tx0, float* xs, int tid) {
+    using namespace stm;
+    const int HW = H * W;
+    const __amdgpu_buffer_rsrc_t rx = rsrc_uniform(x, (unsigned)((size_t)B * 3 * HW * 4));
+    float v[4];
+#pragma unroll
+    for (int u = 0; u < 4; ++u) {
+        const int f = tid + u * 256;
+        const int ci = f / PATCH, e = f - ci * PATCH;
+        const int hy = e / LW, hx = e - hy * LW;
+        const int gy = ty0 + hy - 1, gx = tx0 + hx - 1;
+        const bool ok = ci < 3 && gy >= 0 && gy < H && gx >= 0 && gx < W;
+        v[u] = as_f32(__builtin_amdgcn_raw_buffer_load_b32(rx, ok ? (unsigned)((n0 * 3 + ci) * HW + gy * W + gx) * 4u : kOutOfRange, 0, 0));
+    }
+    bool bad = false;
+#pragma unroll
+    for (int u = 0; u < 4; ++u) {
+        bad |= !(fabsf(v[u]) <= 65000.f);
+        xs[tid + u * 256] = fminf(fmaxf(v[u], -65000.f), 65000.f);
+    }
+    return bad;
+}
+#endif
+
+template <bool EMIT, bool X1>
+__global__ __launch_bounds__(256) void stem_kernel(StemK p) {
+#if defined(__HIP_DEVICE_COMPILE__)
+    using namespace stm;
+    extern __shared__ __attribute__((aligned(16))) char smem_st[];
+    float* const xs = reinterpret_cast<float*>(smem_st);
+    const int tid = threadIdx.x;
+    const int lane = tid & 63;
+    const int wave = __builtin_amdgcn_readfirstlane(tid >> 6);
+    const int l15 = lane & 15, rsub = lane >> 4;
+    float* const tr = xs + XS + wave * SLAB;
+    float4* const tab = reinterpret_cast<float4*>(xs + XS + 4 * SLAB);
+
+    const int tiles_per_img = p.tiles_x * p.tiles_y;
+    const int n0 = blockIdx.x / tiles_per_img;
+    const int trem = blockIdx.x - n0 * tiles_per_img;
+    const int ty0 = (trem / p.tiles_x) * TH, tx0 = (trem % p.tiles_x) * TW;
+    const int HW = p.H * p.W;
+
+    bool bad = stem_load_patch(p.x, p.B, p.H, p.W, n0, ty0, tx0, xs, tid);
+    if constexpr (EMIT)
+        for (int c = tid; c < p.Cout; c += 256) tab[c] = p.prm[(size_t)n0 * p.Cout + c];
+    __syncthreads();
+
+    half8s b_h[4], b_l[4];
+    {
+        int off[8];
+#pragma unroll
+        for (int i = 0; i < 8; ++i) off[i] = tap_off(min(8 * rsub + i, 26));
+#pragma unroll
+        for (int nt = 0; nt < 4; ++nt) {
+            const float* px = xs + (2 * wave + (nt >> 1)) * LW + (nt & 1) * 16 + l15;
+#pragma unroll
+            for (int i = 0; i < 8; ++i) {
+                float v = px[off[i]];
+                v = 8 * rsub + i < 27 ? v : 0.f;
+                const _Float16 h = (_Float16)v;
+                b_h[nt][i] = h;
+                b_l[nt][i] = (_Float16)(v - (float)h);
+            }
+        }
+    }
+
+    const int n_mt = p.Cout >> 4;
+    const __amdgpu_buffer_rsrc_t rw = rsrc_uniform(p.w, (unsigned)n_mt * 2048u);
+    const __amdgpu_buffer_rsrc_t rb = rsrc_uniform(p.bias, (unsigned)p.Cout * 4u);
+    const __amdgpu_buffer_rsrc_t r_out = rsrc_uniform(p.out + (size_t)n0 * p.Cout * HW, (unsigned)((size_t)p.Cout * HW * 4));
+    typedef unsigned int u32x4 __attribute__((ext_vector_type(4)));
+    typedef unsigned int u32x2 __attribute__((ext_vector_type(2)));
+    typedef _Float16 half4v __attribute__((ext_vector_type(4)));
+    const float osc = p.out_scale;
+    const unsigned lane16 = (unsigned)lane * 16u;
+    const unsigned pix_out = (unsigned)((ty0 + 2 * wave + (l15 >> 3)) * p.W + tx0 + 4 * (l15 & 7));
+    const size_t pix_em = (size_t)(ty0 + 2 * wave + (rsub & 1)) * p.W + tx0 + l15;
+    const int C8 = p.Cout >> 3;
+
+    u32x4 a_h = __builtin_amdgcn_raw_buffer_load_b128(rw, lane16, 0, 0);
+    u32x4 a_l = __builtin_amdgcn_raw_buffer_load_b128(rw, lane16, 1024, 0);
+    u32x4 bv = __builtin_amdgcn_raw_buffer_load_b128(rb, (unsigned)(4 * rsub) * 4u, 0, 0);
+    for (int m = 0; m < n_mt; ++m) {
+        const half8s ah = __builtin_bit_cast(half8s, a_h), al = __builtin_bit_cast(half8s, a_l);
+        const float bias4[4] = {as_f32(bv.x), as_f32(bv.y), as_f32(bv.z), as_f32(bv.w)};
+        {
+            const int mn = min(m + 1, n_mt - 1);
+            a_h = __builtin_amdgcn_raw_buffer_load_b128(rw, lane16, (unsigned)mn * 2048u, 0);
+            a_l = __builtin_amdgcn_raw_buffer_load_b128(rw, lane16, (unsigned)mn * 2048u + 1024u, 0);
+            bv = __builtin_amdgcn_raw_buffer_load_b128(rb, (unsigned)(16 * mn + 4 * rsub) * 4u, 0, 0);
+        }
+        floatx4s acc[4];
+#pragma unroll
+        for (int nt = 0; nt < 4; ++nt) acc[nt] = floatx4s{0.f, 0.f, 0.f, 0.f};
+        if constexpr (!X1) {
+#pragma unroll
+            for (int nt = 0; nt < 4; ++nt) acc[nt] = __builtin_amdgcn_mfma_f32_16x16x32_f16(al, b_h[nt], acc[nt], 0, 0, 0);
+#pragma unroll
+            for (int nt = 0; nt < 4; ++nt) acc[nt] = __builtin_amdgcn_mfma_f32_16x16x32_f16(ah, b_l[nt], acc[nt], 0, 0, 0);
+        }
+#pragma unroll
+        for (int nt = 0; nt < 4; ++nt) acc[nt] = __builtin_amdgcn_mfma_f32_16x16x32_f16(ah, b_h[nt], acc[nt], 0, 0, 0);
+#pragma unroll
+        for (int nt = 0; nt < 4; ++nt)
+#pragma unroll
+            for (int r = 0; r < 4; ++r) {
+                acc[nt][r] = acc[nt][r] * osc + bias4[r];
+                tr[(4 * rsub + r) * TS + nt * 16 + l15] = acc[nt][r];
+            }
+        __builtin_amdgcn_wave_barrier();
+#pragma unroll
+        for (int it = 0; it < 4; ++it) {
+            const int co_l = it * 4 + rsub;
+            const float4 v = *reinterpret_cast<const float4*>(tr + co_l * TS + l15 * 4);
+            u32x4 sv;
+            sv.x = as_u32(v.x); sv.y = as_u32(v.y); sv.z = as_u32(v.z); sv.w = as_u32(v.w);
+            __builtin_amdgcn_raw_buffer_store_b128(sv, r_out, ((unsigned)(16 * m + co_l) * (unsigned)HW + pix_out) * 4u, 0, 0);
+        }
+        __builtin_amdgcn_wave_barrier();
+        if constexpr (EMIT) {
+            float4 t4[4];
+#pragma unroll
+            for (int q = 0; q < 4; ++q) t4[q] = tab[16 * m + 4 * rsub + q];
+            auto norm_split = [&](float x, const float4& t, _Float16& h, _Float16& l) __attribute__((always_inline)) {
+                float v = (x - t.x) * t.y + t.z;
+                v = silu_st(v);
+                bad |= !(fabsf(v) <= 65000.f);
+                v = fminf(fmaxf(v, -65000.f), 65000.f);
+                h = (_Float16)v;
+                l = (_Float16)(v - (float)h);
+            };
+            const size_t ebase = ((size_t)n0 * C8 + 2 * m + (rsub >> 1)) * HW + pix_em;
+#pragma unroll
+            for (int cb = 0; cb < 2; ++cb) {
+                half4v h0, l0, h1, l1;
+#pragma unroll
+                for (int q = 0; q < 4; ++q) {
+                    _Float16 th, tl;
+                    norm_split(acc[cb][q], t4[q], th, tl); h0[q] = th; l0[q] = tl;
+                    norm_split(acc[2 + cb][q], t4[q], th, tl); h1[q] = th; l1[q] = tl;
+                }
+                const u32x2 a_hh = __builtin_bit_cast(u32x2, h0), b_hh = __builtin_bit_cast(u32x2, h1);
+                const size_t eo = (ebase + (size_t)(16 * cb)) << 4;
+                u32x4 eh;
+                {
+                    const auto s0 = __builtin_amdgcn_permlane16_swap(a_hh.x, b_hh.x, false, false), s1 = __builtin_amdgcn_permlane16_swap(a_hh.y, b_hh.y, false, false);
+                    eh.x = s0[0]; eh.y = s1[0]; eh.z = s0[1]; eh.w = s1[1];
+                }
+                *reinterpret_cast<u32x4*>(p.hi + eo) = eh;
+                if constexpr (!X1) {
+                    const u32x2 a_ll = __builtin_bit_cast(u32x2, l0), b_ll = __builtin_bit_cast(u32x2, l1);
+                    u32x4 el;
+                    const auto s0 = __builtin_amdgcn_permlane16_swap(a_ll.x, b_ll.x, false, false), s1 = __builtin_amdgcn_permlane16_swap(a_ll.y, b_ll.y, false, false);
+                    el.x = s0[0]; el.y = s1[0]; el.z = s0[1]; el.w = s1[1];
+                    *reinterpret_cast<u32x4*>(p.lo + eo) = el;
+                }
+            }
+        }
+    }
+    {
+        const unsigned long long mk = __ballot(bad);
+        if (mk != 0ull && p.range_ctr && lane == (int)__builtin_ctzll(mk)) atomicAdd(p.range_ctr, (unsigned long long)__builtin_popcountll(mk));
+    }
+#endif
+}
+
+const char* stem_refusal(int Cout, int H, int W) { return stem_shape_refusal(Cout, H, W); }
+
+Status launch_stem(hipStream_t s, const StemArgs& a) {
+    if (const char* why = stem_refusal(a.Cout, a.H, a.W)) return Status{DPIR_ERR_UNSUPPORTED, why};
+    if (!a.x || !a.wst || !a.bias || !a.out || a.B <= 0) return invalid("stem: bad arguments");
+    const bool emit = a.prm != nullptr;
+    if (emit && (!a.hi || (!a.x1 && !a.lo))) return invalid("stem: the plane emission needs the table and the planes");
+    const size_t HW = (size_t)a.H * a.W;
+    if ((size_t)a.B * 3 * HW * 4 >= ((size_t)1 << 32) || (size_t)a.Cout * HW * 4 >= ((size_t)1 << 32))
+        return invalid("stem: the input or an image's output exceeds the 4 GiB buffer-descriptor range");
+    StemK k{};
+    k.x = a.x; k.w = reinterpret_cast<const char*>(a.wst); k.bias = a.bias; k.out = a.out;
+    k.prm = a.prm; k.hi = reinterpret_cast<char*>(a.hi); k.lo = reinterpret_cast<char*>(a.lo); k.range_ctr = a.range_ctr;
+    k.B = a.B; k.Cout = a.Cout; k.H = a.H; k.W = a.W; k.tiles_x = a.W / 32; k.tiles_y = a.H / 8;
+    k.out_scale = 1.0f / a.w_scale;
+    const long long blocks = (long long)k.tiles_x * k.tiles_y * a.B;
+    if (blocks > 0x7FFFFFFFll) return invalid("stem: too many workgroups");
+    const size_t lds = stm::LDS_FIXED + (emit ? (size_t)a.Cout * 16 : 0);
+    if (lds > 64 * 1024) return Status{DPIR_ERR_UNSUPPORTED, "stem: the GroupNorm table does not fit in LDS"};
+    auto fn = emit ? (a.x1 ? stem_kernel<true, true> : stem_kernel<true, false>) : (a.x1 ? stem_kernel<false, true> : stem_kernel<false, false>);
+    hipLaunchKernelGGL(fn, dim3((unsigned)blocks), dim3(256), lds, s, k);
+    DPIR_HIP(hipGetLastError());
+    return Status{};
+}
+
+void pack_weights_stem(const float* w, int cout, float scale, std::vector<uint16_t>& out) {
+    const int n_mt = cout / 16;
+    out.assign((size_t)n_mt * 2 * 512, 0);
+    for (int m = 0; m < n_mt; ++m) {
+        uint16_t* hi = out.data() + (size_t)m * 2 * 512;
+        uint16_t* lo = hi + 512;
+        for (int l = 0; l < 64; ++l)
+            for (int j = 0; j < 8; ++j) {
+                const int co = m * 16 + (l & 15), k = 8 * (l >> 4) + j;
+                const float v = k < 27 ? w[(size_t)co * 27 + k] * scale : 0.f;
+                const _Float16 h = (_Float16)v;
+                const _Float16 lw = (_Float16)(v - (float)h);
+                __builtin_memcpy(&hi[(size_t)l * 8 + j], &h, 2);
+                __builtin_memcpy(&lo[(size_t)l * 8 + j], &lw, 2);
+            }
+    }
+}
+
+template <bool X1>
+__global__ __launch_bounds__(256) void stem_gram_kernel(const float* x, int B, int H, int W, double* part) {
+#if defined(__HIP_DEVICE_COMPILE__)
+    using namespace stm;
+    __shared__ float xs[XS];
+    __shared__ double red[4 * GRAM];
+    const int tid = threadIdx.x;
+    const int lane = tid & 63;
+    const int wave = __builtin_amdgcn_readfirstlane(tid >> 6);
+    const int l15 = lane & 15, kq = lane >> 4;
+    const int n0 = blockIdx.y, ty0 = blockIdx.x * TH;
+    const int HW = H * W;
+    const __amdgpu_buffer_rsrc_t rx = rsrc_uniform(x, (unsigned)((size_t)B * 3 * HW * 4));
+    unsigned base[4]; int hxm1[4];
+#pragma unroll
+    for (int u = 0; u < 4; ++u) {
+        const int f = tid + u * 256;
+        const int ci = f / PATCH, e = f - ci * PATCH;
+        const int hy = e / LW, gy = ty0 + hy - 1;
+        hxm1[u] = e - hy * LW - 1;
+        base[u] = ci < 3 && gy >= 0 && gy < H ? (unsigned)((n0 * 3 + ci) * HW + gy * W) : kOutOfRange;
+    }
+    float nx[4];
+    auto request = [&](int tx0) __attribute__((always_inline)) {
+#pragma unroll
+        for (int u = 0; u < 4; ++u) {
+            const int gx = tx0 + hxm1[u];
+            const bool ok = base[u] != kOutOfRange && gx >= 0 && gx < W;
+            nx[u] = as_f32(__builtin_amdgcn_raw_buffer_load_b32(rx, ok ? (base[u] + (unsigned)gx) * 4u : kOutOfRange, 0, 0));
+        }
+    };
+    const int off0 = tap_off(l15), off1 = tap_off(min(16 + l15, 26));
+    const bool one1 = l15 == 11, zero1 = l15 > 11;
+    doublex4s g00 = {0, 0, 0, 0}, g01 = {0, 0, 0, 0}, g11 = {0, 0, 0, 0};
+    request(0);
+    for (int tx0 = 0; tx0 < W; tx0 += TW) {
+        __syncthreads();
+#pragma unroll
+        for (int u = 0; u < 4; ++u) {
+            float v = fminf(fmaxf(nx[u], -65000.f), 65000.f);
+            if constexpr (X1) v = (float)(_Float16)v;
+            xs[tid + u * 256] = v;
+        }
+        __syncthreads();
+        request(min(tx0 + TW, W - TW));
+#pragma unroll
+        for (int j = 0; j < 2; ++j) {
+            const float* px = xs + (2 * wave + j) * LW + kq;
+#pragma unroll
+            for (int s4 = 0; s4 < TW; s4 += 4) {
+                const double a0 = (double)px[s4 + off0];
+                const float v1 = px[s4 + off1];
+                const double a1 = one1 ? 1.0 : (zero1 ? 0.0 : (double)v1);
+                g00 = __builtin_amdgcn_mfma_f64_16x16x4f64(a0, a0, g00, 0, 0, 0);
+                g01 = __builtin_amdgcn_mfma_f64_16x16x4f64(a0, a1, g01, 0, 0, 0);
+                g11 = __builtin_amdgcn_mfma_f64_16x16x4f64(a1, a1, g11, 0, 0, 0);
+            }
+        }
+    }
+#pragma unroll
+    for (int r = 0; r < 4; ++r) {
+        red[wave * GRAM + (0 * 4 + r) * 64 + lane] = g00[r];
+        red[wave * GRAM + (1 * 4 + r) * 64 + lane] = g01[r];
+        red[wave * GRAM + (2 * 4 + r) * 64 + lane] = g11[r];
+    }
+    __syncthreads();
+    double* const dst = part + ((size_t)n0 * gridDim.x + blockIdx.x) * GRAM;
+#pragma unroll
+    for (int u = 0; u < 3; ++u) {
+        const int e = tid + u * 256;
+        dst[e] = ((red[e] + red[GRAM + e]) + red[2 * GRAM + e]) + red[3 * GRAM + e];
+    }
+#endif
+}
+
+__global__ __launch_bounds__(768) void stem_gram_fold_kernel(const double* part, int strips, const float* w, int w_kstride, int w_cstride, const float* bias, int Cout,
+                                                             float x1_scale, double2* out) {
+    using namespace stm;
+    __shared__ double G[32][33];
+    __shared__ double ti[24][28][2];
+    const int tid = threadIdx.x, n0 = blockIdx.y, c0 = blockIdx.x * 24;
+    const int cl = tid / 28, i = tid - cl * 28;
+    const int c = min(c0 + cl, Cout - 1);
+    double wv[28];
+#pragma unroll
+    for (int j = 0; j < 28; ++j) {
+        float v = j < 27 ? w[(size_t)c * w_cstride + (size_t)j * w_kstride] : bias[c];
+        if (j < 27 && x1_scale != 0.f) v = (float)(_Float16)(v * x1_scale) / x1_scale;
+        wv[j] = (double)v;
+    }
+    {
+        const double* src = part + (size_t)n0 * strips * GRAM + tid;
+        double v = 0.0;
+        int st = 0;
+        for (; st + 16 <= strips; st += 16) {
+            double t[16];
+#pragma unroll
+            for (int u = 0; u < 16; ++u) t[u] = src[(size_t)(st + u) * GRAM];
+#pragma unroll
+            for (int u = 0; u < 16; ++u) v += t[u];
+        }
+        for (; st < strips; ++st) v += src[(size_t)st * GRAM];
+        const int tile = tid >> 8, r = (tid >> 6) & 3, l = tid & 63;
+        const int row = (l >> 4) + 4 * r + (tile == 2 ? 16 : 0), col = (l & 15) + (tile >= 1 ? 16 : 0);
+        G[row][col] = v;
+        if (tile == 1) G[col][row] = v;
+    }
+    __syncthreads();
+    if (cl < 24) {
+        double t = 0.0, wi = 0.0;
+#pragma unroll
+        for (int j = 0; j < 28; ++j) {
+            t += G[i][j] * wv[j];
+            wi = j == i ? wv[j] : wi;
+        }
+        ti[cl][i][0] = wi * G[i][27];
+        ti[cl][i][1] = wi * t;
+    }
+    __syncthreads();
+    if (tid < 24 && c0 + tid < Cout) {
+        double S = 0.0, SS = 0.0;
+        for (int k = 0; k < 28; ++k) { S += ti[tid][k][0]; SS += ti[tid][k][1]; }
+        out[(size_t)n0 * Cout + c0 + tid] = make_double2(S, SS);
+    }
+}
+
+size_t stem_gram_scratch(int B, int H, int W) { (void)W; return (size_t)B * (H / 8) * stm::GRAM; }
+
+Status launch_stem_stats(hipStream_t s, const float* x, const float* w, int w_kstride, int w_cstride, float w_scale, const float* bias, int B, int Cout,
+                         int H, int W, bool x1, double* gram, double2* part) {
+    if (const char* why = stem_refusal(Cout, H, W)) return Status{DPIR_ERR_UNSUPPORTED, why};
+    if (!x || !w || !bias || !gram || !part || B <= 0 || B > 65535) return invalid("stem statistics: bad arguments");
+    if ((size_t)B * 3 * H * W * 4 >= ((size_t)1 << 32)) return invalid("stem statistics: the input exceeds the 4 GiB buffer-descriptor range");
+    if (x1) hipLaunchKernelGGL(stem_gram_kernel<true>, dim3(H / 8, B), dim3(256), 0, s, x, B, H, W, gram);
+    else hipLaunchKernelGGL(stem_gram_kernel<false>, dim3(H / 8, B), dim3(256), 0, s, x, B, H, W, gram);
+    hipLaunchKernelGGL(stem_gram_fold_kernel, dim3((Cout + 23) / 24, B), dim3(768), 0, s, (const double*)gram, H / 8, w, w_kstride, w_cstride, bias, Cout, x1 ? w_scale : 0.f, part);
+    DPIR_HIP(hipGetLastError());
+    return Status{};
+}
+
+}
diff --git a/diffpir_amd/csrc/unet.hip b/diffpir_amd/csrc/unet.hip
--- a/diffpir_amd/csrc/unet.hip
+++ b/diffpir_amd/csrc/unet.hip
@@ -3,6 +3,7 @@
 #include "conv9.h"
 #include "conv11.h"
 #include "conv_up.h"
+#include "stem.h"
 #include <unordered_map>
 #include <cstdint>
 #include <math.h>
@@ -115,6 +116,11 @@
             pack_weights_conv11(w, cout, cin, out->w16_scale, w11);
             DPIR_TRY(upload16(e, w11, "the conv11 weights", &out->w11));
         }
+        if (ks == 3 && !one_d && cin == 3 && cout % 32 == 0) {
+            std::vector<uint16_t> wst;
+            pack_weights_stem(w, cout, out->w16_scale, wst);
+            DPIR_TRY(upload16(e, wst, "the stem weights", &out->wst));
+        }
         if (up_pack && ks == 3 && !one_d && cin % 16 == 0 && cout % 32 == 0) {
             std::vector<uint16_t> wu;
             out->wup_scale = pack_weights_conv_up(w, cout, cin, wu);
@@ -308,6 +314,11 @@
     std::unordered_map<const float*, FusedStat> fused;
     PendingConv pending;
     bool grad = false;
+    struct StemPlanes { const float* h = nullptr; const float* gamma = nullptr; } stem_planes;
+    Status s16_buffer(size_t bytes, char** p) {
+        stem_planes = StemPlanes{};
+        return ws.getT("act#s16", bytes, p);
+    }
     bool x1() const { return e->precision == 2; }
 
     std::string layer;
@@ -374,6 +385,13 @@
                    const float* res, int res_mode, float* out, int Ho, int Wo, float4** prm_out = nullptr, float2** stats_out = nullptr,
                    const Conv6Emit* emit = nullptr) {
         const int C = in.C();
+        if (stem_planes.h && stem_planes.h == in.a && !in.b && stem_planes.gamma == g.gamma && mode == 0 && !grad) {
+            const size_t plane = (size_t)B * (2 * ((C + 15) / 16)) * Ho * Wo * 16;
+            char* s16 = nullptr;
+            DPIR_TRY(ws.getT("act#s16", 2 * plane, &s16));
+            stem_planes = StemPlanes{};
+            return conv6_on_planes(cw, s16, plane, res, res_mode, out, Ho, Wo, emit);
+        }
         const bool planes = cw.ks == 3 && plan_conv3(query(cw, C, Ho, Wo, emit != nullptr, res != nullptr), knobs, caps).kernel != CK_FP32;
         if (knobs.fuse_small && planes && C == g.c && C % 16 == 0 && gn_act_small_supported(C, in.H, in.W, mode)) {
             int eh = mode == 1 ? Ho / 2 : (mode == 2 ? Ho * 2 : Ho), ew = mode == 1 ? Wo / 2 : (mode == 2 ? Wo * 2 : Wo);
@@ -381,7 +399,7 @@
             const int C8 = 2 * ((C + 15) / 16);
             const size_t plane = (size_t)B * C8 * Ho * Wo * 16;
             char* s16 = nullptr;
-            DPIR_TRY(ws.getT("act#s16", 2 * plane, &s16));
+            DPIR_TRY(s16_buffer(2 * plane, &s16));
             DPIR_TRY(small_prologue(g, tag, film_off, in, mode, res, s16, plane, prm_out, stats_out));
             return conv6_on_planes(cw, s16, plane, res, res_mode, out, Ho, Wo, emit);
         }
@@ -470,7 +488,7 @@
             const size_t plane = (size_t)B * C8 * Ho * Wo * 16;
             if (plane >= ((size_t)1 << 32)) return invalid("conv: split activation plane exceeds the 4 GiB buffer-descriptor range; reduce the batch");
             char* s16 = nullptr;
-            DPIR_TRY(ws.getT("act#s16", 2 * plane, &s16));
+            DPIR_TRY(s16_buffer(2 * plane, &s16));
             {
                 ProfScope ps(&e->prof, PC_ELEM);
                 DPIR_TRY(launch_act_split(s, CatSrc{in.a, in.ca, in.b, in.cb}, prm, mode, B, Ho, Wo, s16, x1() ? nullptr : s16 + plane, e->range_ctr));
@@ -555,7 +573,7 @@
         const int C = in.C(), C8 = 2 * (C / 16);
         const size_t plane = (size_t)B * C8 * in.H * in.W * 16;
         char* s16 = nullptr;
-        DPIR_TRY(ws.getT("act#s16", 2 * plane, &s16));
+        DPIR_TRY(s16_buffer(2 * plane, &s16));
         if (knobs.fuse_small && gn_act_small_supported(C, in.H, in.W, 0)) {
             DPIR_TRY(small_prologue(r.gn1, r.name + "#gn1", -1, in, 0, nullptr, s16, plane));
         } else {
@@ -599,6 +617,20 @@
         return Status{};
     }
 
+    ResblockQuery res_query(const ResW& r, const Act& in) const {
+        const int Cin = in.C();
+        const int Ho = r.mode == 1 ? in.H * 2 : (r.mode == 2 ? in.H / 2 : in.H), Wo = r.mode == 1 ? in.W * 2 : (r.mode == 2 ? in.W / 2 : in.W);
+        ResblockQuery rq;
+        rq.B = B; rq.Cin = Cin; rq.Cout = r.cout; rq.H = in.H; rq.W = in.W; rq.mode = r.mode; rq.concat = in.b != nullptr; rq.has_skip = r.has_skip;
+        rq.gn1_c = r.gn1.c; rq.gn2_c = r.gn2.c; rq.precision = e->precision; rq.grad = grad;
+        rq.hop_allowed = fuse_h1; rq.arena_words_left = fuse_arena ? fuse_cap - fuse_off : 0;
+        rq.conv1_w16 = r.conv1.w16; rq.conv1_w11 = r.conv1.w11; rq.conv1_wup = r.conv1.wup; rq.conv2_w16 = r.conv2.w16; rq.conv2_w11 = r.conv2.w11;
+        rq.skip_w16 = r.has_skip && r.skip.w16;
+        rq.small_prologue = gn_act_small_supported(Cin, in.H, in.W, 0); rq.conv5_ok = conv5_supported(B, r.cout, Ho, Wo);
+        rq.slab = true; rq.slab_floats = partial_cap;
+        return rq;
+    }
+
     Status resblock(const ResW& r, const Act& in, Act* out) {
         if (in.C() != r.cin) return invalid("resblock " + r.name + ": input channels mismatch");
         int Ho = r.mode == 1 ? in.H * 2 : (r.mode == 2 ? in.H / 2 : in.H);
@@ -608,14 +640,7 @@
         float* h1 = nullptr;
         DPIR_TRY(ws.getT(r.name + "#h1", on, &h1));
         const int Cin = in.C();
-        ResblockQuery rq;
-        rq.B = B; rq.Cin = Cin; rq.Cout = r.cout; rq.H = in.H; rq.W = in.W; rq.mode = r.mode; rq.concat = in.b != nullptr; rq.has_skip = r.has_skip;
-        rq.gn1_c = r.gn1.c; rq.gn2_c = r.gn2.c; rq.precision = e->precision; rq.grad = grad;
-        rq.hop_allowed = fuse_h1; rq.arena_words_left = fuse_arena ? fuse_cap - fuse_off : 0;
-        rq.conv1_w16 = r.conv1.w16; rq.conv1_w11 = r.conv1.w11; rq.conv1_wup = r.conv1.wup; rq.conv2_w16 = r.conv2.w16; rq.conv2_w11 = r.conv2.w11;
-        rq.skip_w16 = r.has_skip && r.skip.w16;
-        rq.small_prologue = gn_act_small_supported(Cin, in.H, in.W, 0); rq.conv5_ok = conv5_supported(B, r.cout, Ho, Wo);
-        rq.slab = true; rq.slab_floats = partial_cap;
+        const ResblockQuery rq = res_query(r, in);
         const ResblockPlan rp = plan_resblock(rq, knobs, caps);
         if (rp.up) return resblock_up(r, rp, in, out, Ho, Wo, h1, on);
         Act h1a; h1a.a = h1; h1a.ca = r.cout; h1a.H = Ho; h1a.W = Wo;
@@ -631,7 +656,7 @@
             DPIR_TRY(gn(r.gn1, in, r.name + "#gn1", -1, true, &prm1, &tr.st1));
             tr.prm1 = prm1;
             char* s16 = nullptr;
-            DPIR_TRY(ws.getT("act#s16", 2 * eplane, &s16));
+            DPIR_TRY(s16_buffer(2 * eplane, &s16));
             float* sk = nullptr;
             DPIR_TRY(ws.getT(r.name + "#skip", on, &sk));
             Conv5Args a5;
@@ -811,9 +836,48 @@
         DPIR_TRY(ws.getT("input_blocks.0.0#out", on, &o));
         Act xin; xin.a = x; xin.ca = 3; xin.H = H; xin.W = W;
         f.layer = "input_blocks.0.0";
-        DPIR_TRY(f.conv(net.conv_in, xin, 0, nullptr, nullptr, 0, o, H, W));
+        h.a = o; h.ca = net.conv_in.cout; h.H = H; h.W = W;
+        StemQuery sq;
+        sq.B = B; sq.Cin = net.conv_in.cin; sq.Cout = net.conv_in.cout; sq.H = H; sq.W = W; sq.precision = e->precision; sq.grad = f.grad;
+        sq.pack = net.conv_in.ks == 3 && net.conv_in.wst;
+        const ResW* r1 = net.in_blocks.size() > 1 && !net.in_blocks[1].empty() && net.in_blocks[1][0].kind == 1 ? &net.res[net.in_blocks[1][0].idx] : nullptr;
+        if (r1 && r1->cin == h.ca) {
+            sq.block1_res = true; sq.block1_mode = r1->mode; sq.block1_gn1_c = r1->gn1.c;
+            const ResblockQuery rq = f.res_query(*r1, h);
+            sq.block1 = plan_resblock(rq, f.knobs, f.caps);
+            sq.block1_small_prologue = f.knobs.fuse_small && r1->conv1.ks == 3 && sq.block1.conv1.kernel != CK_FP32 && h.ca == r1->gn1.c && h.ca % 16 == 0 && rq.small_prologue;
+        }
+        const StemPlan sp = plan_stem(sq, f.knobs);
+        if (sp.take) {
+            double* gram = nullptr; double2* part = nullptr;
+            DPIR_TRY(ws.getT("stem#gram", stem_gram_scratch(B, H, W), &gram));
+            DPIR_TRY(ws.getT("sp#" + std::to_string(reinterpret_cast<uintptr_t>(o)), (size_t)B * h.ca, &part));
+            {
+                ProfScope ps(&e->prof, PC_GN);
+                DPIR_TRY(launch_stem_stats(s, x, net.conv_in.w, net.conv_in.coutp, 1, net.conv_in.w16_scale, net.conv_in.bias, B, h.ca, H, W, f.x1(), gram, part));
+            }
+            f.fused[o] = Fwd::FusedStat{nullptr, 0, part};
+            float4* prm = nullptr;
+            DPIR_TRY(f.gn(r1->gn1, h, r1->name + "#gn1", -1, true, &prm));
+            const size_t plane = (size_t)B * (h.ca / 8) * H * W * 16;
+            if (plane >= ((size_t)1 << 32)) return invalid("conv: split activation plane exceeds the 4 GiB buffer-descriptor range; reduce the batch");
+            char* s16 = nullptr;
+            DPIR_TRY(f.s16_buffer(2 * plane, &s16));
+            StemArgs sa;
+            sa.x = x; sa.wst = net.conv_in.wst; sa.w_scale = net.conv_in.w16_scale; sa.bias = net.conv_in.bias; sa.out = o;
+            sa.prm = prm; sa.hi = s16; sa.lo = f.x1() ? nullptr : s16 + plane; sa.B = B; sa.Cout = h.ca; sa.H = H; sa.W = W;
+            sa.range_ctr = e->range_ctr; sa.x1 = f.x1();
+            {
+                ProfScope ps(&e->prof, PC_CONV3);
+                DPIR_TRY(launch_stem(s, sa));
+            }
+            Conv3Plan lp; lp.kernel = CK_STEM; lp.geo = 0; lp.workgroups = sp.workgroups; lp.stat_kind = ST_PLANE;
+            f.log(CK_STEM, 3, lp, HOP_NONE);
+            f.stem_planes.h = o; f.stem_planes.gamma = r1->gn1.gamma;
+        } else {
+            DPIR_TRY(f.conv(net.conv_in, xin, 0, nullptr, nullptr, 0, o, H, W));
+        }
         f.tap("input_blocks.0.0", o, on);
-        h.a = o; h.ca = net.conv_in.cout; h.H = H; h.W = W;
         hs.push_back(h);
         if (f.grad) e->tape.conv_in_out = o;
     }
diff --git a/include/diffpir_debug.h b/include/diffpir_debug.h
--- a/include/diffpir_debug.h
+++ b/include/diffpir_debug.h
@@ -91,6 +91,13 @@
     uint64_t guard_bad_out;
 } dpir_debug_groupnorm_desc;
 int dpir_debug_groupnorm(dpir_engine* e, dpir_debug_groupnorm_desc* d);
+typedef struct dpir_debug_stem_desc {
+    int32_t B, Cout, H, W, route, emit, iters, ran_out;
+    const float *x, *w, *bias, *gamma, *beta;
+    float* out; double* stat_out; float* prm_out; uint16_t* hi_out; uint16_t* lo_out;
+    double ms_out;
+} dpir_debug_stem_desc;
+int dpir_debug_stem(dpir_engine* e, dpir_debug_stem_desc* d);
 #ifdef __cplusplus
 }
 #endif
```

After: 9.736 images/s, median of 6. About the same (+0.9%).
